# ponimatkin/freepose

Hardware: AMD Instinct MI355X
Metric: proposals/sec (ViT-L feat + top-k + 576-pose render-compare) (higher is better)
Workload: dtype bf16

## Files before the change

### freepose_amd/_lib.py

```python
from __future__ import annotations

import ctypes as C
import os
from pathlib import Path

_HERE = Path(__file__).resolve().parent
LIB_PATH = _HERE / "lib" / "libfreepose_hip.so"
LAB_LIB_PATH = _HERE / "lib" / "libfreepose_hip_lab.so"

_lib = None
_use_lab = False


def use_lab():
    global _use_lab
    if _lib is not None and not _use_lab:
        raise RuntimeError("use_lab() after the product library was loaded")
    _use_lab = True


def is_lab() -> bool:
    return _use_lab

c_void_p, c_int, c_float, c_double, c_size_t, c_char_p = C.c_void_p, C.c_int, C.c_float, C.c_double, C.c_size_t, C.c_char_p
P = C.POINTER


class VitArch(C.Structure):
    _fields_ = [("dim", c_int), ("depth", c_int), ("heads", c_int), ("mlp_dim", c_int), ("patch", c_int),
                ("n_reg", c_int), ("pos_grid", c_int), ("ln_eps", c_float)]


class ClipArch(C.Structure):
    _fields_ = [("width", c_int), ("depth", c_int), ("heads", c_int), ("mlp_dim", c_int), ("patch", c_int), ("grid", c_int),
                ("embed_dim", c_int), ("ln_eps", c_float), ("quick_gelu", c_int)]


class ClipTextArch(C.Structure):
    _fields_ = [("width", c_int), ("depth", c_int), ("heads", c_int), ("mlp_dim", c_int), ("vocab", c_int), ("ctx", c_int),
                ("embed_dim", c_int), ("ln_eps", c_float)]


SIGNATURES = {
    "fp_last_error": (c_char_p, []),
    "fp_version": (c_int, []),
    "fp_ctx_create": (c_int, [c_int, P(c_void_p)]),
    "fp_ctx_destroy": (c_int, [c_void_p]),
    "fp_ctx_set_option": (c_int, [c_void_p, c_char_p, c_int]),
    "fp_ctx_workspace_bytes": (c_size_t, [c_void_p]),
    "fp_vit_create": (c_int, [c_void_p, P(VitArch), P(c_void_p)]),
    "fp_vit_destroy": (c_int, [c_void_p]),
    "fp_vit_set_weight": (c_int, [c_void_p, c_char_p, c_void_p, c_size_t, c_void_p]),
    "fp_vit_forward": (c_int, [c_void_p, c_void_p, c_int, c_int, c_int, c_int, c_int, c_void_p, c_void_p]),
    "fp_vit_flops": (c_double, [c_void_p, c_int, c_int, c_int, c_int]),
    "fp_ffa": (c_int, [c_void_p, c_void_p, c_void_p, c_int, c_int, c_int, c_int, c_int, c_int, c_void_p, c_void_p, c_void_p]),
    "fp_bank_prepare": (c_int, [c_void_p, c_void_p, c_int, c_int, c_void_p, c_void_p]),
    "fp_bank_topk": (c_int, [c_void_p, c_void_p, c_int, c_int, c_void_p, c_int, c_int, c_int, c_void_p, c_void_p, c_void_p]),
    "fp_topk_merge": (c_int, [c_void_p, c_void_p, c_void_p, c_int, c_int, c_int, c_void_p, c_void_p, c_void_p]),
    "fp_rerank_views": (c_int, [c_void_p, c_void_p, c_void_p, c_void_p, c_void_p, c_int, c_int, c_int, c_int, c_void_p, c_void_p]),
    "fp_l2_normalize": (c_int, [c_void_p, c_void_p, c_int, c_int, c_void_p, c_void_p]),
    "fp_template_score": (c_int, [c_void_p, c_void_p, c_void_p, c_void_p, c_int, c_int, c_int, c_void_p, c_void_p]),
    "fp_template_score_normed": (c_int, [c_void_p, c_void_p, c_void_p, c_void_p, c_int, c_int, c_int, c_void_p, c_void_p]),
    "fp_crop_resize_pad": (c_int, [c_void_p, c_void_p, c_int, c_int, c_int, c_int, c_int, c_void_p, c_int, c_float,
                                   c_int, c_void_p, c_int, c_void_p, c_int, c_void_p]),
    "fp_roi_align": (c_int, [c_void_p, c_void_p, c_int, c_int, c_int, c_int, c_void_p, c_int, c_int, c_int, c_int, c_float,
                             c_void_p, c_void_p]),
    "fp_generate_rotations": (c_int, [c_int, c_void_p]),
    "fp_geodesic_select": (c_int, [c_void_p, c_void_p, c_int, c_void_p, c_double, c_void_p, P(c_int), c_void_p]),
    "fp_mesh_upload": (c_int, [c_void_p, c_void_p, c_int, c_void_p, c_int, c_void_p, P(c_void_p)]),
    "fp_mesh_upload_textured": (c_int, [c_void_p, c_void_p, c_int, c_void_p, c_int, c_void_p, c_void_p, c_int, c_int, c_void_p,
                                        P(c_void_p)]),
    "fp_mesh_set_ambient": (c_int, [c_void_p, c_float]),
    "fp_mesh_set_shading": (c_int, [c_void_p, c_int]),
    "fp_mesh_set_filter": (c_int, [c_void_p, c_int]),
    "fp_mesh_set_cull": (c_int, [c_void_p, c_int]),
    "fp_project_vertices": (c_int, [c_void_p, c_void_p, c_void_p, c_int, c_float, c_float, c_float, c_float, c_float, c_void_p,
                                    c_void_p, c_void_p]),
    "fp_mesh_destroy": (c_int, [c_void_p]),
    "fp_rasterize": (c_int, [c_void_p, c_void_p, c_void_p, c_int, c_float, c_float, c_float, c_float, c_float, c_int,
                             c_int, c_void_p, c_void_p, c_void_p]),
    "fp_rasterize_extents": (c_int, [c_void_p, c_void_p, c_void_p, c_int, c_float, c_float, c_float, c_float, c_float, c_int,
                                     c_int, c_void_p, c_void_p, c_void_p, c_void_p, c_void_p]),
    "fp_depth_extents": (c_int, [c_void_p, c_void_p, c_int, c_int, c_int, c_float, c_float, c_float, c_float, c_void_p,
                                 c_void_p]),
    "fp_chamfer": (c_int, [c_void_p, c_void_p, c_int, c_void_p, c_void_p, c_int, c_int, c_int, c_int, c_void_p, c_void_p]),
    "fp_depth_compare": (c_int, [c_void_p, c_void_p, c_void_p, c_int, c_int, c_int, c_void_p, c_int, c_void_p, c_void_p, c_void_p, c_int,
                                 c_void_p, c_void_p]),
    "fp_label_components": (c_int, [c_void_p, c_void_p, c_int, c_int, c_int, c_int, c_void_p, c_void_p]),
    "fp_depthmap_scale": (c_int, [c_void_p, c_void_p, c_void_p, c_int, c_int, c_int, c_double, c_double, c_double, c_double, c_double,
                                  c_double, c_int, c_int, c_void_p, c_void_p, c_void_p, c_void_p]),
    "fp_comm_unique_id": (c_int, [c_void_p]),
    "fp_comm_init": (c_int, [c_void_p, c_int, c_int, c_void_p]),
    "fp_comm_destroy": (c_int, [c_void_p]),
    "fp_comm_size": (c_int, [c_void_p]),
    "fp_comm_rank": (c_int, [c_void_p]),
    "fp_allgather_bytes": (c_int, [c_void_p, c_void_p, c_size_t, c_void_p, c_void_p]),
    "fp_allgather_topk": (c_int, [c_void_p, c_void_p, c_void_p, c_int, c_int, c_int, c_void_p, c_void_p, c_void_p]),
    "fp_allgather_poses": (c_int, [c_void_p, c_void_p, c_int, c_int, c_void_p, c_void_p]),
    "fp_op_gemm": (c_int, [c_void_p, c_void_p, c_int, c_void_p, c_int, c_void_p, c_int, c_void_p, c_void_p, c_void_p, c_int, c_int,
                           c_int, c_int, c_int, c_void_p]),
    "fp_op_gemm_vt": (c_int, [c_void_p, c_void_p, c_int, c_void_p, c_int, c_void_p, c_void_p, c_int, c_int, c_int, c_int, c_int,
                              c_void_p]),
    "fp_op_ln_linear": (c_int, [c_void_p, c_void_p, c_int, c_int, c_void_p, c_void_p, c_float, c_void_p, c_int, c_void_p, c_int, c_int,
                                c_int, c_int, c_float, c_void_p, c_void_p]),
    "fp_op_gemm_stats": (c_int, [c_void_p, c_void_p, c_int, c_void_p, c_int, c_void_p, c_int, c_void_p, c_void_p, c_void_p, c_int, c_int,
                                 c_int, c_int, c_float, c_void_p, c_void_p]),
    "fp_op_gemm_patch": (c_int, [c_void_p, c_void_p, c_int, c_void_p, c_int, c_void_p, c_int, c_void_p, c_void_p, c_int, c_int, c_int,
                                 c_int, c_int, c_int, c_void_p]),
    "fp_op_ln_chain": (c_int, [c_void_p, c_void_p, c_int, c_void_p, c_void_p, c_void_p, c_void_p, c_void_p, c_int, c_int, c_void_p,
                               c_void_p, c_float, c_void_p, c_int, c_void_p, c_int, c_int, c_float, c_int, c_void_p, c_int, c_void_p,
                               c_void_p, c_void_p]),
    "fp_op_gelu": (c_int, [c_void_p, c_void_p, c_size_t, c_void_p]),
    "fp_op_attention": (c_int, [c_void_p, c_int, c_void_p, c_void_p, c_int, c_int, c_int, c_int, c_int, c_int, c_void_p]),
    "fp_op_layernorm": (c_int, [c_void_p, c_void_p, c_void_p, c_void_p, c_int, c_int, c_float, c_void_p]),
    "fp_op_im2col_norm": (c_int, [c_void_p, c_void_p, c_int, c_int, c_int, c_int, c_int, c_void_p]),
    "fp_op_attention_hd": (c_int, [c_void_p, c_int, c_void_p, c_int, c_int, c_int, c_int, c_int, c_int, c_float, c_void_p]),
    "fp_op_attention_causal": (c_int, [c_void_p, c_int, c_void_p, c_int, c_int, c_int, c_int, c_int, c_int, c_float, c_void_p]),
    "fp_clip_text_create": (c_int, [c_void_p, P(ClipTextArch), P(c_void_p)]),
    "fp_clip_text_destroy": (c_int, [c_void_p]),
    "fp_clip_text_set_weight": (c_int, [c_void_p, c_char_p, c_void_p, c_size_t, c_void_p]),
    "fp_clip_text_encode": (c_int, [c_void_p, c_void_p, c_int, c_void_p, c_void_p]),
    "fp_clip_text_flops": (c_double, [c_void_p, c_int]),
    "fp_clip_create": (c_int, [c_void_p, P(ClipArch), P(c_void_p)]),
    "fp_clip_destroy": (c_int, [c_void_p]),
    "fp_clip_set_weight": (c_int, [c_void_p, c_char_p, c_void_p, c_size_t, c_void_p]),
    "fp_clip_encode_image": (c_int, [c_void_p, c_void_p, c_int, c_int, c_void_p, c_void_p]),
    "fp_clip_flops": (c_double, [c_void_p, c_int]),
    "fp_knn_l2": (c_int, [c_void_p, c_void_p, c_int, c_int, c_void_p, c_int, c_int, c_void_p, c_void_p, c_void_p]),
    "fp_patch_points": (c_int, [c_void_p, c_void_p, c_int, c_void_p, c_void_p, c_void_p, c_void_p, c_int, c_int, c_double, c_void_p, c_void_p]),
    "fp_pnp_epnp": (c_int, [c_void_p, c_void_p, c_void_p, c_void_p, c_void_p, c_int, c_int, c_void_p, c_void_p]),
    "fp_video_errors": (c_int, [c_void_p, c_void_p, c_void_p, c_void_p, c_void_p, c_int, c_int, c_int, c_int, c_void_p, c_void_p, c_void_p,
                                c_void_p, c_void_p]),
    "fp_bop_scores": (c_int, [c_void_p, c_void_p, c_void_p, c_void_p, c_void_p, c_void_p, c_void_p, c_int, c_int, c_int, c_int, c_int, c_int,
                              c_int, c_void_p, c_void_p, c_void_p, c_void_p, c_void_p, c_void_p]),
    "fp_gt_visibility": (c_int, [c_void_p, c_void_p, c_int, c_int, c_int, c_int, c_int, c_void_p, c_int, c_int, c_int, c_void_p, c_void_p,
                                 c_void_p, c_void_p, c_void_p, c_void_p]),
    "fp_pts_diameter": (c_int, [c_void_p, c_void_p, c_int, c_void_p, c_int, c_void_p, c_void_p]),
    "fp_timer_create": (c_int, [P(c_void_p)]),
    "fp_timer_start": (c_int, [c_void_p, c_void_p]),
    "fp_timer_stop": (c_int, [c_void_p, c_void_p]),
    "fp_timer_elapsed_ms": (c_int, [c_void_p, P(c_float)]),
    "fp_timer_destroy": (c_int, [c_void_p]),
    "fp_vit_profile": (c_int, [c_void_p, c_int]),
    "fp_vit_profile_read": (c_int, [c_void_p, P(c_float), P(c_float), P(c_float), P(c_double)]),
    "fp_vit_profile_gemm_launches": (C.c_long, [c_void_p]),
}


def load(path: os.PathLike | None = None):
    global _lib
    if _lib is not None and path is None:
        return _lib
    p = Path(path) if path else (LAB_LIB_PATH if _use_lab else LIB_PATH)
    if not p.exists():
        raise RuntimeError(
            f"{p} not found: the HIP extension is not built (run `python -m freepose_amd.build`). "
            "freepose_amd has no CPU fallback.")
    lib = C.CDLL(str(p), mode=C.RTLD_GLOBAL)
    for name, (res, args) in SIGNATURES.items():
        fn = getattr(lib, name)
        fn.restype = res
        fn.argtypes = args
    if hasattr(lib, "fp_lab_set_option"):
        lib.fp_lab_set_option.restype = c_int
        lib.fp_lab_set_option.argtypes = [c_char_p, c_int]
        lib.fp_lab_read_scratch.restype = c_int
        lib.fp_lab_read_scratch.argtypes = [c_void_p, c_void_p, c_size_t]
    if path is None:
        _lib = lib
    return lib


def check(rc: int, what: str = ""):
    if rc != 0:
        msg = load().fp_last_error()
        raise RuntimeError(f"libfreepose_hip {what} failed (code {rc}): {msg.decode() if msg else '?'}")


def ptr(t):
    if t is None:
        return None
    if hasattr(t, "data_ptr"):
        return C.c_void_p(t.data_ptr())
    return C.c_void_p(t.ctypes.data)


def current_stream():
    import torch
    return C.c_void_p(torch.cuda.current_stream().cuda_stream)
```

### freepose_amd/csrc/attention.hip

```cpp
#include "internal.h"

#include <stdlib.h>

#include <type_traits>

namespace {

typedef __attribute__((ext_vector_type(2))) float f32x2_t;

constexpr int HD = 64;
constexpr int KVB = 64;
constexpr int QW = 32;
constexpr int NWAVE = 4;
constexpr int QB = QW * NWAVE;
constexpr int ROWB = 128;
constexpr int TILE = KVB * ROWB;
constexpr int STAGE = 2 * TILE;
constexpr float LAZY_THR = 40.0f;

struct AttnArgs {
    const bf16_t* QK; int ldqk;
    const bf16_t* Vt;
    bf16_t* O; int ldo;
    int B, H, n_tok, npad, D;
    float scale_log2e;
    int q_base;
};

__device__ __forceinline__ float vmax2(float a, float b) {
    float d;
    asm("v_max_f32 %0, %1, %2" : "=v"(d) : "v"(a), "v"(b));
    return d;
}
__device__ __forceinline__ float xlane_max16(float v) {
    const auto r = __builtin_amdgcn_permlane16_swap(__float_as_uint(v), __float_as_uint(v), false, false);
    return vmax2(__uint_as_float(r[0]), __uint_as_float(r[1]));
}
__device__ __forceinline__ float xlane_max32(float v) {
    const auto r = __builtin_amdgcn_permlane32_swap(__float_as_uint(v), __float_as_uint(v), false, false);
    return vmax2(__uint_as_float(r[0]), __uint_as_float(r[1]));
}
__device__ __forceinline__ int key_plain(int row) { return (row >> 1) & 7; }
__device__ __forceinline__ int key_krow(int row) { return ((((row >> 3) & 3) << 1) | ((row >> 1) & 1)) & 7; }
__device__ __forceinline__ int key_perm4(int row) {
    const int rl = row & 63;
    return (((rl >> 4) << 1) | ((rl & 3) >> 1)) & 7;
}

template <int NSLOT, int VAR = 0>
__global__ __launch_bounds__(NWAVE * 64, (VAR & 16) ? 4 : 3) void attn_fwd_kernel(AttnArgs p) {
    extern __shared__ __attribute__((aligned(1024))) char smem[];
    const int tid = threadIdx.x, lane = tid & 63;
    const int wave = __builtin_amdgcn_readfirstlane(tid >> 6);
    const int li = lane & 15, lg = lane >> 4;
    const int nqb = (p.npad - p.q_base + QB - 1) / QB;
    int bid = blockIdx.x;
    {
        const int nwg = gridDim.x;
        const int q = nwg >> 3, r = nwg & 7, xcd = bid & 7, pos = bid >> 3;
        bid = (xcd < r ? xcd * (q + 1) : r * (q + 1) + (xcd - r) * q) + pos;
    }
    const int qb = bid % nqb, bh = bid / nqb;
    const int h = bh % p.H, b = bh / p.H;
    const int q0 = p.q_base + qb * QB + wave * QW;
    const bool idle = q0 >= p.npad;

    const size_t rowbase = (size_t)b * p.npad;
    const char* gQK = (const char*)p.QK;
    const char* gVt = (const char*)(p.Vt + ((size_t)b * p.H + h) * HD * p.npad);

    bf16x8_t qf[2][2];
#pragma unroll
    for (int fq = 0; fq < 2; ++fq) {
        const int q = min(q0 + 16 * fq + li, p.npad - 1);
        const char* src = gQK + ((rowbase + q) * p.ldqk + h * HD) * 2;
#pragma unroll
        for (int kk = 0; kk < 2; ++kk) qf[fq][kk] = *(const bf16x8_t*)(src + (kk * 4 + lg) * 16);
    }

    uint32_t offK[2];
    int rowK[2];
    uint32_t offV[2];
    int slotV[2];
#pragma unroll
    for (int it = 0; it < 2; ++it) {
        const int row = (it * NWAVE + wave) * 8 + (lane >> 3);
        rowK[it] = row;
        offK[it] = (uint32_t)((p.D + h * HD) * 2 + (((lane & 7) ^ key_krow(row)) << 4));
        slotV[it] = (lane & 7) ^ key_perm4(row);
        offV[it] = (uint32_t)row * (uint32_t)p.npad * 2u;
    }
    const char* gKb = gQK + rowbase * (size_t)p.ldqk * 2;
    uint32_t lofK[2], lofV[2];
#pragma unroll
    for (int it = 0; it < 2; ++it) {
        lofK[it] = (uint32_t)rowK[it] * (uint32_t)p.ldqk * 2u + offK[it];
        lofV[it] = offV[it] + (uint32_t)(slotV[it] * 16);
    }
    const uint32_t kstep = (uint32_t)p.ldqk * 2u;
    auto stage = [&](int buf, int kv0) {
        char* sb = smem + buf * STAGE;
        if (kv0 + KVB <= p.npad) {
#pragma unroll
            for (int it = 0; it < 2; ++it) glds16_buf(gKb, lofK[it], (uint32_t)kv0 * kstep, sb + (it * NWAVE + wave) * 1024);
#pragma unroll
            for (int it = 0; it < 2; ++it) glds16_buf(gVt, lofV[it], (uint32_t)kv0 * 2u, sb + TILE + (it * NWAVE + wave) * 1024);
        } else {
#pragma unroll
            for (int it = 0; it < 2; ++it) {
                const int key = min(kv0 + rowK[it], p.npad - 1);
                glds16(gQK + (rowbase + key) * (size_t)p.ldqk * 2 + offK[it], sb + (it * NWAVE + wave) * 1024);
            }
#pragma unroll
            for (int it = 0; it < 2; ++it) {
                const int k8 = min(kv0 + slotV[it] * 8, p.npad - 8);
                glds16(gVt + offV[it] + (size_t)k8 * 2, sb + TILE + (it * NWAVE + wave) * 1024);
            }
        }
    };

    const int keyK = (((li >> 2) << 1) | ((li & 3) >> 1)) & 7;
    const int baseK = ((li >> 2) * 8 + (li & 3)) * ROWB;
    const int keyV = (((li >> 2) << 1) | ((li & 3) >> 1)) & 7;
    const int baseV = TILE + ((li >> 2) * 16 + (li & 3)) * ROWB;

    f32x4_t o[4][2];
#pragma unroll
    for (int i = 0; i < 4; ++i)
#pragma unroll
        for (int j = 0; j < 2; ++j) o[i][j] = f32x4_t{0.f, 0.f, 0.f, 0.f};
    float mrow[2] = {-1e30f, -1e30f};
    float mthr[2] = {-1e30f, -1e30f};
    float nmb[2] = {0.f, 0.f};
    constexpr bool PRE = (VAR & 64) != 0;
    constexpr bool VSUM = (VAR & 256) != 0;
    float vsum[2] = {0.f, 0.f};
    f32x4_t nref[2] = {f32x4_t{0.f, 0.f, 0.f, 0.f}, f32x4_t{0.f, 0.f, 0.f, 0.f}};
    f32x4_t lacc[2] = {f32x4_t{0.f, 0.f, 0.f, 0.f}, f32x4_t{0.f, 0.f, 0.f, 0.f}};
    bf16x8_t ones;
#pragma unroll
    for (int e = 0; e < 8; ++e) ones[e] = (__bf16)1.0f;

    const int ntile = (p.n_tok + KVB - 1) / KVB;
    constexpr bool SHORT = (VAR & 4) != 0;
    auto tile_of = [&](int sq) { return SHORT ? (sq == 0 ? ntile - 1 : sq - 1) : sq; };
    constexpr int PF = NSLOT - 1;
    stage(0, tile_of(0) * KVB);
#pragma unroll
    for (int i = 1; i < PF; ++i)
        if (ntile > i) stage(i, tile_of(i) * KVB);
    asm volatile("s_waitcnt vmcnt(0)" ::: "memory");
#pragma unroll
    for (int fq = 0; fq < 2; ++fq)
#pragma unroll
        for (int kk = 0; kk < 2; ++kk) asm volatile("" : "+v"(qf[fq][kk]));
    if constexpr (VAR & 2) {
        const int d = (blockIdx.x * 5) % 12;
        for (int i = 0; i < d; ++i) __builtin_amdgcn_s_sleep(2);
    }
    auto tile_body = [&](int t, auto slot_c, auto nks_c, auto first_c) {
        const int slot = slot_c;
        constexpr int NKS = decltype(nks_c)::value;
        constexpr bool FIRST = decltype(first_c)::value;
        const int ahead = min(PF - 1, ntile - 1 - t);
        if (ahead >= 2) asm volatile("s_waitcnt vmcnt(8)" ::: "memory");
        else if (ahead == 1) asm volatile("s_waitcnt vmcnt(4)" ::: "memory");
        else asm volatile("s_waitcnt vmcnt(0)" ::: "memory");
        __builtin_amdgcn_s_barrier();
        asm volatile("" ::: "memory");
        if (t + PF < ntile) stage(slot >= 1 ? slot - 1 : NSLOT - 1, tile_of(t + PF) * KVB);
        if (idle) return;
        const char* sb = smem + slot * STAGE;
        const int kv0 = tile_of(t) * KVB;

        f32x4_t s[4][2];
        if constexpr (VAR & 1) __builtin_amdgcn_s_setprio(1);
#pragma unroll
        for (int kk = 0; kk < 2; ++kk) {
            const int slot = (((kk << 2) | lg) ^ keyK) << 4;
#pragma unroll
            for (int fk = 0; fk < 2 * NKS; ++fk) {
                const bf16x8_t kf = *(const bf16x8_t*)(sb + baseK + (32 * (fk >> 1) + 4 * (fk & 1)) * ROWB + slot);
#pragma unroll
                for (int fq = 0; fq < 2; ++fq)
                    s[fk][fq] = __builtin_amdgcn_mfma_f32_16x16x32_bf16(kf, qf[fq][kk], kk == 0 ? (PRE ? nref[fq] : f32x4_t{0.f, 0.f, 0.f, 0.f}) : s[fk][fq], 0, 0, 0);
            }
        }
        if constexpr (VAR & 1) __builtin_amdgcn_s_setprio(0);
        if (kv0 + KVB > p.n_tok) {
#pragma unroll
            for (int fk = 0; fk < 2 * NKS; ++fk)
#pragma unroll
                for (int r = 0; r < 4; ++r)
                    if (kv0 + 32 * (fk >> 1) + 8 * lg + 4 * (fk & 1) + r >= p.n_tok) {
                        s[fk][0][r] = -1e30f;
                        s[fk][1][r] = -1e30f;
                    }
        }

        constexpr bool JITV = (VAR & 16) != 0;
        bf16x8_t vf[JITV ? 1 : 2][4];
        if constexpr (!JITV) {
#pragma unroll
        for (int ks = 0; ks < NKS; ++ks) {
            const int sv = (((ks << 2) | lg) ^ keyV) << 4;
#pragma unroll
            for (int fd = 0; fd < 4; ++fd) vf[ks][fd] = *(const bf16x8_t*)(sb + baseV + fd * 4 * ROWB + sv);
        }
        }

        bf16x8_t pf[2][2];
        auto softmax_max = [&](int fq) {
            float mx;
            if constexpr (NKS == 1)
                asm("v_max3_f32 %0, %1, %2, %3\n\tv_max3_f32 %0, %0, %4, %5\n\tv_max3_f32 %0, %0, %6, %7\n\tv_max_f32 %0, %0, %8"
                    : "=&v"(mx)
                    : "v"(s[0][fq][0]), "v"(s[0][fq][1]), "v"(s[0][fq][2]), "v"(s[0][fq][3]), "v"(s[1][fq][0]), "v"(s[1][fq][1]),
                      "v"(s[1][fq][2]), "v"(s[1][fq][3]));
            else
            asm("v_max3_f32 %0, %1, %2, %3\n\tv_max3_f32 %0, %0, %4, %5\n\tv_max3_f32 %0, %0, %6, %7\n\tv_max3_f32 %0, %0, %8, %9\n\t"
                "v_max3_f32 %0, %0, %10, %11\n\tv_max3_f32 %0, %0, %12, %13\n\tv_max3_f32 %0, %0, %14, %15\n\tv_max_f32 %0, %0, %16"
                : "=&v"(mx)
                : "v"(s[0][fq][0]), "v"(s[0][fq][1]), "v"(s[0][fq][2]), "v"(s[0][fq][3]), "v"(s[1][fq][0]), "v"(s[1][fq][1]),
                  "v"(s[1][fq][2]), "v"(s[1][fq][3]), "v"(s[2][fq][0]), "v"(s[2][fq][1]), "v"(s[2][fq][2]), "v"(s[2][fq][3]),
                  "v"(s[3][fq][0]), "v"(s[3][fq][1]), "v"(s[3][fq][2]), "v"(s[3][fq][3]));
            if constexpr (PRE) {
                constexpr float THR2 = LAZY_THR * 1.4426950408889634f / 8.0f;
                if (FIRST || __builtin_amdgcn_ballot_w64(mx > THR2) != 0) {
                    mx = xlane_max16(mx);
                    mx = xlane_max32(mx);
                    const float delta = FIRST ? mx : vmax2(mx, 0.f);
#pragma unroll
                    for (int r = 0; r < 4; ++r) nref[fq][r] -= delta;
#pragma unroll
                    for (int fk = 0; fk < 2 * NKS; ++fk)
#pragma unroll
                        for (int r = 0; r < 4; ++r) s[fk][fq][r] -= delta;
                    if constexpr (!FIRST) {
                        const float alpha = __builtin_amdgcn_exp2f(-delta);
                        lacc[fq][0] *= alpha;
                        if constexpr (VSUM) vsum[fq] *= alpha;
#pragma unroll
                        for (int fd = 0; fd < 4; ++fd)
#pragma unroll
                            for (int r = 0; r < 4; ++r) o[fd][fq][r] *= alpha;
                    }
                }
            } else
            if (__builtin_amdgcn_ballot_w64(mx > mthr[fq]) != 0) {
                mx = xlane_max16(mx);
                mx = xlane_max32(mx);
                const float mnew = vmax2(mrow[fq], mx);
                const float alpha = __builtin_amdgcn_exp2f((mrow[fq] - mnew) * p.scale_log2e);
                mrow[fq] = mnew;
                mthr[fq] = mnew + LAZY_THR;
                nmb[fq] = -(mnew * p.scale_log2e);
                lacc[fq][0] *= alpha;
#pragma unroll
                for (int fd = 0; fd < 4; ++fd)
#pragma unroll
                    for (int r = 0; r < 4; ++r) o[fd][fq][r] *= alpha;
            }
        };
        auto softmax_exp = [&](int fq) {
            float pv[4][4];
            if constexpr (PRE) {
#pragma unroll
                for (int fk = 0; fk < 2 * NKS; ++fk)
#pragma unroll
                    for (int r = 0; r < 4; ++r) pv[fk][r] = __builtin_amdgcn_exp2f(s[fk][fq][r]);
            } else if constexpr (VAR & 128) {
                const f32x2_t sc2 = {p.scale_log2e, p.scale_log2e};
                const f32x2_t mb2 = {nmb[fq], nmb[fq]};
#pragma unroll
                for (int fk = 0; fk < 2 * NKS; ++fk)
#pragma unroll
                    for (int r = 0; r < 4; r += 2) {
                        const f32x2_t a = {s[fk][fq][r], s[fk][fq][r + 1]};
                        const f32x2_t e = __builtin_elementwise_fma(a, sc2, mb2);
                        pv[fk][r] = __builtin_amdgcn_exp2f(e[0]);
                        pv[fk][r + 1] = __builtin_amdgcn_exp2f(e[1]);
                    }
            } else {
#pragma unroll
                for (int fk = 0; fk < 2 * NKS; ++fk)
#pragma unroll
                    for (int r = 0; r < 4; ++r) {
                        float e;
                        asm("v_fma_f32 %0, %1, %2, %3" : "=v"(e) : "v"(s[fk][fq][r]), "v"(p.scale_log2e), "v"(nmb[fq]));
                        pv[fk][r] = __builtin_amdgcn_exp2f(e);
                    }
            }
#pragma unroll
            for (int ks = 0; ks < NKS; ++ks) {
                uint4 w;
                w.x = pack_bf2(pv[2 * ks][0], pv[2 * ks][1]);
                w.y = pack_bf2(pv[2 * ks][2], pv[2 * ks][3]);
                w.z = pack_bf2(pv[2 * ks + 1][0], pv[2 * ks + 1][1]);
                w.w = pack_bf2(pv[2 * ks + 1][2], pv[2 * ks + 1][3]);
                pf[fq][ks] = __builtin_bit_cast(bf16x8_t, w);
            }
        };
        auto pv_half = [&](int fq) {
#pragma unroll
            for (int ks = 0; ks < NKS; ++ks) {
#pragma unroll
                for (int fd = 0; fd < 4; ++fd)
                    o[fd][fq] = __builtin_amdgcn_mfma_f32_16x16x32_bf16(vf[JITV ? 0 : ks][fd], pf[fq][ks], o[fd][fq], 0, 0, 0);
                lacc[fq] = __builtin_amdgcn_mfma_f32_16x16x32_bf16(ones, pf[fq][ks], lacc[fq], 0, 0, 0);
            }
        };

        if constexpr (JITV) {
            softmax_max(0);
            softmax_exp(0);
            softmax_max(1);
            softmax_exp(1);
#pragma unroll
            for (int ks = 0; ks < NKS; ++ks) {
                const int sv = (((ks << 2) | lg) ^ keyV) << 4;
#pragma unroll
                for (int fd = 0; fd < 4; ++fd) vf[0][fd] = *(const bf16x8_t*)(sb + baseV + fd * 4 * ROWB + sv);
#pragma unroll
                for (int fq = 0; fq < 2; ++fq) {
#pragma unroll
                    for (int fd = 0; fd < 4; ++fd)
                        o[fd][fq] = __builtin_amdgcn_mfma_f32_16x16x32_bf16(vf[0][fd], pf[fq][ks], o[fd][fq], 0, 0, 0);
                    if constexpr (VSUM) {
                        typedef __bf16 bf16x2_hw __attribute__((ext_vector_type(2)));
                        const uint4 pw = __builtin_bit_cast(uint4, pf[fq][ks]);
                        const bf16x2_hw one2 = __builtin_bit_cast(bf16x2_hw, 0x3f803f80u);
                        vsum[fq] = __builtin_amdgcn_fdot2_f32_bf16(__builtin_bit_cast(bf16x2_hw, pw.x), one2, vsum[fq], false);
                        vsum[fq] = __builtin_amdgcn_fdot2_f32_bf16(__builtin_bit_cast(bf16x2_hw, pw.y), one2, vsum[fq], false);
                        vsum[fq] = __builtin_amdgcn_fdot2_f32_bf16(__builtin_bit_cast(bf16x2_hw, pw.z), one2, vsum[fq], false);
                        vsum[fq] = __builtin_amdgcn_fdot2_f32_bf16(__builtin_bit_cast(bf16x2_hw, pw.w), one2, vsum[fq], false);
                    } else {
                        lacc[fq] = __builtin_amdgcn_mfma_f32_16x16x32_bf16(ones, pf[fq][ks], lacc[fq], 0, 0, 0);
                    }
                }
            }
            return;
        }
        softmax_max(0);
        softmax_exp(0);
        softmax_max(1);
        __builtin_amdgcn_sched_barrier(0);
        softmax_exp(1);
        pv_half(0);
#pragma unroll
        for (int g = 0; g < 5 * NKS; ++g) {
            __builtin_amdgcn_sched_group_barrier(0x008, 1, 0);
            __builtin_amdgcn_sched_group_barrier(0x002, 4, 0);
        }
        __builtin_amdgcn_sched_barrier(0);
        if constexpr (VAR & 1) __builtin_amdgcn_s_setprio(1);
        pv_half(1);
        if constexpr (VAR & 1) __builtin_amdgcn_s_setprio(0);
    };
    using full_c = std::integral_constant<int, 2>;
    using half_c = std::integral_constant<int, 1>;
    using yes_c = std::true_type;
    using no_c = std::false_type;
    if constexpr (SHORT) {
        static_assert(NSLOT == 2, "the short-tail prologue is written for the 2-slot ring");
        tile_body(0, std::integral_constant<int, 0>{}, half_c{}, yes_c{});
        for (int t = 1; t < ntile; t += 2) {
            tile_body(t, std::integral_constant<int, 1>{}, full_c{}, no_c{});
            if (t + 1 < ntile) tile_body(t + 1, std::integral_constant<int, 0>{}, full_c{}, no_c{});
        }
    } else if constexpr (NSLOT == 2 && PRE) {
        tile_body(0, std::integral_constant<int, 0>{}, full_c{}, yes_c{});
        for (int t = 1; t < ntile; t += 2) {
            tile_body(t, std::integral_constant<int, 1>{}, full_c{}, no_c{});
            if (t + 1 < ntile) tile_body(t + 1, std::integral_constant<int, 0>{}, full_c{}, no_c{});
        }
    } else if constexpr (NSLOT == 2) {
        for (int t = 0; t < ntile; t += 2) {
            tile_body(t, std::integral_constant<int, 0>{}, full_c{}, no_c{});
            if (t + 1 < ntile) tile_body(t + 1, std::integral_constant<int, 1>{}, full_c{}, no_c{});
        }
    } else {
        tile_body(0, 0, full_c{}, yes_c{});
        int slot = NSLOT > 1 ? 1 : 0;
        for (int t = 1; t < ntile; ++t) {
            tile_body(t, slot, full_c{}, no_c{});
            slot = slot + 1 == NSLOT ? 0 : slot + 1;
        }
    }

#pragma unroll
    for (int fq = 0; fq < 2; ++fq) {
        float rowsum = lacc[fq][0];
        if constexpr (VSUM) {
            rowsum = vsum[fq];
            rowsum += lane_xor<16>(rowsum);
            rowsum += lane_xor<32>(rowsum);
        }
        const float inv = 1.0f / rowsum;
        const int q = q0 + 16 * fq + li;
        if (q < p.npad) {
            uint4 w0, w1;
            w0.x = pack_bf2(o[0][fq][0] * inv, o[0][fq][1] * inv);
            w0.y = pack_bf2(o[0][fq][2] * inv, o[0][fq][3] * inv);
            w0.z = pack_bf2(o[1][fq][0] * inv, o[1][fq][1] * inv);
            w0.w = pack_bf2(o[1][fq][2] * inv, o[1][fq][3] * inv);
            w1.x = pack_bf2(o[2][fq][0] * inv, o[2][fq][1] * inv);
            w1.y = pack_bf2(o[2][fq][2] * inv, o[2][fq][3] * inv);
            w1.z = pack_bf2(o[3][fq][0] * inv, o[3][fq][1] * inv);
            w1.w = pack_bf2(o[3][fq][2] * inv, o[3][fq][3] * inv);
            uint4* dst = (uint4*)(p.O + (rowbase + q) * p.ldo + h * HD + lg * 16);
            dst[0] = w0;
            dst[1] = w1;
        }
    }
}

}

int fp_attention_fwd(const bf16_t* QK, int ldqk, const bf16_t* Vt, bf16_t* O, int ldo, int B, int H,
                     int n_tok, int npad, bool q_prescaled, hipStream_t stream) {
    FP_REQUIRE(B > 0 && H > 0 && n_tok > 0 && npad >= n_tok && npad % 16 == 0,
               "attention: bad shape B=%d H=%d n_tok=%d npad=%d", B, H, n_tok, npad);
    FP_REQUIRE(npad >= 8, "attention: npad too small");
    AttnArgs a;
    a.QK = QK; a.ldqk = ldqk; a.Vt = Vt; a.O = O; a.ldo = ldo;
    a.B = B; a.H = H; a.n_tok = n_tok; a.npad = npad; a.D = H * HD;
    a.scale_log2e = FP_ATTN_QSCALE;
    a.q_base = 0;
    dim3 grid(cdiv(npad - a.q_base, QB) * H * B);
    const bool short_tail = n_tok > KVB && n_tok - (cdiv(n_tok, KVB) - 1) * KVB <= KVB / 2;
#ifdef FP_LAB
    const int nslot = fp_opt_get(FP_OPT_ATTN_SLOTS, 2);
    static int env_var = [] { const char* e = getenv("FP_ATTN_VARIANT"); return e ? atoi(e) : 0; }();
    const int avar = fp_opt_get(FP_OPT_ATTN_VARIANT, env_var);
    if (!q_prescaled) {
    if (nslot == 2 && (avar & 2)) { hipLaunchKernelGGL((attn_fwd_kernel<2, 2>), grid, dim3(NWAVE * 64), 2 * STAGE, stream, a); FP_LAUNCH_CHECK(); return FP_OK; }
    if (nslot == 2 && (avar & 1)) { hipLaunchKernelGGL((attn_fwd_kernel<2, 1>), grid, dim3(NWAVE * 64), 2 * STAGE, stream, a); FP_LAUNCH_CHECK(); return FP_OK; }
    if (nslot == 4) { hipLaunchKernelGGL(attn_fwd_kernel<4>, grid, dim3(NWAVE * 64), 4 * STAGE, stream, a); FP_LAUNCH_CHECK(); return FP_OK; }
    if (nslot == 3) { hipLaunchKernelGGL(attn_fwd_kernel<3>, grid, dim3(NWAVE * 64), 3 * STAGE, stream, a); FP_LAUNCH_CHECK(); return FP_OK; }
    if (avar & 8) { hipLaunchKernelGGL(attn_fwd_kernel<2>, grid, dim3(NWAVE * 64), 2 * STAGE, stream, a); FP_LAUNCH_CHECK(); return FP_OK; }
    if ((avar & 128) && !q_prescaled) {
        if (short_tail) hipLaunchKernelGGL((attn_fwd_kernel<2, 4 | 16 | 128>), grid, dim3(NWAVE * 64), 2 * STAGE, stream, a);
        else hipLaunchKernelGGL((attn_fwd_kernel<2, 16 | 128>), grid, dim3(NWAVE * 64), 2 * STAGE, stream, a);
        FP_LAUNCH_CHECK();
        return FP_OK;
    }
    if (avar & 32) {
        if (short_tail) hipLaunchKernelGGL((attn_fwd_kernel<2, 4>), grid, dim3(NWAVE * 64), 2 * STAGE, stream, a);
        else hipLaunchKernelGGL(attn_fwd_kernel<2>, grid, dim3(NWAVE * 64), 2 * STAGE, stream, a);
        FP_LAUNCH_CHECK();
        return FP_OK;
    }
    }
#endif
#ifdef FP_LAB
    if (q_prescaled && (fp_opt_get(FP_OPT_ATTN_VARIANT, 0) & 256)) {
        if (short_tail) hipLaunchKernelGGL((attn_fwd_kernel<2, 4 | 16 | 64 | 256>), grid, dim3(NWAVE * 64), 2 * STAGE, stream, a);
        else hipLaunchKernelGGL((attn_fwd_kernel<2, 16 | 64 | 256>), grid, dim3(NWAVE * 64), 2 * STAGE, stream, a);
        FP_LAUNCH_CHECK();
        return FP_OK;
    }
#endif
    if (q_prescaled) {
        if (short_tail) hipLaunchKernelGGL((attn_fwd_kernel<2, 4 | 16 | 64>), grid, dim3(NWAVE * 64), 2 * STAGE, stream, a);
        else hipLaunchKernelGGL((attn_fwd_kernel<2, 16 | 64>), grid, dim3(NWAVE * 64), 2 * STAGE, stream, a);
    } else {
        if (short_tail) hipLaunchKernelGGL((attn_fwd_kernel<2, 4 | 16>), grid, dim3(NWAVE * 64), 2 * STAGE, stream, a);
        else hipLaunchKernelGGL((attn_fwd_kernel<2, 16>), grid, dim3(NWAVE * 64), 2 * STAGE, stream, a);
    }
    FP_LAUNCH_CHECK();
    return FP_OK;
}
```

### freepose_amd/csrc/capi.hip

```cpp
#include <stdarg.h>
#include <stdio.h>

#include "../../include/freepose_hip.h"
#include "tower_steps.h"
#include "pnp_core.h"
#include "video_eval_core.h"
#include "gt_info_core.h"

static thread_local char g_err[512] = "";
void fp_set_error(const char* fmt, ...) {
    va_list ap;
    va_start(ap, fmt);
    vsnprintf(g_err, sizeof(g_err), fmt, ap);
    va_end(ap);
}
extern "C" const char* fp_last_error(void) { return g_err; }
extern "C" int fp_version(void) { return 100; }

#ifdef FP_LAB
static int g_opts[FP_OPT_COUNT] = {-1, -1, -1, -1, -1, -1, -1, -1, -1, -1, -1, -1};
int fp_opt_get(int key, int dflt) { return (key >= 0 && key < FP_OPT_COUNT && g_opts[key] >= 0) ? g_opts[key] : dflt; }
extern "C" int fp_lab_set_option(const char* name, int value) {
    FP_REQUIRE(name, "lab_set_option: null name");
    if (!strcmp(name, "gemm_variant")) g_opts[FP_OPT_GEMM_VARIANT] = value;
// ... 207 lines not shown
extern "C" int fp_template_score_normed(fp_ctx* ctx, const void* d_tmpl_normed, const void* d_query, const float* d_weights,
                                        int T, int P, int D, float* d_scores, void* stream) {
    FP_REQUIRE(ctx && d_tmpl_normed && d_query && d_scores, "template_score_normed: null argument");
    if (T == 0) return FP_OK;
    float* dots;
    FP_WS(ctx, "tmpl.dots", (size_t)T * P * 4, dots);
    return fp_template_score_launch((const bf16_t*)d_tmpl_normed, (const bf16_t*)d_query, d_weights, dots, d_scores, T, P, D, 1,
                                    (hipStream_t)stream);
}

extern "C" int fp_chamfer(fp_ctx* ctx, const double* d_pts, int n_pts, const int32_t* d_table, const double* d_xf, int B, int max_n,
                          int ws_pts, int projected, double* d_out, void* stream) {
    FP_REQUIRE(ctx && d_pts && d_table && d_xf && d_out, "chamfer: null argument");
    FP_REQUIRE(B > 0 && B <= 65535, "chamfer: B=%d pairs (1..65535 per call)", B);
    FP_REQUIRE(n_pts > 0 && max_n > 0 && max_n <= n_pts, "chamfer: n_pts=%d max_n=%d (0 < max_n <= n_pts)", n_pts, max_n);
    FP_REQUIRE(ws_pts >= 2 && (size_t)ws_pts <= (size_t)2 * B * (size_t)max_n, "chamfer: ws_pts=%d for %d pairs of clouds up to %d points",
               ws_pts, B, max_n);
    FP_REQUIRE(projected == 0 || projected == 1, "chamfer: projected=%d (0 or 1)", projected);
    float* ws;
    double* slots;
    FP_WS(ctx, "chamfer.cloud", (size_t)ws_pts * 3 * sizeof(float), ws);
    FP_WS(ctx, "chamfer.slots", (size_t)B * 2 * fp_chamfer_chunks(max_n) * sizeof(double), slots);
    return fp_chamfer_launch(d_pts, n_pts, d_table, d_xf, B, max_n, ws_pts, projected, ws, slots, d_out, (hipStream_t)stream);
}

extern "C" int fp_depth_compare(fp_ctx* ctx, const float* d_depth_est, const float* d_depth_gt, int B, int Hh, int W,
                                const float* d_depth_test, int n_img, const int32_t* d_img_idx, const double* d_params,
                                const double* d_taus, int n_tau, int32_t* d_out, void* stream) {
    FP_REQUIRE(ctx && d_depth_est && d_depth_gt && d_out, "depth_compare: null argument");
    FP_REQUIRE(B > 0 && B <= 65535, "depth_compare: B=%d pairs (1..65535 per call)", B);
    FP_REQUIRE(Hh > 0 && W > 0 && (size_t)Hh * W <= ((size_t)1 << 30), "depth_compare: image %d x %d", W, Hh);
    if (d_depth_test) {
        FP_REQUIRE(d_img_idx && d_params && d_taus, "depth_compare: the VSD counts need d_img_idx, d_params and d_taus");
        FP_REQUIRE(n_img > 0 && n_tau > 0 && n_tau <= FP_EVAL_MAX_TAUS, "depth_compare: n_img=%d n_tau=%d (n_tau 1..%d)", n_img, n_tau,
                   FP_EVAL_MAX_TAUS);
    } else {
        FP_REQUIRE(n_tau == 0, "depth_compare: n_tau=%d without a test depth image (the CUS counts take none)", n_tau);
    }
    return fp_depth_compare_launch(d_depth_est, d_depth_gt, B, Hh, W, d_depth_test, n_img, d_img_idx, d_params, d_taus, n_tau, d_out,
                                   (hipStream_t)stream);
}

extern "C" int fp_gt_visibility(fp_ctx* ctx, const float* d_depth_gt, int B, int Hr, int Wr, int ox, int oy, const float* d_depth_test,
                                int n_img, int H, int W, const int32_t* d_img_idx, const double* d_params, uint8_t* d_mask,
                                uint8_t* d_mask_visib, int32_t* d_out, void* stream) {
    FP_REQUIRE(ctx, "gt_visibility: null context");
    FP_REQUIRE(B >= 0 && B <= 65535, "gt_visibility: B=%d instances (0..65535 per call)", B);
    FP_REQUIRE(Hr > 0 && Wr > 0 && (size_t)Hr * Wr <= ((size_t)1 << 30), "gt_visibility: canvas %d x %d", Wr, Hr);
    FP_REQUIRE(gi_window_ok(Wr, Hr, ox, oy, W, H), "gt_visibility: window %d x %d at (%d, %d) leaves the canvas %d x %d", W, H, ox, oy, Wr, Hr);
    FP_REQUIRE(n_img > 0, "gt_visibility: n_img=%d test depth images (>= 1)", n_img);
    if (B == 0) return FP_OK;
    FP_REQUIRE(d_depth_gt && d_depth_test && d_img_idx && d_params && d_out, "gt_visibility: null d_depth_gt, d_depth_test, d_img_idx, d_params or d_out");
    std::vector<int32_t> idx(B);
    FP_HIP(hipMemcpyAsync(idx.data(), d_img_idx, (size_t)B * sizeof(int32_t), hipMemcpyDeviceToHost, (hipStream_t)stream));
    FP_HIP(hipStreamSynchronize((hipStream_t)stream));
    for (int b = 0; b < B; ++b) FP_REQUIRE(gi_img_ok(idx[b], n_img), "gt_visibility: d_img_idx[%d] = %d outside [0, %d)", b, idx[b], n_img);
    return fp_gt_visibility_launch(d_depth_gt, B, Hr, Wr, ox, oy, d_depth_test, n_img, H, W, d_img_idx, d_params, d_mask, d_mask_visib, d_out,
                                   (hipStream_t)stream);
}

extern "C" int fp_pts_diameter(fp_ctx* ctx, const double* d_pts, int n_pts, const int32_t* d_ranges, int M, double* d_out, void* stream) {
    FP_REQUIRE(ctx, "pts_diameter: null context");
    FP_REQUIRE(M >= 0 && M <= 65535, "pts_diameter: M=%d models (0..65535 per call)", M);
    FP_REQUIRE(n_pts >= 0, "pts_diameter: n_pts=%d", n_pts);
    if (M == 0) return FP_OK;
    FP_REQUIRE(d_pts && d_ranges && d_out, "pts_diameter: null d_pts, d_ranges or d_out");
    std::vector<int32_t> rg((size_t)M * 2);
    FP_HIP(hipMemcpyAsync(rg.data(), d_ranges, rg.size() * sizeof(int32_t), hipMemcpyDeviceToHost, (hipStream_t)stream));
    FP_HIP(hipStreamSynchronize((hipStream_t)stream));
    int max_count = 0;
    for (int m = 0; m < M; ++m) {
        FP_REQUIRE(gi_range_ok(rg[2 * m], rg[2 * m + 1], n_pts), "pts_diameter: range %d = {first %d, count %d} is empty or outside [0, %d]", m,
                   rg[2 * m], rg[2 * m + 1], n_pts);
        max_count = std::max(max_count, rg[2 * m + 1]);
    }
    FP_REQUIRE(max_count <= FP_DIAM_MAX_POINTS, "pts_diameter: a model of %d points (at most %d)", max_count, FP_DIAM_MAX_POINTS);
    const size_t tiles = (size_t)cdiv(max_count, fp_pts_diameter_tile()), n_slots = (size_t)M * (tiles * (tiles + 1) / 2);
    FP_REQUIRE(n_slots <= FP_DIAM_MAX_SLOTS, "pts_diameter: %d models of up to %d points need %zu per-block slots (at most %zu per call)", M,
               max_count, n_slots, (size_t)FP_DIAM_MAX_SLOTS);
    double* slots;
    FP_WS(ctx, "diam.slots", n_slots * sizeof(double), slots);
    return fp_pts_diameter_launch(d_pts, n_pts, d_ranges, M, max_count, slots, d_out, (hipStream_t)stream);
}

extern "C" int fp_label_components(fp_ctx* ctx, const uint8_t* d_masks, int n, int H, int W, int connectivity, int32_t* d_labels,
                                   void* stream) {
    FP_REQUIRE(ctx && d_masks && d_labels, "label_components: null argument");
    FP_REQUIRE(connectivity == 4 || connectivity == 8, "label_components: connectivity %d (4 or 8)", connectivity);
    FP_REQUIRE(H >= 1 && W >= 1 && (size_t)H * W <= ((size_t)1 << 30), "label_components: image %d x %d", W, H);
    FP_REQUIRE(n >= 0 && n <= 65535, "label_components: n=%d masks (0..65535 per call)", n);
    if (n == 0) return FP_OK;
    int* uf;
    FP_WS(ctx, "scale.uf", (size_t)n * H * W * sizeof(int), uf);
    return fp_label_launch(d_masks, n, H, W, connectivity, uf, d_labels, nullptr, (hipStream_t)stream);
}

extern "C" int fp_depthmap_scale(fp_ctx* ctx, const double* d_depth, const uint8_t* d_masks, int n, int H, int W, double fx, double fy,
                                 double cx, double cy, double erosion_radius, double std_factor, int min_vertices, int align,
                                 double* d_scale, int32_t* d_info, uint8_t* d_keep, void* stream) {
    FP_REQUIRE(ctx && d_depth && d_masks && d_scale && d_info, "depthmap_scale: null argument");
    FP_REQUIRE(H >= 1 && W >= 1 && (size_t)H * W <= ((size_t)1 << 30), "depthmap_scale: image %d x %d", W, H);
    FP_REQUIRE(n >= 0 && n <= 65535, "depthmap_scale: n=%d masks (0..65535 per call)", n);
    FP_REQUIRE(erosion_radius > 0.0 && erosion_radius <= 8.0, "depthmap_scale: erosion_radius %g (0 < r <= 8: the distance window)", erosion_radius);
    FP_REQUIRE(std_factor >= 0.0 && min_vertices >= 1, "depthmap_scale: std_factor %g, min_vertices %d (>= 0, >= 1)", std_factor, min_vertices);
    FP_REQUIRE(fx != 0.0 && fy != 0.0, "depthmap_scale: focal lengths %g, %g", fx, fy);
    FP_REQUIRE(align == 0 || align == 1, "depthmap_scale: align=%d (0 or 1)", align);
    if (n == 0) return FP_OK;
    const size_t px = (size_t)n * H * W;
    FpScaleWs ws{};
    FP_WS(ctx, "scale.uf", px * sizeof(int), ws.uf);
    FP_WS(ctx, "scale.labels", px * sizeof(int), ws.labels);
    FP_WS(ctx, "scale.area", px * sizeof(int), ws.area);
    FP_WS(ctx, "scale.d2", px, ws.d2);
    FP_WS(ctx, "scale.kflag", px, ws.kflag);
    FP_WS(ctx, "scale.best", (size_t)n * sizeof(unsigned long long), ws.best);
    FP_WS(ctx, "scale.cnt", (size_t)n * 8 * sizeof(int), ws.cnt);
    return fp_depthmap_scale_launch(d_depth, d_masks, n, H, W, fx, fy, cx, cy, erosion_radius, std_factor, min_vertices, align, ws, d_scale,
                                    d_info, d_keep, (hipStream_t)stream);
}

extern "C" int fp_patch_points(fp_ctx* ctx, const double* d_samples, int S, const double* d_T, const double* d_K, const int32_t* d_cells,
                               const int32_t* d_ncells, int B, int C, double patch, int32_t* d_out, void* stream) {
    FP_REQUIRE(ctx && d_samples && d_T && d_K && d_cells && d_ncells && d_out, "patch_points: null argument");
    FP_REQUIRE(S >= 1 && S <= (1 << 24), "patch_points: S=%d samples (1..2^24)", S);
    FP_REQUIRE(B >= 0 && B <= 65535, "patch_points: B=%d items (0..65535 per call)", B);
    FP_REQUIRE(C >= 0 && C <= (1 << 20), "patch_points: C=%d cells per item (0..2^20)", C);
    FP_REQUIRE(patch > 0.0, "patch_points: patch %g (> 0)", patch);
    if (B == 0 || C == 0) return FP_OK;
    double* ws;
    FP_WS(ctx, "refine.proj", (size_t)B * 4 * S * sizeof(double), ws);
    return fp_patch_points_launch(d_samples, S, d_T, d_K, d_cells, d_ncells, B, C, patch, ws, d_out, (hipStream_t)stream);
}

extern "C" int fp_pnp_epnp(fp_ctx* ctx, const double* d_pts3d, const double* d_pts2d, const uint8_t* d_vis, const double* d_K9, int B, int N,
                           double* d_out, void* stream) {
    FP_REQUIRE(ctx && d_pts3d && d_pts2d && d_K9 && d_out, "pnp_epnp: null argument");
    FP_REQUIRE(N >= FP_PNP_MIN_N && N <= FP_PNP_MAX_N, "pnp_epnp: N=%d points (%d..%d)", N, FP_PNP_MIN_N, FP_PNP_MAX_N);
    FP_REQUIRE(B >= 0 && B <= (1 << 20), "pnp_epnp: B=%d problems (0..2^20 per call)", B);
    if (B == 0) return FP_OK;
    return fp_pnp_epnp_launch(d_pts3d, d_pts2d, d_vis, d_K9, B, N, d_out, (hipStream_t)stream);
}

extern "C" int fp_video_errors(fp_ctx* ctx, const double* d_est, const double* d_gt, const int32_t* h_meta, const double* h_params, int M,
                               int V, int Nmax, int D, double* d_per_offset, double* d_final, double* d_aligned, double* d_pairs,
                               void* stream) {
    FP_REQUIRE(ctx && d_est && d_gt && h_meta && h_params && d_per_offset && d_final, "video_errors: null argument");
    FP_REQUIRE(M >= 0 && M <= 65535, "video_errors: M=%d tracks (0..65535 per call)", M);
    FP_REQUIRE(V >= 1 && V <= (1 << 20), "video_errors: V=%d ground-truth trajectories (1..2^20)", V);
    FP_REQUIRE(Nmax >= FP_VE_MIN_N && Nmax <= (1 << 20), "video_errors: Nmax=%d frames (%d..2^20)", Nmax, FP_VE_MIN_N);
    FP_REQUIRE(D >= 1 && D <= FP_VE_MAX_D, "video_errors: D=%d time offsets (1..%d)", D, FP_VE_MAX_D);
    for (int m = 0; m < M; ++m) {
        const int32_t* mt = h_meta + (size_t)m * FP_VE_META_LD;
        const double* pr = h_params + (size_t)m * FP_VE_PARAM_LD;
        FP_REQUIRE(mt[0] >= 0 && mt[0] < V, "video_errors: track %d: video %d (0..%d)", m, mt[0], V - 1);
        FP_REQUIRE(mt[1] >= FP_VE_MIN_N && mt[1] <= Nmax, "video_errors: track %d: N=%d frames (%d..Nmax=%d)", m, mt[1], FP_VE_MIN_N, Nmax);
        FP_REQUIRE(mt[2] >= 1 && mt[2] <= FP_VE_MAX_SYM, "video_errors: track %d: n_sym=%d (1..%d)", m, mt[2], FP_VE_MAX_SYM);
        FP_REQUIRE((mt[3] & ~(FP_VE_HAS_AXIS | FP_VE_HAS_K | FP_VE_NO_ALIGN)) == 0, "video_errors: track %d: flags %d", m, mt[3]);
        for (int d = 0; d < D; ++d)
            FP_REQUIRE(mt[4 + d] >= 1 && mt[4 + d] <= mt[1] - 1, "video_errors: track %d: dt[%d]=%d (1..N-1=%d)", m, d, mt[4 + d], mt[1] - 1);
        FP_REQUIRE(pr[0] > 0.0 && pr[1] > 0.0 && pr[0] < INFINITY && pr[1] < INFINITY, "video_errors: track %d: scales %g, %g (finite, > 0)",
                   m, pr[0], pr[1]);
        FP_REQUIRE(pr[2] > 0.0 && pr[3] > 0.0 && pr[2] < INFINITY && pr[3] < INFINITY, "video_errors: track %d: frame size %g x %g", m, pr[2],
                   pr[3]);
    }
    if (M == 0) return FP_OK;
    int32_t* meta;
    double *params, *frames, *aligned = d_aligned;
    FP_WS(ctx, "video.meta", (size_t)M * FP_VE_META_LD * sizeof(int32_t), meta);
    FP_WS(ctx, "video.params", (size_t)M * FP_VE_PARAM_LD * sizeof(double), params);
    FP_WS(ctx, "video.frames", (size_t)M * Nmax * FP_VE_FRAME_LD * sizeof(double), frames);
    if (!aligned) FP_WS(ctx, "video.aligned", (size_t)M * Nmax * 3 * sizeof(double), aligned);
    hipStream_t s = (hipStream_t)stream;
    FP_HIP(hipMemcpyAsync(meta, h_meta, (size_t)M * FP_VE_META_LD * sizeof(int32_t), hipMemcpyHostToDevice, s));
    FP_HIP(hipMemcpyAsync(params, h_params, (size_t)M * FP_VE_PARAM_LD * sizeof(double), hipMemcpyHostToDevice, s));
    FP_HIP(hipStreamSynchronize(s));
    return fp_video_errors_launch(d_est, d_gt, meta, params, M, Nmax, D, aligned, frames, d_per_offset, d_final, d_pairs, s);
}

extern "C" int fp_bop_scores(fp_ctx* ctx, const double* d_err, const int32_t* d_groups, const uint8_t* d_gt_valid, const int32_t* d_gt_obj,
                             const int32_t* d_gt_scene, const double* d_th, int P, int Gr, int R, int T, int n_obj, int n_scene, int n_top,
                             int32_t* d_match, int32_t* d_tp_obj, int32_t* d_tp_scene, int32_t* d_tar_obj, int32_t* d_tar_scene,
                             void* stream) {
    FP_REQUIRE(ctx && d_th && d_tp_obj && d_tp_scene && d_tar_obj && d_tar_scene, "bop_scores: null argument");
    FP_REQUIRE(T >= 1 && T <= 65536, "bop_scores: T=%d thresholds (1..65536)", T);
    FP_REQUIRE(P >= 0 && Gr >= 0 && R >= 0, "bop_scores: P=%d errors, Gr=%d groups, R=%d ground truths (>= 0)", P, Gr, R);
    FP_REQUIRE(n_obj >= 1 && n_scene >= 1, "bop_scores: n_obj=%d, n_scene=%d (>= 1)", n_obj, n_scene);
    FP_REQUIRE((int64_t)Gr * T <= INT32_MAX && (int64_t)R * T <= INT32_MAX && (int64_t)n_obj * T <= INT32_MAX &&
                   (int64_t)n_scene * T <= INT32_MAX,
               "bop_scores: Gr=%d, R=%d, n_obj=%d, n_scene=%d times T=%d (each product below 2^31)", Gr, R, n_obj, n_scene, T);
    FP_REQUIRE(P == 0 || d_err, "bop_scores: null d_err with P=%d", P);
    FP_REQUIRE(Gr == 0 || d_groups, "bop_scores: null d_groups with Gr=%d", Gr);
    FP_REQUIRE(R == 0 || (d_gt_valid && d_gt_obj && d_gt_scene && d_match), "bop_scores: null ground-truth table or d_match with R=%d", R);
    return fp_bop_scores_launch(d_err, d_groups, d_gt_valid, d_gt_obj, d_gt_scene, d_th, P, Gr, R, T, n_obj, n_scene, n_top, d_match,
                                d_tp_obj, d_tp_scene, d_tar_obj, d_tar_scene, (hipStream_t)stream);
}

extern "C" int fp_op_gemm(fp_ctx* ctx, const void* X, int ldx, const void* W, int ldw, void* Cc, int ldc, const void* bias,
                          const void* gamma, const void* resid, int ldr, int M, int N, int K, int epi, void* stream) {
    FP_REQUIRE(ctx && X && W && Cc && bias, "op_gemm: null argument");
    FP_REQUIRE(epi >= 0 && epi <= 2, "op_gemm: epi %d (0..2)", epi);
    GemmStep t((const bf16_t*)X, ldx, (const bf16_t*)W, K, (bf16_t*)Cc, ldc, (const bf16_t*)bias, M, N, epi == FP_EPI_BIAS_GELU);
    if (epi == FP_EPI_BIAS_LS_RES) t.residual((const bf16_t*)gamma, (const bf16_t*)resid, ldr);
    t.g.ldw = ldw;
    return t.run(ctx, (hipStream_t)stream);
}
extern "C" int fp_op_gemm_vt(fp_ctx* ctx, const void* X, int ldx, const void* W, int ldw, void* Vt, const void* bias, int M, int N,
                             int K, int npad, int heads, void* stream) {
    FP_REQUIRE(ctx && X && W && Vt, "op_gemm_vt: null argument");
    GemmStep t((const bf16_t*)X, ldx, (const bf16_t*)W, K, (bf16_t*)Vt, 8, (const bf16_t*)bias, M, N);
    t.transposed_v(npad, heads).g.ldw = ldw;
    return t.run(ctx, (hipStream_t)stream);
}
extern "C" int fp_op_ln_linear(fp_ctx* ctx, const void* X, int M, int K, const void* g_ln, const void* b_ln, float eps,
                               const void* W, int N, const void* bias, int mode, int npad, int heads, int n_scaled, float row_scale,
                               void* out, void* stream) {
    FP_REQUIRE(ctx && X && g_ln && b_ln && W && bias && out, "op_ln_linear: null argument");
    FP_REQUIRE(mode >= 0 && mode <= 2, "op_ln_linear: mode %d (0..2)", mode);
    hipStream_t s = (hipStream_t)stream;
    const bf16_t* Xb = (const bf16_t*)X;
    bf16_t* Wf;
    uint4* cb;
    LnStats st{nullptr, nullptr, nullptr, M, K, eps};
    int rc;
    FP_WS(ctx, "op.ln_wf", (size_t)N * K * 2, Wf);
    FP_WS(ctx, "op.ln_cb", (size_t)N * sizeof(uint4), cb);
    FP_WS(ctx, "op.ln_stat", (size_t)M * sizeof(uint4), st.stat);
    FP_WS(ctx, "op.ln_rstd", (size_t)M * sizeof(float), st.rstd);
    FP_REQUIRE(n_scaled >= 0 && n_scaled <= N, "op_ln_linear: n_scaled %d outside [0, N]", n_scaled);
    if ((rc = fp_ln_fold((const bf16_t*)W, (const bf16_t*)g_ln, (const bf16_t*)b_ln, (const bf16_t*)bias, Wf, cb, N, K, n_scaled, row_scale, s))) return rc;
    if ((rc = st.ready(Xb, N, s))) return rc;
    GemmStep t(Xb, K, Wf, K, (bf16_t*)out, N, (const bf16_t*)bias, M, N, mode == 1);
    if (mode == 2) t.transposed_v(npad, heads);
    if ((rc = st.attach(t, cb))) return rc;
    return t.run(ctx, s);
}
extern "C" int fp_op_gemm_stats(fp_ctx* ctx, const void* X, int ldx, const void* W, int ldw, void* Cc, int ldc, const void* bias,
                                const void* gamma, const void* resid, int ldr, int M, int N, int K, float eps, float* d_stat,
                                void* stream) {
    FP_REQUIRE(ctx && X && W && Cc && bias && gamma && resid && d_stat, "op_gemm_stats: null argument");
    hipStream_t s = (hipStream_t)stream;
    LnStats st{nullptr, nullptr, nullptr, M, N, eps};
    int rc;
    FP_WS(ctx, "op.ln_part", (size_t)M * (N / 64) * sizeof(float2), st.part);
    FP_WS(ctx, "op.ln_stat", (size_t)M * sizeof(uint4), st.stat);
    FP_WS(ctx, "op.ln_rstd", (size_t)M * sizeof(float), st.rstd);
    GemmStep t((const bf16_t*)X, ldx, (const bf16_t*)W, K, (bf16_t*)Cc, ldc, (const bf16_t*)bias, M, N);
    t.residual((const bf16_t*)gamma, (const bf16_t*)resid, ldr, st.part).g.ldw = ldw;
    if ((rc = t.run(ctx, s))) return rc;
    if ((rc = fp_stats_finalize(st.part, st.stat, st.rstd, M, N, eps, s))) return rc;
    FP_HIP(hipMemcpy2DAsync(d_stat, 24, st.stat, 16, 16, M, hipMemcpyDeviceToDevice, s));
    FP_HIP(hipMemcpy2DAsync(d_stat + 4, 24, st.rstd, 4, 4, M, hipMemcpyDeviceToDevice, s));
    return FP_OK;
}
extern "C" int fp_op_gemm_patch(fp_ctx* ctx, const void* X, int ldx, const void* W, int ldw, void* Cc, int ldc, const void* bias,
                                const void* pos, int M, int N, int K, int P, int npad, int tok_off, void* stream) {
    FP_REQUIRE(ctx && X && W && Cc && bias && pos, "op_gemm_patch: null argument");
    FP_REQUIRE(P > 0 && M > 0 && M % P == 0 && tok_off >= 0 && tok_off + P <= npad && ldc >= N,
               "op_gemm_patch: M=%d P=%d npad=%d tok_off=%d (M %% P == 0, tok_off + P <= npad, ldc >= N)", M, P, npad, tok_off);
    GemmStep t((const bf16_t*)X, ldx, (const bf16_t*)W, K, (bf16_t*)Cc, ldc, (const bf16_t*)bias, M, N);
    t.patch_embed((const bf16_t*)pos, P, npad, tok_off).g.ldw = ldw;
    return t.run(ctx, (hipStream_t)stream);
}
extern "C" int fp_op_ln_chain(fp_ctx* ctx, const void* X1, int K1, const void* W1, const void* b1, const void* gamma, const void* resid,
                              void* Y, int M, int D, const void* g_ln, const void* b_ln, float eps, const void* W2, int N2,
                              const void* b2, int mode, int n_scaled, float row_scale, int route, void* out, int ldo, void* d_mfrag,
                              float* d_rstd, void* stream) {
    FP_REQUIRE(ctx && X1 && W1 && b1 && gamma && resid && Y && g_ln && b_ln && W2 && b2 && out && d_mfrag && d_rstd, "op_ln_chain: null argument");
    FP_REQUIRE((mode == 0 || mode == 1) && (route == 0 || route == 1), "op_ln_chain: mode %d (0..1), route %d (0..1)", mode, route);
    FP_REQUIRE(M > 0 && D > 0 && D % 64 == 0 && ldo >= N2 && n_scaled >= 0 && n_scaled <= N2, "op_ln_chain: M=%d D=%d N2=%d ldo=%d n_scaled=%d", M, D, N2, ldo, n_scaled);
    hipStream_t s = (hipStream_t)stream;
    bf16_t* Wf;
    uint4* cb;
    LnStats st{nullptr, nullptr, nullptr, M, D, eps};
    int rc;
    FP_WS(ctx, "op.ln_wf", (size_t)N2 * D * 2, Wf);
    FP_WS(ctx, "op.ln_cb", (size_t)N2 * sizeof(uint4), cb);
    FP_WS(ctx, "op.ln_stat", (size_t)M * sizeof(uint4), st.stat);
    FP_WS(ctx, "op.ln_rstd", (size_t)M * sizeof(float), st.rstd);
    FP_WS(ctx, "op.ln_part", (size_t)M * (D / 64) * sizeof(float2), st.part);
    FP_HIP(hipMemsetAsync(st.stat, 0xFF, (size_t)M * sizeof(uint4), s));
    FP_HIP(hipMemsetAsync(st.rstd, 0xFF, (size_t)M * sizeof(float), s));
    if ((rc = fp_ln_fold((const bf16_t*)W2, (const bf16_t*)g_ln, (const bf16_t*)b_ln, (const bf16_t*)b2, Wf, cb, N2, D, n_scaled, row_scale, s))) return rc;
    GemmStep prod((const bf16_t*)X1, K1, (const bf16_t*)W1, K1, (bf16_t*)Y, D, (const bf16_t*)b1, M, D);
    if ((rc = prod.residual((const bf16_t*)gamma, (const bf16_t*)resid, D, st.part).run(ctx, s))) return rc;
    if (route == 0 && (rc = fp_stats_finalize(st.part, st.stat, st.rstd, M, D, eps, s))) return rc;
    st.pending = route == 1;
    GemmStep cons((const bf16_t*)Y, D, Wf, D, (bf16_t*)out, ldo, (const bf16_t*)b2, M, N2, mode == 1);
    if ((rc = st.attach(cons, cb))) return rc;
    if ((rc = cons.run(ctx, s))) return rc;
    FP_HIP(hipMemcpyAsync(d_mfrag, st.stat, (size_t)M * sizeof(uint4), hipMemcpyDeviceToDevice, s));
    FP_HIP(hipMemcpyAsync(d_rstd, st.rstd, (size_t)M * sizeof(float), hipMemcpyDeviceToDevice, s));
    return FP_OK;
}
extern "C" int fp_op_gelu(const void* x, void* y, size_t n, void* stream) {
    FP_REQUIRE(x && y, "op_gelu: null argument");
    return fp_gemm_gelu_direct((const bf16_t*)x, (bf16_t*)y, n, (hipStream_t)stream);
}
extern "C" int fp_op_attention(const void* QK, int ldqk, const void* Vt, void* O, int ldo, int B, int H, int n_tok,
                               int npad, int q_prescaled, void* stream) {
    FP_REQUIRE(QK && Vt && O, "op_attention: null argument");
    return fp_attention_fwd((const bf16_t*)QK, ldqk, (const bf16_t*)Vt, (bf16_t*)O, ldo, B, H, n_tok, npad, q_prescaled != 0,
                            (hipStream_t)stream);
}
extern "C" int fp_op_attention_hd(const void* QKV, int ldqkv, void* O, int ldo, int B, int heads, int head_dim, int n_tok, int npad,
                                  float scale, void* stream) {
    return fp_attention_hd_fwd((const bf16_t*)QKV, ldqkv, (bf16_t*)O, ldo, B, heads, head_dim, n_tok, npad, scale, (hipStream_t)stream);
}
extern "C" int fp_op_attention_causal(const void* QKV, int ldqkv, void* O, int ldo, int B, int heads, int head_dim, int n_tok, int npad,
                                      float scale, void* stream) {
    return fp_attention_causal_fwd((const bf16_t*)QKV, ldqkv, (bf16_t*)O, ldo, B, heads, head_dim, n_tok, npad, scale, (hipStream_t)stream);
}
extern "C" int fp_knn_l2(fp_ctx* ctx, const float* d_table, int N, int E, const float* d_queries, int Q, int k, int32_t* d_out_idx,
                         float* d_out_d2, void* stream) {
    FP_REQUIRE(ctx, "knn_l2: null context");
    FP_REQUIRE(N > 0 && Q > 0, "knn_l2: bad shape N=%d Q=%d", N, Q);
    float* ws = nullptr;
    FP_WS(ctx, "knn.d2", (size_t)Q * N * sizeof(float), ws);
    return fp_knn_l2_launch(d_table, N, E, d_queries, Q, k, ws, d_out_idx, d_out_d2, (hipStream_t)stream);
}
extern "C" int fp_op_im2col_norm(const void* img, void* A, int B, int H, int W, int ps, int KP, void* stream) {
    FP_REQUIRE(img && A && B > 0, "op_im2col_norm: null argument / empty batch");
    return fp_im2col_norm_ms((const bf16_t*)img, (bf16_t*)A, B, H, W, ps, KP, FP_IMAGENET_MEAN, FP_IMAGENET_SD, (hipStream_t)stream);
}
extern "C" int fp_op_layernorm(const void* X, void* Y, const void* g, const void* b, int rows, int D, float eps,
                               void* stream) {
    FP_REQUIRE(X && Y && g && b, "op_layernorm: null argument");
    return fp_layernorm((const bf16_t*)X, (bf16_t*)Y, (const bf16_t*)g, (const bf16_t*)b, rows, D, eps, 0, 0, 0,
                        (hipStream_t)stream);
}

struct FpTimer { hipEvent_t a, b; };
extern "C" int fp_timer_create(void** out) {
    FP_REQUIRE(out, "timer_create: null");
    FpTimer* t = new FpTimer();
    FP_HIP(hipEventCreate(&t->a));
    FP_HIP(hipEventCreate(&t->b));
    *out = t;
    return FP_OK;
}
extern "C" int fp_timer_start(void* t, void* s) { FP_HIP(hipEventRecord(((FpTimer*)t)->a, (hipStream_t)s)); return FP_OK; }
extern "C" int fp_timer_stop(void* t, void* s) { FP_HIP(hipEventRecord(((FpTimer*)t)->b, (hipStream_t)s)); return FP_OK; }
extern "C" int fp_timer_elapsed_ms(void* t, float* ms) {
    FP_HIP(hipEventSynchronize(((FpTimer*)t)->b));
    FP_HIP(hipEventElapsedTime(ms, ((FpTimer*)t)->a, ((FpTimer*)t)->b));
    return FP_OK;
}
extern "C" int fp_timer_destroy(void* t) {
    if (!t) return FP_OK;
    (void)hipEventDestroy(((FpTimer*)t)->a);
    (void)hipEventDestroy(((FpTimer*)t)->b);
    delete (FpTimer*)t;
    return FP_OK;
}
```

### freepose_amd/csrc/internal.h

```cpp
#pragma once
#include <algorithm>
#include <map>
#include <string>
#include <vector>

#include "common.h"
#include "gemm_bf16.h"

struct fp_ctx {
    int device = 0;
    struct Buf { void* p = nullptr; size_t bytes = 0; };
    std::map<std::string, Buf> bufs;
    int get(const char* name, size_t bytes, void** out);
    template <class T> int ws(const char* name, size_t bytes, T*& out) { return get(name, bytes, (void**)&out); }
    void* comm = nullptr;
    int comm_rank = 0, comm_size = 1;
    int opt_ln_fused = -1;
    int opt_raster_tiled = -1;
    int opt_comm_timeout_s = -1;
    int opt_row_split = -1;
    int opt_stream_k = -1;
    float* sk_ws = nullptr;
    int* sk_cnt = nullptr;
    static constexpr size_t SK_WS_BYTES = (size_t)64 << 20;
    static constexpr int SK_CNT_N = 16384;
    int sk_scratch(FpGemmArgs& g, hipStream_t s);
    int gemm(FpGemmArgs& g, int epi, hipStream_t s);
    int* ffa_arrive = nullptr;
    size_t total() const;
    void release();
};
#define FP_WS(ctx, name, bytes, p)                                   \
    do {                                                             \
        if (int rc__ = (ctx)->ws(name, bytes, p)) return rc__;       \
    } while (0)

constexpr float FP_ATTN_QSCALE = 1.4426950408889634f / 8.0f;
int fp_attention_fwd(const bf16_t* QK, int ldqk, const bf16_t* Vt, bf16_t* O, int ldo, int B, int H, int n_tok,
                     int npad, bool q_prescaled, hipStream_t stream);
int fp_attention_hd_fwd(const bf16_t* QKV, int ldqkv, bf16_t* O, int ldo, int B, int heads, int head_dim, int n_tok, int npad, float scale,
                        hipStream_t stream);
int fp_attention_causal_fwd(const bf16_t* QKV, int ldqkv, bf16_t* O, int ldo, int B, int heads, int head_dim, int n_tok, int npad, float scale,
                            hipStream_t stream);
constexpr float FP_IMAGENET_MEAN[3] = {0.485f, 0.456f, 0.406f}, FP_IMAGENET_SD[3] = {0.229f, 0.224f, 0.225f};
int fp_im2col_norm_ms(const bf16_t* img, bf16_t* A, int B, int H, int W, int ps, int KP, const float* mean, const float* sd, hipStream_t s);
int fp_token_init(bf16_t* X, const bf16_t* cls, const bf16_t* pos0, const bf16_t* reg, int nreg, int B, int n_tok,
                  int npad, int D, hipStream_t s);
int fp_layernorm(const bf16_t* X, bf16_t* Y, const bf16_t* gamma, const bf16_t* beta, int rows, int D, float eps,
                 int rows_per_b, int in_stride_b, int in_off, hipStream_t s, int l2_normalize = 0);
int fp_posembed_aa(const bf16_t* src, bf16_t* dst, int G, int gh, int gw, int D, hipStream_t s);
int fp_ffa_pool(const bf16_t* feats, const uint8_t* mask, bf16_t* out, float* out_f32, int B, int P, int D, int gh,
                int gw, int cell, uint8_t* pm_scratch, hipStream_t s, bf16_t* out_norm = nullptr, int* arrive = nullptr);
int fp_l2norm_rows(const bf16_t* X, bf16_t* Y, int rows, int D, hipStream_t s);
int fp_row_stats(const bf16_t* X, uint4* mfrag, float* rstd, int rows, int D, float eps, hipStream_t s);
int fp_stats_finalize(const float2* part, uint4* mfrag, float* rstd, int rows, int D, float eps, hipStream_t s, int part_ld = 0);
int fp_ln_fold(const bf16_t* W, const bf16_t* gamma, const bf16_t* beta, const bf16_t* bias, bf16_t* Wf, uint4* cfrag, int N, int K,
               int n_scaled, float row_scale, hipStream_t s);
int fp_cast_f32_bf16(const float* x, bf16_t* y, size_t n, hipStream_t s);
int fp_bank_scan(const bf16_t* bank, const bf16_t* queries, uint16_t* keys, int ldk, int N, int D, int Q, hipStream_t s);
int fp_topk_select(const uint16_t* keys, int ldk, int N, int Q, int k, int idx_offset, float* out_scores, int* out_idx,
                   hipStream_t s);
int fp_topk_merge_launch(const float* cs, const int* ci, int Q, int C, int k, float* out_scores, int* out_idx,
                         hipStream_t s);
int fp_rerank_views_launch(const bf16_t* views, const int* offsets, const int* cand, const bf16_t* queries, float* out,
                           int Q, int C, int D, int k, hipStream_t s);
int fp_template_score_launch(const bf16_t* tmpl, const bf16_t* qn, const float* weights, float* dots, float* scores,
                             int T, int P, int D, int templates_normalised, hipStream_t s);
int fp_knn_l2_launch(const float* table, int N, int E, const float* queries, int Q, int k, float* d2_ws, int* out_idx, float* out_d2,
                     hipStream_t s);
#define FP_EVAL_XF_LD 40
#define FP_EVAL_TABLE_LD 8
#define FP_EVAL_MAX_TAUS 16
int fp_chamfer_chunks(int max_n);
int fp_chamfer_launch(const double* pts, int n_pts, const int* table, const double* xf, int B, int max_n, int ws_pts, int projected,
                      float* ws, double* slots, double* out, hipStream_t s);
int fp_depth_compare_launch(const float* d_est, const float* d_gt, int B, int Hh, int W, const float* d_test, int n_img, const int* img_idx,
                            const double* params, const double* taus, int n_tau, int* out, hipStream_t s);
struct FpScaleWs {
    int* uf;
    int* labels;
    int* area;
    uint8_t* d2;
    uint8_t* kflag;
    unsigned long long* best;
    int* cnt;
};
int fp_label_launch(const uint8_t* masks, int n, int H, int W, int connectivity, int* uf, int* labels, int* area, hipStream_t s);
int fp_depthmap_scale_launch(const double* depth, const uint8_t* masks, int n, int H, int W, double fx, double fy, double cx, double cy,
                             double erosion_radius, double std_factor, int min_vertices, int align, const FpScaleWs& ws, double* scale,
                             int* info, uint8_t* keep, hipStream_t s);
int fp_patch_points_launch(const double* samples, int S, const double* Tm, const double* Km, const int* cells, const int* ncells, int B, int C,
                           double patch, double* ws, int* out, hipStream_t s);
int fp_pnp_epnp_launch(const double* pts3d, const double* pts2d, const uint8_t* vis, const double* K9, int B, int N, double* out,
                       hipStream_t s);
int fp_video_errors_launch(const double* est, const double* gt, const int* meta, const double* params, int M, int Nmax, int D,
                           double* aligned, double* frames, double* per_offset, double* final_out, double* pairs_out, hipStream_t s);
int fp_bop_scores_launch(const double* err, const int32_t* groups, const uint8_t* gt_valid, const int32_t* gt_obj, const int32_t* gt_scene,
                         const double* th, int P, int Gr, int R, int T, int n_obj, int n_scene, int n_top, int32_t* match, int32_t* tp_obj,
                         int32_t* tp_scene, int32_t* tar_obj, int32_t* tar_scene, hipStream_t s);
int fp_gt_visibility_launch(const float* d_gt, int B, int Hr, int Wr, int ox, int oy, const float* d_test, int n_img, int H, int W,
                            const int* img_idx, const double* params, uint8_t* mask, uint8_t* mask_visib, int32_t* out, hipStream_t s);
#define FP_DIAM_MAX_POINTS (1 << 21)
#define FP_DIAM_MAX_SLOTS ((size_t)1 << 26)
int fp_pts_diameter_tile(void);
int fp_pts_diameter_launch(const double* pts, int n_pts, const int* ranges, int M, int max_count, double* slots, double* out, hipStream_t s);
```

### freepose_amd/csrc/vit.hip

```cpp
#include <stdio.h>

#include "../../include/freepose_hip.h"
#include "tower_steps.h"

struct fp_vit {
    fp_ctx* ctx = nullptr;
    fp_vit_arch a{};
    TowerEmbedW emb;
    const bf16_t *normw = nullptr, *normb = nullptr;
    bf16_t* ones = nullptr;
    std::vector<TowerBlockW> blk;
    struct VitFold { bf16_t *qkvw = nullptr, *fc1w = nullptr; uint4 *qkv_cb = nullptr, *fc1_cb = nullptr; };
    std::vector<VitFold> fold;
    int folded_upto = 0;
    hipEvent_t fold_ev = nullptr;
    hipStream_t fold_stream = nullptr;
    bool refold = false;
    std::map<std::pair<int, int>, bf16_t*> pos_cache;
    TowerProf prof;
};

extern "C" int fp_vit_create(fp_ctx* ctx, const fp_vit_arch* arch, fp_vit** out) {
    FP_REQUIRE(ctx && arch && out, "vit_create: null argument");
    FP_REQUIRE(arch->dim % 64 == 0 && arch->heads * 64 == arch->dim, "vit_create: dim=%d heads=%d (head dim must be 64)",
               arch->dim, arch->heads);
    FP_REQUIRE(arch->mlp_dim % 64 == 0 && arch->depth > 0 && arch->patch > 0, "vit_create: bad arch");
    fp_vit* v = new fp_vit();
    v->ctx = ctx;
    v->a = *arch;
    v->blk.resize(arch->depth);
    v->fold.resize(arch->depth);
    v->emb.patch = arch->patch; v->emb.n_reg = arch->n_reg; v->emb.mean = FP_IMAGENET_MEAN; v->emb.sd = FP_IMAGENET_SD;
    v->emb.KP = cdiv(3 * arch->patch * arch->patch, 64) * 64;
    if (hipMalloc((void**)&v->emb.pe_w, (size_t)arch->dim * v->emb.KP * 2) != hipSuccess ||
        hipMalloc((void**)&v->ones, (size_t)arch->dim * 2) != hipSuccess) {
        fp_set_error("vit_create: hipMalloc failed");
        delete v;
        return FP_ERR_HIP;
    }
    FP_HIP(hipMemset(v->emb.pe_w, 0, (size_t)arch->dim * v->emb.KP * 2));
    std::vector<bf16_t> one(arch->dim, f2bf(1.0f));
    FP_HIP(hipMemcpy(v->ones, one.data(), (size_t)arch->dim * 2, hipMemcpyHostToDevice));
    *out = v;
    return FP_OK;
}
extern "C" int fp_vit_destroy(fp_vit* v) {
    if (!v) return FP_OK;
    if (v->emb.pe_w) (void)hipFree(v->emb.pe_w);
    if (v->ones) (void)hipFree(v->ones);
    for (auto& kv : v->pos_cache) (void)hipFree(kv.second);
    for (auto& f : v->fold) {
        if (f.qkvw) (void)hipFree(f.qkvw);
        if (f.fc1w) (void)hipFree(f.fc1w);
        if (f.qkv_cb) (void)hipFree(f.qkv_cb);
        if (f.fc1_cb) (void)hipFree(f.fc1_cb);
    }
    for (auto& p : v->prof.ev_pool) { (void)hipEventDestroy(p.a); (void)hipEventDestroy(p.b); }
    if (v->fold_ev) (void)hipEventDestroy(v->fold_ev);
    delete v;
    return FP_OK;
}

extern "C" int fp_vit_set_weight(fp_vit* v, const char* name, const void* d, size_t numel, void* stream) {
    FP_REQUIRE(v && name && d, "vit_set_weight: null argument");
    const fp_vit_arch& a = v->a;
    const bf16_t* p = (const bf16_t*)d;
    const size_t D = a.dim;
    if (v->folded_upto > 0) v->refold = true;
    v->folded_upto = 0;
    std::string s(name);
    if (s == "pos_embed") {
        if (!fp_weight_numel("vit_set_weight", name, numel, (size_t)(1 + a.pos_grid * a.pos_grid) * D)) return FP_ERR_INVALID;
        v->emb.pos = p;
        for (auto& kv : v->pos_cache) (void)hipFree(kv.second);
        v->pos_cache.clear();
        return FP_OK;
    }
    if (s == "mask_token") return FP_OK;
    if (s == "patch_embed.proj.weight") return fp_tower_set_patch_weight("vit_set_weight", name, p, numel, v->emb, D, (hipStream_t)stream);
    const WeightEnt top[] = {{"cls_token", &v->emb.cls, D}, {"register_tokens", &v->emb.reg, (size_t)a.n_reg * D}, {"patch_embed.proj.bias", &v->emb.pe_b, D},
                             {"norm.weight", &v->normw, D}, {"norm.bias", &v->normb, D}};
    if (const int hit = fp_set_named_weight("vit_set_weight", name, name, top, p, numel)) return hit > 0 ? FP_OK : FP_ERR_INVALID;
    int bi = -1;
    char rest[64] = {0};
    if (sscanf(name, "blocks.%d.%63s", &bi, rest) == 2 && bi >= 0 && bi < a.depth) {
        TowerBlockW& w = v->blk[bi];
        const size_t M = a.mlp_dim;
        const WeightEnt tab[] = {
            {"norm1.weight", &w.n1w, D}, {"norm1.bias", &w.n1b, D},
            {"attn.qkv.weight", &w.qkvw, 3 * D * D}, {"attn.qkv.bias", &w.qkvb, 3 * D},
            {"attn.proj.weight", &w.projw, D * D}, {"attn.proj.bias", &w.projb, D},
            {"ls1.gamma", &w.ls1, D}, {"norm2.weight", &w.n2w, D}, {"norm2.bias", &w.n2b, D},
            {"mlp.fc1.weight", &w.fc1w, M * D}, {"mlp.fc1.bias", &w.fc1b, M},
            {"mlp.fc2.weight", &w.fc2w, D * M}, {"mlp.fc2.bias", &w.fc2b, D}, {"ls2.gamma", &w.ls2, D}};
        if (const int hit = fp_set_named_weight("vit_set_weight", name, rest, tab, p, numel)) return hit > 0 ? FP_OK : FP_ERR_INVALID;
    }
    fp_set_error("vit_set_weight: unknown tensor name '%s'", name);
    return FP_ERR_INVALID;
}

static int vit_pos(fp_vit* v, int gh, int gw, hipStream_t s, const bf16_t** out) {
    const fp_vit_arch& a = v->a;
    if (gh == a.pos_grid && gw == a.pos_grid) { *out = v->emb.pos + a.dim; return FP_OK; }
    auto key = std::make_pair(gh, gw);
    auto it = v->pos_cache.find(key);
    if (it == v->pos_cache.end()) {
        bf16_t* buf = nullptr;
        FP_HIP(hipMalloc((void**)&buf, (size_t)gh * gw * a.dim * 2));
        int rc = fp_posembed_aa(v->emb.pos + a.dim, buf, a.pos_grid, gh, gw, a.dim, s);
        if (rc) { (void)hipFree(buf); return rc; }
        it = v->pos_cache.emplace(key, buf).first;
    }
    *out = it->second;
    return FP_OK;
}

static int vit_fold(fp_vit* v, int first, int L, hipStream_t s) {
    const fp_vit_arch& a = v->a;
    const size_t D = a.dim, Mm = a.mlp_dim;
    for (int i = first; i < L; ++i) {
        const TowerBlockW& w = v->blk[i];
        fp_vit::VitFold& f = v->fold[i];
        if (!f.qkvw) FP_HIP(hipMalloc((void**)&f.qkvw, 3 * D * D * 2));
        if (!f.qkv_cb) FP_HIP(hipMalloc((void**)&f.qkv_cb, 3 * D * sizeof(uint4)));
        if (!f.fc1w) FP_HIP(hipMalloc((void**)&f.fc1w, Mm * D * 2));
        if (!f.fc1_cb) FP_HIP(hipMalloc((void**)&f.fc1_cb, Mm * sizeof(uint4)));
        int rc;
        if ((rc = fp_ln_fold(w.qkvw, w.n1w, w.n1b, w.qkvb, f.qkvw, f.qkv_cb, (int)(3 * D), (int)D, (int)D, FP_ATTN_QSCALE, s))) return rc;
        if ((rc = fp_ln_fold(w.fc1w, w.n2w, w.n2b, w.fc1b, f.fc1w, f.fc1_cb, (int)Mm, (int)D, 0, 1.0f, s))) return rc;
    }
    return FP_OK;
}

extern "C" double fp_vit_flops(const fp_vit* v, int B, int H, int W, int layer) {
    const fp_vit_arch& a = v->a;
    const double P = (double)(H / a.patch) * (W / a.patch), N = P + 1 + a.n_reg, D = a.dim;
    const int L = std::min(layer, a.depth);
    const double mlp_ratio = (double)a.mlp_dim / a.dim;
    const double per_block = (8.0 + 4.0 * mlp_ratio) * N * D * D + 4.0 * N * N * D;
    return B * (L * per_block + 2.0 * P * (3.0 * a.patch * a.patch) * D);
}

extern "C" int fp_vit_forward(fp_vit* v, const void* d_images, int B, int H, int W, int layer, int feature_type,
                              void* d_out, void* stream) {
    FP_REQUIRE(v && d_images && d_out, "vit_forward: null argument");
    const fp_vit_arch& a = v->a;
    hipStream_t s = (hipStream_t)stream;
    fp_ctx* ctx = v->ctx;
    FP_REQUIRE(B > 0 && H % a.patch == 0 && W % a.patch == 0, "vit_forward: B=%d H=%d W=%d (patch %d)", B, H, W, a.patch);
    FP_REQUIRE(feature_type >= 0 && feature_type <= 3, "vit_forward: feature_type %d", feature_type);
    FP_REQUIRE(v->emb.cls && v->emb.pos && v->emb.pe_b && v->normw && v->normb && (a.n_reg == 0 || v->emb.reg),
               "vit_forward: embedding / final-norm weights not set");
    const int L = (layer >= 1 && layer <= a.depth) ? layer : a.depth;
    for (int i = 0; i < L; ++i) {
        FP_REQUIRE(v->blk[i].complete(), "vit_forward: weights of block %d not set", i);
    }
    const int D = a.dim, gh = H / a.patch, gw = W / a.patch, P = gh * gw;
    const int n_tok = P + 1 + a.n_reg;
    const int npad = cdiv(n_tok, 16) * 16;
    const size_t M = (size_t)B * npad;
    FP_REQUIRE(M * (size_t)a.mlp_dim * 2 < 0xffffffffull, "vit_forward: batch too large for 32-bit tile offsets (B=%d)", B);
    const int Mi = (int)M;

    bf16_t *A0, *X, *Y, *QK, *Vt, *AO, *H1;
    int rc;
    const bool lnf = ctx->opt_ln_fused != 0 && D % 64 == 0;
    LnStats st{nullptr, nullptr, nullptr, Mi, D, a.ln_eps};
    if (lnf) {
        if (v->fold_ev && s != v->fold_stream) FP_HIP(hipStreamWaitEvent(s, v->fold_ev, 0));
        if (v->folded_upto < L) {
            if (v->refold) {
                FP_HIP(hipDeviceSynchronize());
                v->refold = false;
            }
            if ((rc = vit_fold(v, v->folded_upto, L, s))) return rc;
            if (!v->fold_ev) FP_HIP(hipEventCreateWithFlags(&v->fold_ev, hipEventDisableTiming));
            FP_HIP(hipEventRecord(v->fold_ev, s));
            v->fold_stream = s;
            v->folded_upto = L;
        }
        FP_WS(ctx, "vit.ln_stat", M * sizeof(uint4), st.stat);
        FP_WS(ctx, "vit.ln_rstd", M * sizeof(float), st.rstd);
        FP_WS(ctx, "vit.ln_part", M * (size_t)(D / 64) * sizeof(float2), st.part);
    }
    FP_WS(ctx, "vit.im2col", (size_t)B * P * v->emb.KP * 2, A0);
    FP_WS(ctx, "vit.x", M * D * 2, X);
    FP_WS(ctx, "vit.y", M * D * 2, Y);
    FP_WS(ctx, "vit.qk", M * 2 * D * 2, QK);
    FP_WS(ctx, "vit.vt", M * D * 2 + 256, Vt);
    FP_WS(ctx, "vit.ao", M * D * 2, AO);
    FP_WS(ctx, "vit.h1", M * (size_t)a.mlp_dim * 2, H1);

    const bf16_t* pos_patch;
    if ((rc = vit_pos(v, gh, gw, s, &pos_patch))) return rc;

    const TowerRun t{ctx, &v->prof, s, B, n_tok, npad, D, a.mlp_dim, a.ln_eps, X, Y, AO, H1, v->ones};
    if ((rc = fp_tower_embed(t, v->emb, pos_patch, (const bf16_t*)d_images, H, W, A0, X))) return rc;
    const bf16_t* in = lnf ? X : Y;
    for (int i = 0; i < L; ++i) {
        const TowerBlockW& w = v->blk[i];
        const fp_vit::VitFold& f = v->fold[i];
        {
            ProfScope ps(&v->prof, s, TOWER_OTHER);
            if ((rc = lnf ? st.ready(i == 0 ? X : nullptr, 2 * D, s) : fp_layernorm(X, Y, w.n1w, w.n1b, Mi, D, a.ln_eps, 0, 0, 0, s))) return rc;
        }
        {
            ProfScope ps(&v->prof, s, TOWER_GEMM);
            const bf16_t* qkvw = lnf ? f.qkvw : w.qkvw;
            GemmStep qk(in, D, qkvw, D, QK, 2 * D, w.qkvb, Mi, 2 * D), vt(in, D, qkvw + (size_t)2 * D * D, D, Vt, 8, w.qkvb + 2 * D, Mi, D);
            vt.transposed_v(npad, a.heads);
            if (lnf && ((rc = st.attach(qk, f.qkv_cb)) || (rc = st.attach(vt, f.qkv_cb + 2 * D)))) return rc;
            if ((rc = qk.run(ctx, s))) return rc;
            if ((rc = vt.run(ctx, s))) return rc;
            t.count(2.0 * 3.0 * D * D, 2);
        }
        {
            ProfScope ps(&v->prof, s, TOWER_ATTN);
            if ((rc = fp_attention_fwd(QK, 2 * D, Vt, AO, D, B, a.heads, n_tok, npad, lnf, s))) return rc;
        }
        if ((rc = fp_tower_out_proj(t, w, st.part))) return rc;
        if ((rc = fp_tower_mlp(t, w, lnf ? &st : nullptr, f.fc1w, f.fc1_cb, i + 1 < L ? st.part : nullptr))) return rc;
    }
    {
        ProfScope ps(&v->prof, s, TOWER_OTHER);
        const int rows_per_b = feature_type == 0 ? 1 : (feature_type == 1 ? a.n_reg : P);
        const int off = feature_type == 0 ? 0 : (feature_type == 1 ? 1 : 1 + a.n_reg);
        if (rows_per_b > 0)
            if ((rc = fp_layernorm(X, (bf16_t*)d_out, v->normw, v->normb, B * rows_per_b, D, a.ln_eps, rows_per_b, npad,
                                   off, s, feature_type == 3)))
                return rc;
    }
    return FP_OK;
}

extern "C" int fp_vit_profile(fp_vit* v, int enable) {
    FP_REQUIRE(v, "vit_profile: null");
    TowerProf& p = v->prof;
    p.on = enable != 0;
    p.ev_used = 0;
    p.gemm_flops = 0;
    p.gemm_launches = 0;
    return FP_OK;
}
extern "C" int fp_vit_profile_read(fp_vit* v, float* g, float* at, float* o, double* fl) {
    FP_REQUIRE(v, "vit_profile_read: null");
    TowerProf& p = v->prof;
    float acc[3] = {0.f, 0.f, 0.f};
    for (size_t i = 0; i < p.ev_used; ++i) {
        FP_HIP(hipEventSynchronize(p.ev_pool[i].b));
        float ms = 0.f;
        FP_HIP(hipEventElapsedTime(&ms, p.ev_pool[i].a, p.ev_pool[i].b));
        acc[p.ev_pool[i].cls] += ms;
    }
    if (g) *g = acc[TOWER_GEMM];
    if (at) *at = acc[TOWER_ATTN];
    if (o) *o = acc[TOWER_OTHER];
    if (fl) *fl = p.gemm_flops;
    return FP_OK;
}
extern "C" long fp_vit_profile_gemm_launches(const fp_vit* v) { return v ? v->prof.gemm_launches : 0; }
```

### freepose_amd/ops.py

```python
from __future__ import annotations

import ctypes as C
import functools
from typing import Optional

import numpy as np
import torch

from . import _lib
from ._lib import check, current_stream, ptr

_ctx = {}


def context(device: Optional[int] = None):
    if device is None:
        device = torch.cuda.current_device()
    h = _ctx.get(device)
    if h is None:
        lib = _lib.load()
        out = C.c_void_p()
        check(lib.fp_ctx_create(int(device), C.byref(out)), "fp_ctx_create")
        h = _ctx[device] = out
    return h
# ... 594 lines not shown
            if len(wrong):
                r = int(idx[wrong[0]])
                raise ValueError(f"bop_scores: {name}[{r}] = {int(col[r])} (one index in 0..{n - 1} for all rows of a group)")
    return err, groups, gt_valid, gt_obj, gt_scene, th


def bop_scores(err, groups, gt_valid, gt_obj, gt_scene, th, n_obj: int, n_scene: int, n_top: int = 0):
    err, groups, gt_valid, gt_obj, gt_scene, th = bop_tables_check(err, groups, gt_valid, gt_obj, gt_scene, th, n_obj, n_scene)
    lib = _lib.load()
    P, Gr, R, T = len(err), len(groups), len(gt_valid), len(th)
    dev = torch.device("cuda", torch.cuda.current_device())
    up = lambda a: torch.from_numpy(a).to(dev) if a.size else None
    d_err, d_groups, d_valid, d_obj, d_scene, d_th = up(err), up(groups), up(gt_valid), up(gt_obj), up(gt_scene), up(th)
    match = torch.empty((T, R), dtype=torch.int32, device=dev)
    tp_obj = torch.empty((T, int(n_obj)), dtype=torch.int32, device=dev)
    tp_scene = torch.empty((T, int(n_scene)), dtype=torch.int32, device=dev)
    tar_obj = torch.empty((int(n_obj),), dtype=torch.int32, device=dev)
    tar_scene = torch.empty((int(n_scene),), dtype=torch.int32, device=dev)
    check(lib.fp_bop_scores(context(), ptr(d_err), ptr(d_groups), ptr(d_valid), ptr(d_obj), ptr(d_scene), ptr(d_th), P, Gr, R, T, int(n_obj),
                            int(n_scene), int(n_top), ptr(match) if R else None, ptr(tp_obj), ptr(tp_scene), ptr(tar_obj), ptr(tar_scene),
                            current_stream()), "fp_bop_scores")
    return match, tp_obj, tp_scene, tar_obj, tar_scene


EVAL_XF_LD, EVAL_TABLE_LD, EVAL_MAX_TAUS = 40, 8, 16
EVAL_MAX_PAIRS = 65535
EVAL_MAX_WS_POINTS = 32 << 20


def _per_pair(x, B, shape, what):
    a = np.asarray(x.detach().cpu() if isinstance(x, torch.Tensor) else x, dtype=np.float64)
    if a.size == int(np.prod(shape)):
        a = np.broadcast_to(a.reshape(shape), (B,) + tuple(shape))
    if a.size != B * int(np.prod(shape)):
        raise ValueError(f"{what}: expected {tuple(shape)} or {(B,) + tuple(shape)}, got {a.shape}")
    return a.reshape((B,) + tuple(shape))


def _chamfer(clouds, pairs, s_e, R_e, t_e, R_g, t_g, K):
    lib = _lib.load()
    pairs = np.asarray(pairs, dtype=np.int64).reshape(-1, 2)
    B = pairs.shape[0]
    dev = torch.device("cuda", torch.cuda.current_device())
    out = torch.empty((B,), dtype=torch.float64, device=dev)
    if B == 0:
        return out
    cl = [_dev(torch.as_tensor(c), torch.float64).reshape(-1, 3) for c in clouds]
    sizes = np.array([c.shape[0] for c in cl], dtype=np.int64)
    if (sizes <= 0).any():
        raise ValueError("chamfer: empty vertex cloud")
    if pairs.min() < 0 or pairs.max() >= len(cl):
        raise ValueError("chamfer: pair refers to a cloud that was not given")
    starts = np.concatenate([[0], np.cumsum(sizes)])
    if starts[-1] >= 1 << 31:
        raise ValueError("chamfer: more than 2^31 vertices in one call")
    pts = cl[0] if len(cl) == 1 else torch.cat(cl, dim=0)
    centroid = {}
    for g in np.unique(pairs[:, 1]):
        centroid[int(g)] = cl[int(g)].mean(dim=0).cpu().numpy()
    xf = np.zeros((B, EVAL_XF_LD), dtype=np.float64)
    xf[:, 0] = _per_pair(s_e, B, (), "s_e")
    xf[:, 1:10] = _per_pair(R_e, B, (3, 3), "R_e").reshape(B, 9)
    xf[:, 10:13] = _per_pair(t_e, B, (3,), "t_e")
    xf[:, 13:22] = _per_pair(R_g, B, (3, 3), "R_g").reshape(B, 9)
    xf[:, 22:25] = _per_pair(t_g, B, (3,), "t_g")
    xf[:, 25:28] = np.stack([centroid[int(g)] for g in pairs[:, 1]])
    if K is not None:
        xf[:, 28:37] = _per_pair(K, B, (3, 3), "K").reshape(B, 9)
    n_e, n_g = sizes[pairs[:, 0]], sizes[pairs[:, 1]]
    b0 = 0
    while b0 < B:
        b1, ws = b0, 0
        while b1 < B and b1 - b0 < EVAL_MAX_PAIRS and (b1 == b0 or ws + n_e[b1] + n_g[b1] <= EVAL_MAX_WS_POINTS):
            ws += int(n_e[b1] + n_g[b1])
            b1 += 1
        if ws >= 1 << 31:
            raise ValueError("chamfer: one pair of clouds exceeds the workspace index range")
        nb = b1 - b0
        table = np.zeros((nb, EVAL_TABLE_LD), dtype=np.int32)
        table[:, 0], table[:, 1] = starts[pairs[b0:b1, 0]], n_e[b0:b1]
        table[:, 2], table[:, 3] = starts[pairs[b0:b1, 1]], n_g[b0:b1]
        slot = np.concatenate([[0], np.cumsum(n_e[b0:b1] + n_g[b0:b1])])
        table[:, 4], table[:, 5] = slot[:-1], slot[:-1] + n_e[b0:b1]
        d_table = torch.from_numpy(table).to(dev)
        d_xf = torch.from_numpy(xf[b0:b1].copy()).to(dev)
        max_n = int(max(n_e[b0:b1].max(), n_g[b0:b1].max()))
        check(lib.fp_chamfer(context(), ptr(pts), int(starts[-1]), ptr(d_table), ptr(d_xf), nb, max_n, int(ws), int(K is not None),
                             C.c_void_p(out.data_ptr() + 8 * b0), current_stream()), "fp_chamfer")
        b0 = b1
    return out


def chamfer(clouds, pairs, s_e, R_e, t_e, R_g, t_g) -> torch.Tensor:
    return _chamfer(clouds, pairs, s_e, R_e, t_e, R_g, t_g, None)


def chamfer_proj(clouds, pairs, s_e, R_e, t_e, R_g, t_g, K) -> torch.Tensor:
    return _chamfer(clouds, pairs, s_e, R_e, t_e, R_g, t_g, K)


def depth_compare(depth_est: torch.Tensor, depth_gt: torch.Tensor, depth_test: Optional[torch.Tensor] = None, img_idx=None, K=None,
                  delta=None, taus=None, divisor=1.0) -> torch.Tensor:
    lib = _lib.load()
    de, dg = _dev(depth_est, torch.float32), _dev(depth_gt, torch.float32)
    if de.dim() != 3 or de.shape != dg.shape:
        raise ValueError(f"depth_compare: depth stacks {tuple(de.shape)} and {tuple(dg.shape)}")
    B, H, W = de.shape
    if depth_test is None:
        out = torch.zeros((B, 4), dtype=torch.int32, device=de.device)
        for b0 in range(0, B, EVAL_MAX_PAIRS):
            nb = min(EVAL_MAX_PAIRS, B - b0)
            check(lib.fp_depth_compare(context(), ptr(de[b0:]), ptr(dg[b0:]), nb, H, W, None, 0, None, None, None, 0, ptr(out[b0:]),
                                       current_stream()), "fp_depth_compare")
        return out
    dt = _dev(depth_test, torch.float32)
    if dt.dim() == 2:
        dt = dt[None]
    if tuple(dt.shape[1:]) != (H, W):
        raise ValueError(f"depth_compare: test depth {tuple(dt.shape)} for renders of {H} x {W}")
    tau = np.asarray(taus, dtype=np.float64).reshape(-1)
    if not 0 < tau.size <= EVAL_MAX_TAUS:
        raise ValueError(f"depth_compare: {tau.size} taus (1..{EVAL_MAX_TAUS})")
    idx = np.zeros(B, np.int32) if img_idx is None else np.asarray(img_idx, dtype=np.int32).reshape(B)
    if B and (idx.min() < 0 or idx.max() >= dt.shape[0]):
        raise ValueError("depth_compare: img_idx outside the test depth stack")
    Kb = _per_pair(K, B, (3, 3), "K")
    prm = np.zeros((B, 8), dtype=np.float64)
    prm[:, 0], prm[:, 1], prm[:, 2], prm[:, 3] = Kb[:, 0, 0], Kb[:, 1, 1], Kb[:, 0, 2], Kb[:, 1, 2]
    prm[:, 4] = _per_pair(delta, B, (), "delta")
    prm[:, 5] = _per_pair(divisor, B, (), "divisor")
    d_prm, d_idx, d_tau = torch.from_numpy(prm).to(de.device), torch.from_numpy(idx).to(de.device), torch.from_numpy(tau).to(de.device)
    out = torch.zeros((B, 4 + tau.size), dtype=torch.int32, device=de.device)
    for b0 in range(0, B, EVAL_MAX_PAIRS):
        nb = min(EVAL_MAX_PAIRS, B - b0)
        check(lib.fp_depth_compare(context(), ptr(de[b0:]), ptr(dg[b0:]), nb, H, W, ptr(dt), int(dt.shape[0]), ptr(d_idx[b0:]),
                                   ptr(d_prm[b0:]), ptr(d_tau), int(tau.size), ptr(out[b0:]), current_stream()), "fp_depth_compare")
    return out


GT_INFO_OUT_LD = 12
GT_INFO_MAX_BATCH = 65535
GT_INFO_BOX_EMPTY = (2 ** 31 - 1, 2 ** 31 - 1, -2 ** 31, -2 ** 31)
DIAMETER_TILE = 1024
DIAMETER_MAX_POINTS = 1 << 21
DIAMETER_MAX_MODELS = 65535
DIAMETER_MAX_SLOTS = 1 << 24


def gt_visibility(depth_gt, depth_test, img_idx, K, delta, window=None, want_masks: bool = True):
    lib = _lib.load()
    dg, dt = _dev(torch.as_tensor(depth_gt), torch.float32), _dev(torch.as_tensor(depth_test), torch.float32)
    if dt.dim() == 2:
        dt = dt[None]
    if dg.dim() != 3 or dt.dim() != 3:
        raise ValueError(f"gt_visibility: depth stacks {tuple(dg.shape)} and {tuple(dt.shape)} ([B,Hr,Wr] and [n_img,H,W])")
    B, Hr, Wr = dg.shape
    n_img, H, W = dt.shape
    if window is None:
        if (Hr, Wr) != (H, W):
            raise ValueError(f"gt_visibility: canvases of {Wr} x {Hr} for images of {W} x {H} need a window")
        ox, oy = 0, 0
    else:
        ox, oy = int(window[0]), int(window[1])
    if n_img < 1 or H < 1 or W < 1 or Hr * Wr > 1 << 30:
        raise ValueError(f"gt_visibility: {n_img} test images of {W} x {H}, canvas {Wr} x {Hr}")
    if ox < 0 or oy < 0 or ox + W > Wr or oy + H > Hr:
        raise ValueError(f"gt_visibility: window {W} x {H} at ({ox}, {oy}) leaves the canvas {Wr} x {Hr}")
    idx = np.zeros(B, np.int32) if img_idx is None else np.asarray(img_idx, dtype=np.int64).reshape(-1)
    if idx.size != B:
        raise ValueError(f"gt_visibility: {idx.size} image indices for {B} instances")
    if B and (idx.min() < 0 or idx.max() >= n_img):
        raise ValueError(f"gt_visibility: img_idx outside [0, {n_img})")
    Kb = _per_pair(K, B, (3, 3), "K")
    prm = np.zeros((B, 8), dtype=np.float64)
    prm[:, 0], prm[:, 1], prm[:, 2], prm[:, 3] = Kb[:, 0, 0], Kb[:, 1, 1], Kb[:, 0, 2], Kb[:, 1, 2]
    prm[:, 4] = _per_pair(delta, B, (), "delta")
    out = torch.empty((B, GT_INFO_OUT_LD), dtype=torch.int32, device=dg.device)
    mask = torch.empty((B, H, W), dtype=torch.uint8, device=dg.device) if want_masks else None
    visib = torch.empty((B, H, W), dtype=torch.uint8, device=dg.device) if want_masks else None
    if B == 0:
        return out, mask, visib
    d_prm, d_idx = torch.from_numpy(prm).to(dg.device), torch.from_numpy(idx.astype(np.int32)).to(dg.device)
    for b0 in range(0, B, GT_INFO_MAX_BATCH):
        nb = min(GT_INFO_MAX_BATCH, B - b0)
        check(lib.fp_gt_visibility(context(), ptr(dg[b0:]), nb, Hr, Wr, ox, oy, ptr(dt), n_img, H, W, ptr(d_idx[b0:]), ptr(d_prm[b0:]),
                                   ptr(mask[b0:]) if want_masks else None, ptr(visib[b0:]) if want_masks else None, ptr(out[b0:]),
                                   current_stream()), "fp_gt_visibility")
    return out, mask, visib


def pts_diameter(clouds) -> torch.Tensor:
    lib = _lib.load()
    cl = [_dev(torch.as_tensor(c), torch.float64).reshape(-1, 3) for c in clouds]
    M = len(cl)
    dev = torch.device("cuda", torch.cuda.current_device())
    out = torch.empty((M, 8), dtype=torch.float64, device=dev)
    if M == 0:
        return out
    sizes = np.array([c.shape[0] for c in cl], dtype=np.int64)
    if (sizes <= 0).any():
        raise ValueError(f"pts_diameter: cloud {int(np.flatnonzero(sizes <= 0)[0])} is empty")
    if sizes.max() > DIAMETER_MAX_POINTS:
        raise ValueError(f"pts_diameter: a cloud of {int(sizes.max())} points (at most {DIAMETER_MAX_POINTS})")
    starts = np.concatenate([[0], np.cumsum(sizes)])
    if starts[-1] >= 1 << 31:
        raise ValueError("pts_diameter: more than 2^31 points in one call")
    pts = cl[0] if M == 1 else torch.cat(cl, dim=0)
    tiles = -(-sizes // DIAMETER_TILE)
    pairs = tiles * (tiles + 1) // 2
    if pairs.max() > DIAMETER_MAX_SLOTS:
        raise ValueError(f"pts_diameter: a cloud of {int(sizes.max())} points needs {int(pairs.max())} slots (limit {DIAMETER_MAX_SLOTS})")
    m0 = 0
    while m0 < M:
        m1, most = m0, 0
        while m1 < M and m1 - m0 < DIAMETER_MAX_MODELS and (m1 == m0 or max(most, int(pairs[m1])) * (m1 - m0 + 1) <= DIAMETER_MAX_SLOTS):
            most = max(most, int(pairs[m1]))
            m1 += 1
        rg = np.stack([starts[m0:m1], sizes[m0:m1]], axis=1).astype(np.int32)
        d_rg = torch.from_numpy(rg).to(dev)
        check(lib.fp_pts_diameter(context(), ptr(pts), int(starts[-1]), ptr(d_rg), m1 - m0, ptr(out[m0:]), current_stream()), "fp_pts_diameter")
        m0 = m1
    return out


def gemm(x: torch.Tensor, w: torch.Tensor, bias: torch.Tensor, epi: int = 0, gamma=None, resid=None,
         out: Optional[torch.Tensor] = None) -> torch.Tensor:
    lib = _lib.load()
    x, w, bias = _dev(x, torch.bfloat16), _dev(w, torch.bfloat16), _dev(bias, torch.bfloat16)
    M, K = x.shape
    N = w.shape[0]
    g = _dev(gamma, torch.bfloat16) if gamma is not None else None
    r = _dev(resid, torch.bfloat16) if resid is not None else None
    if out is None:
        out = torch.empty((M, N), dtype=torch.bfloat16, device=x.device)
    check(lib.fp_op_gemm(context(), ptr(x), K, ptr(w), K, ptr(out), N, ptr(bias), ptr(g), ptr(r), N, M, N, K, epi, current_stream()),
          "fp_op_gemm")
    return out


def gelu_direct(x: torch.Tensor) -> torch.Tensor:
    x = _dev(x, torch.bfloat16)
    y = torch.empty_like(x)
    check(_lib.load().fp_op_gelu(ptr(x), ptr(y), x.numel(), current_stream()), "fp_op_gelu")
    return y


def gemm_vt(x: torch.Tensor, w: torch.Tensor, bias: torch.Tensor, npad: int, heads: int,
            out: Optional[torch.Tensor] = None) -> torch.Tensor:
    lib = _lib.load()
    x, w, bias = _dev(x, torch.bfloat16), _dev(w, torch.bfloat16), _dev(bias, torch.bfloat16)
    M, K = x.shape
    N = w.shape[0]
    B = M // npad
    vt = out if out is not None else torch.zeros((B, heads, 64, npad), dtype=torch.bfloat16, device=x.device)
    check(lib.fp_op_gemm_vt(context(), ptr(x), K, ptr(w), K, ptr(vt), ptr(bias), M, N, K, npad, heads, current_stream()), "fp_op_gemm_vt")
    return vt


def ln_linear(x: torch.Tensor, g_ln: torch.Tensor, b_ln: torch.Tensor, w: torch.Tensor, bias: torch.Tensor, mode: int = 0,
              npad: int = 0, heads: int = 0, eps: float = 1e-6, n_scaled: int = 0, row_scale: float = 1.0) -> torch.Tensor:
    lib = _lib.load()
    x, w, bias = _dev(x, torch.bfloat16), _dev(w, torch.bfloat16), _dev(bias, torch.bfloat16)
    g_ln, b_ln = _dev(g_ln, torch.bfloat16), _dev(b_ln, torch.bfloat16)
    M, K = x.shape
    N = w.shape[0]
    if mode == 2:
        out = torch.zeros((M // npad, heads, 64, npad), dtype=torch.bfloat16, device=x.device)
    else:
        out = torch.empty((M, N), dtype=torch.bfloat16, device=x.device)
    check(lib.fp_op_ln_linear(context(), ptr(x), M, K, ptr(g_ln), ptr(b_ln), float(eps), ptr(w), N, ptr(bias), int(mode), int(npad),
                              int(heads), int(n_scaled), float(row_scale), ptr(out), current_stream()), "fp_op_ln_linear")
    return out


def gemm_stats(x: torch.Tensor, w: torch.Tensor, bias: torch.Tensor, gamma: torch.Tensor, resid: torch.Tensor, eps: float = 1e-6):
    lib = _lib.load()
    x, w, bias = _dev(x, torch.bfloat16), _dev(w, torch.bfloat16), _dev(bias, torch.bfloat16)
    g, r = _dev(gamma, torch.bfloat16), _dev(resid, torch.bfloat16)
    M, K = x.shape
    N = w.shape[0]
    out = torch.empty((M, N), dtype=torch.bfloat16, device=x.device)
    raw = torch.zeros((M, 6), dtype=torch.float32, device=x.device)
    check(lib.fp_op_gemm_stats(context(), ptr(x), K, ptr(w), K, ptr(out), N, ptr(bias), ptr(g), ptr(r), N, M, N, K, float(eps), ptr(raw),
                               current_stream()), "fp_op_gemm_stats")
    rec = raw[:, :4].contiguous().view(torch.bfloat16).float()
    stat = torch.stack([-(rec[:, 3] + rec[:, 4]), rec[:, 0] + rec[:, 1], raw[:, 4]], dim=1)
    return out, stat


ATTN_QSCALE = 1.4426950408889634 / 8.0


def attention(qk: torch.Tensor, vt: torch.Tensor, n_tok: int, out: Optional[torch.Tensor] = None, q_prescaled: bool = False) -> torch.Tensor:
    lib = _lib.load()
    qk, vt = _dev(qk, torch.bfloat16), _dev(vt, torch.bfloat16)
    B, H, _, npad = vt.shape
    if out is None:
        out = torch.zeros((B * npad, H * 64), dtype=torch.bfloat16, device=qk.device)
    check(lib.fp_op_attention(ptr(qk), 2 * H * 64, ptr(vt), ptr(out), H * 64, B, H, n_tok, npad, int(bool(q_prescaled)), current_stream()),
          "fp_op_attention")
    return out


def attention_hd(qkv: torch.Tensor, heads: int, n_tok: int, scale: Optional[float] = None, out: Optional[torch.Tensor] = None) -> torch.Tensor:
    lib = _lib.load()
    qkv = _dev(qkv, torch.bfloat16)
    if qkv.dim() != 3 or qkv.shape[2] % (3 * heads) != 0:
        raise ValueError(f"attention_hd: qkv of shape {tuple(qkv.shape)} ([B, npad, 3*heads*hd]) with heads={heads}")
    B, npad, w3 = qkv.shape
    width = w3 // 3
    hd = width // heads
    if out is None:
        out = torch.zeros((B, npad, width), dtype=torch.bfloat16, device=qkv.device)
    else:
        assert out.dtype == torch.bfloat16 and out.is_cuda and tuple(out.shape) == (B, npad, width)
        assert out.stride(2) == 1 and out.stride(0) == npad * out.stride(1)
    sc = float(scale) if scale is not None else 1.0 / float(np.sqrt(hd))
    check(lib.fp_op_attention_hd(ptr(qkv), w3, ptr(out), int(out.stride(1)), B, heads, hd, int(n_tok), npad, sc, current_stream()),
          "fp_op_attention_hd")
    return out


def attention_causal(qkv: torch.Tensor, heads: int, n_tok: int, scale: Optional[float] = None, out: Optional[torch.Tensor] = None) -> torch.Tensor:
    lib = _lib.load()
    qkv = _dev(qkv, torch.bfloat16)
    if qkv.dim() != 3 or qkv.shape[2] % (3 * heads) != 0:
        raise ValueError(f"attention_causal: qkv of shape {tuple(qkv.shape)} ([B, npad, 3*heads*hd]) with heads={heads}")
    B, npad, w3 = qkv.shape
    width = w3 // 3
    hd = width // heads
    if out is None:
        out = torch.zeros((B, npad, width), dtype=torch.bfloat16, device=qkv.device)
    else:
        assert out.dtype == torch.bfloat16 and out.is_cuda and tuple(out.shape) == (B, npad, width)
        assert out.stride(2) == 1 and out.stride(0) == npad * out.stride(1)
    sc = float(scale) if scale is not None else 1.0 / float(np.sqrt(hd))
    check(lib.fp_op_attention_causal(ptr(qkv), w3, ptr(out), int(out.stride(1)), B, heads, hd, int(n_tok), npad, sc, current_stream()),
          "fp_op_attention_causal")
    return out


def knn_l2(table: torch.Tensor, queries: torch.Tensor, k: int):
    lib = _lib.load()
    t, q = _dev(torch.as_tensor(table), torch.float32), _dev(torch.as_tensor(queries), torch.float32)
    if t.dim() != 2 or q.dim() != 2 or t.shape[1] != q.shape[1]:
        raise ValueError(f"knn_l2: table {tuple(t.shape)} and queries {tuple(q.shape)} ([N,E] and [Q,E])")
    N, E = t.shape
    Q = q.shape[0]
    idx = torch.empty((Q, int(k)), dtype=torch.int32, device=t.device)
    d2 = torch.empty((Q, int(k)), dtype=torch.float32, device=t.device)
    if Q > 0:
        check(lib.fp_knn_l2(context(), ptr(t), N, E, ptr(q), Q, int(k), ptr(idx), ptr(d2), current_stream()), "fp_knn_l2")
    return idx, d2


CLIP_ARCHS = {
    "ViT-bigG-14": (1664, 48, 16, 8192, 1280, 14, 16),
    "ViT-H-14": (1280, 32, 16, 5120, 1024, 14, 16),
    "ViT-L-14": (1024, 24, 16, 4096, 768, 14, 16),
    "tiny-64": (128, 2, 2, 512, 64, 14, 16), "tiny-80": (320, 2, 4, 640, 64, 14, 16), "tiny-104": (832, 2, 8, 1024, 64, 14, 16),
    "tiny-64-s56": (128, 2, 2, 512, 64, 14, 4), "tiny-80-s56": (320, 2, 4, 640, 64, 14, 4), "tiny-104-s56": (832, 2, 8, 1024, 64, 14, 4),
    "tiny-bigG-wide": (1664, 1, 16, 128, 1280, 14, 4),
}


def clip_state_dict_names(model_name: str) -> dict:
    width, depth, heads, mlp, embed, patch, grid = CLIP_ARCHS[model_name]
    names = {"conv1.weight": (width, 3, patch, patch), "class_embedding": (width,), "positional_embedding": (1 + grid * grid, width),
             "ln_pre.weight": (width,), "ln_pre.bias": (width,), "ln_post.weight": (width,), "ln_post.bias": (width,), "proj": (width, embed)}
    for i in range(depth):
        p = f"transformer.resblocks.{i}."
        names.update({p + "ln_1.weight": (width,), p + "ln_1.bias": (width,), p + "attn.in_proj_weight": (3 * width, width),
                      p + "attn.in_proj_bias": (3 * width,), p + "attn.out_proj.weight": (width, width), p + "attn.out_proj.bias": (width,),
                      p + "ln_2.weight": (width,), p + "ln_2.bias": (width,), p + "mlp.c_fc.weight": (mlp, width), p + "mlp.c_fc.bias": (mlp,),
                      p + "mlp.c_proj.weight": (width, mlp), p + "mlp.c_proj.bias": (width,)})
    return names


def random_clip_state_dict(model_name: str, seed: int = 0) -> dict:
    width = CLIP_ARCHS[model_name][0]
    g = torch.Generator().manual_seed(seed)

    def tn(shape, std=0.02):
        return torch.nn.init.trunc_normal_(torch.empty(*shape), std=std, a=-2 * std, b=2 * std, generator=g)

    sd = {}
    for name, shape in clip_state_dict_names(model_name).items():
        if name.endswith(("ln_pre.weight", "ln_post.weight", "ln_1.weight", "ln_2.weight")):
            sd[name] = torch.ones(shape) + tn(shape, std=0.05)
        elif name == "proj":
            sd[name] = tn(shape, std=width ** -0.5)
        else:
            sd[name] = tn(shape)
    return {k: v.to(torch.bfloat16) for k, v in sd.items()}


class ClipVisual:

    def __init__(self, model_name: str = "ViT-bigG-14", state_dict: Optional[dict] = None, seed: int = 0, device: Optional[int] = None,
                 quick_gelu: bool = False):
        if model_name not in CLIP_ARCHS:
            raise ValueError(f"unknown CLIP model {model_name}")
        self.width, self.depth, self.heads, self.mlp_dim, self.embed_dim, self.patch, self.grid = CLIP_ARCHS[model_name]
        self.model_name = model_name
        self.image_size = self.patch * self.grid
        self.lib = _lib.load()
        self.ctx = context(device)
        arch = _lib.ClipArch(self.width, self.depth, self.heads, self.mlp_dim, self.patch, self.grid, self.embed_dim, 1e-5, int(bool(quick_gelu)))
        h = C.c_void_p()
        check(self.lib.fp_clip_create(self.ctx, C.byref(arch), C.byref(h)), "fp_clip_create")
        self.handle = h
        self.weights = {}
        self.load_state_dict(state_dict if state_dict is not None else random_clip_state_dict(model_name, seed))

    def load_state_dict(self, sd: dict):
        s = current_stream()
        want = clip_state_dict_names(self.model_name)
        missing = sorted(set(want) - set(sd))
        if missing:
            raise KeyError(f"CLIP state dict lacks {len(missing)} tensors, e.g. {missing[:3]}")
        for name in want:
            w = _dev(torch.as_tensor(sd[name]), torch.bfloat16)
            self.weights[name] = w
            check(self.lib.fp_clip_set_weight(self.handle, name.encode(), ptr(w), w.numel(), s), f"set_weight({name})")
        torch.cuda.synchronize()

    def encode_image(self, images: torch.Tensor) -> torch.Tensor:
        x = _dev(images, torch.bfloat16)
        if x.dim() != 4 or x.shape[1] != 3 or x.shape[2] != x.shape[3]:
            raise ValueError(f"CLIP images of shape {tuple(x.shape)} ([B,3,S,S])")
        B, S = x.shape[0], x.shape[2]
        out = torch.empty((B, self.embed_dim), dtype=torch.bfloat16, device=x.device)
        if B > 0:
            check(self.lib.fp_clip_encode_image(self.handle, ptr(x), B, S, ptr(out), current_stream()), "fp_clip_encode_image")
        return out

    __call__ = encode_image

    def flops(self, B: int) -> float:
        return float(self.lib.fp_clip_flops(self.handle, int(B)))

    def __del__(self):
        try:
            self.lib.fp_clip_destroy(self.handle)
        except Exception:
            pass


CLIP_TEXT_ARCHS = {
    "ViT-bigG-14": (1280, 32, 20, 5120, 49408, 77, 1280),
    "ViT-H-14": (1024, 24, 16, 4096, 49408, 77, 1024),
    "ViT-L-14": (768, 12, 12, 3072, 49408, 77, 768),
    "tiny-64": (128, 2, 2, 512, 1024, 77, 64), "tiny-80": (320, 2, 4, 640, 1024, 77, 64), "tiny-104": (832, 2, 8, 1024, 1024, 77, 64),
    "tiny-64-s56": (128, 2, 2, 512, 1024, 77, 64), "tiny-80-s56": (320, 2, 4, 640, 1024, 77, 64), "tiny-104-s56": (832, 2, 8, 1024, 1024, 77, 64),
    "tiny-bigG-wide": (1280, 2, 20, 256, 1024, 77, 1280),
    "tiny-64-c17": (128, 2, 2, 512, 1024, 17, 64),
    "tiny-bigG-text": (1280, 1, 20, 256, 1024, 77, 1280),
}


def clip_text_state_dict_names(model_name: str) -> dict:
    width, depth, heads, mlp, vocab, ctx, embed = CLIP_TEXT_ARCHS[model_name]
    names = {"token_embedding.weight": (vocab, width), "positional_embedding": (ctx, width), "ln_final.weight": (width,),
             "ln_final.bias": (width,), "text_projection": (width, embed)}
    for i in range(depth):
        p = f"transformer.resblocks.{i}."
        names.update({p + "ln_1.weight": (width,), p + "ln_1.bias": (width,), p + "attn.in_proj_weight": (3 * width, width),
                      p + "attn.in_proj_bias": (3 * width,), p + "attn.out_proj.weight": (width, width), p + "attn.out_proj.bias": (width,),
                      p + "ln_2.weight": (width,), p + "ln_2.bias": (width,), p + "mlp.c_fc.weight": (mlp, width), p + "mlp.c_fc.bias": (mlp,),
                      p + "mlp.c_proj.weight": (width, mlp), p + "mlp.c_proj.bias": (width,)})
    return names


def random_clip_text_state_dict(model_name: str, seed: int = 0) -> dict:
    width = CLIP_TEXT_ARCHS[model_name][0]
    g = torch.Generator().manual_seed(seed)

    def tn(shape, std=0.02):
        return torch.nn.init.trunc_normal_(torch.empty(*shape), std=std, a=-2 * std, b=2 * std, generator=g)

    sd = {}
    for name, shape in clip_text_state_dict_names(model_name).items():
        if name.endswith(("ln_final.weight", "ln_1.weight", "ln_2.weight")):
            sd[name] = torch.ones(shape) + tn(shape, std=0.05)
        elif name == "text_projection":
            sd[name] = tn(shape, std=width ** -0.5)
        elif name == "positional_embedding":
            sd[name] = tn(shape, std=0.01)
        else:
            sd[name] = tn(shape)
    return {k: v.to(torch.bfloat16) for k, v in sd.items()}


class ClipText:

    def __init__(self, model_name: str = "ViT-bigG-14", state_dict: Optional[dict] = None, seed: int = 0, device: Optional[int] = None,
                 chunk: int = 256):
        if model_name not in CLIP_TEXT_ARCHS:
            raise ValueError(f"unknown CLIP text model {model_name}")
        self.width, self.depth, self.heads, self.mlp_dim, self.vocab, self.ctx, self.embed_dim = CLIP_TEXT_ARCHS[model_name]
        self.model_name = model_name
        self.chunk = int(chunk)
        self.lib = _lib.load()
        self.ctx_handle = context(device)
        arch = _lib.ClipTextArch(self.width, self.depth, self.heads, self.mlp_dim, self.vocab, self.ctx, self.embed_dim, 1e-5)
        h = C.c_void_p()
        check(self.lib.fp_clip_text_create(self.ctx_handle, C.byref(arch), C.byref(h)), "fp_clip_text_create")
        self.handle = h
        self.weights = {}
        self.load_state_dict(state_dict if state_dict is not None else random_clip_text_state_dict(model_name, seed))

    def load_state_dict(self, sd: dict):
        s = current_stream()
        want = clip_text_state_dict_names(self.model_name)
        missing = sorted(set(want) - set(sd))
        if missing:
            raise KeyError(f"CLIP text state dict lacks {len(missing)} tensors, e.g. {missing[:3]}")
        for name in want:
            w = _dev(torch.as_tensor(sd[name]), torch.bfloat16)
            self.weights[name] = w
            check(self.lib.fp_clip_text_set_weight(self.handle, name.encode(), ptr(w), w.numel(), s), f"set_weight({name})")
        torch.cuda.synchronize()

    def encode_text(self, ids: torch.Tensor, chunk: Optional[int] = None) -> torch.Tensor:
        ids = torch.as_tensor(ids)
        if ids.dim() != 2 or ids.shape[1] != self.ctx or ids.is_floating_point():
            raise ValueError(f"CLIP text ids of shape {tuple(ids.shape)} {ids.dtype} (integer [N, {self.ctx}])")
        x = ids.to("cuda", dtype=torch.int32).contiguous()
        step = max(1, int(chunk or self.chunk))
        out = torch.empty((x.shape[0], self.embed_dim), dtype=torch.bfloat16, device=x.device)
        for i in range(0, x.shape[0], step):
            part, dst = x[i:i + step], out[i:i + step]
            check(self.lib.fp_clip_text_encode(self.handle, ptr(part), part.shape[0], ptr(dst), current_stream()), "fp_clip_text_encode")
        return out

    __call__ = encode_text

    def flops(self, B: int) -> float:
        return float(self.lib.fp_clip_text_flops(self.handle, int(B)))

    def __del__(self):
        try:
            self.lib.fp_clip_text_destroy(self.handle)
        except Exception:
            pass


def im2col_norm(images: torch.Tensor, ps: int = 14, kp: Optional[int] = None) -> torch.Tensor:
    lib = _lib.load()
    images = _dev(images, torch.bfloat16)
    B, _, H, W = images.shape
    kp = kp or (3 * ps * ps + 63) // 64 * 64
    out = torch.empty((B * (H // ps) * (W // ps), kp), dtype=torch.bfloat16, device=images.device)
    check(lib.fp_op_im2col_norm(ptr(images), ptr(out), B, H, W, ps, kp, current_stream()), "fp_op_im2col_norm")
    return out


def layernorm(x: torch.Tensor, gamma: torch.Tensor, beta: torch.Tensor, eps: float = 1e-6) -> torch.Tensor:
    lib = _lib.load()
    x, gamma, beta = _dev(x, torch.bfloat16), _dev(gamma, torch.bfloat16), _dev(beta, torch.bfloat16)
    rows, D = x.shape
    y = torch.empty_like(x)
    check(lib.fp_op_layernorm(ptr(x), ptr(y), ptr(gamma), ptr(beta), rows, D, float(eps), current_stream()), "fp_op_layernorm")
    return y


def plan_vit_batches(n: int, n_tok: int, max_batch: int = 192, n_cu: int = 256) -> list:
    return list(_plan_vit_batches(int(n), int(n_tok), int(max_batch), int(n_cu)))


@functools.lru_cache(maxsize=256)
def _plan_vit_batches(n: int, n_tok: int, max_batch: int, n_cu: int) -> tuple:
    if n <= 0:
        return ()
    npad = (n_tok + 15) // 16 * 16
    lo, hi = max(1, max_batch // 2), max_batch + max(1, max_batch // 8)

    def rounds(b):
        return -(-(-(-b * npad // 256) * 4) // n_cu)

    if n <= hi:
        return (n,)
    INF = (1 << 60, 1 << 60)
    best = [INF] * (n + 1)
    back = [0] * (n + 1)
    best[0] = (0, 0)
    for m in range(1, n + 1):
        for b in range(lo, min(hi, m) + 1):
            prev = best[m - b]
            if prev == INF:
                continue
            cand = (prev[0] + rounds(b), prev[1] + 1)
            if cand < best[m]:
                best[m], back[m] = cand, b
    if best[n] == INF:
        return (n,) if n <= hi else (n // 2, n - n // 2)
    out, m = [], n
    while m > 0:
        out.append(back[m])
        m -= back[m]
    return tuple(sorted(out, reverse=True))


class Timer:

    def __init__(self):
# ... 22 lines not shown
```

### include/freepose_hip.h

```cpp
#ifndef FREEPOSE_HIP_H
#define FREEPOSE_HIP_H
#include <stddef.h>
#include <stdint.h>

#ifdef __cplusplus
extern "C" {
#endif

#define FP_OK 0
#define FP_ERR_INVALID 1
#define FP_ERR_HIP 2
#define FP_ERR_STATE 3

typedef struct fp_ctx fp_ctx;
typedef struct fp_vit fp_vit;
typedef struct fp_mesh fp_mesh;

const char* fp_last_error(void);
int fp_version(void);
int fp_ctx_create(int device, fp_ctx** out);
int fp_ctx_destroy(fp_ctx* ctx);
int fp_ctx_set_option(fp_ctx* ctx, const char* name, int value);
size_t fp_ctx_workspace_bytes(const fp_ctx* ctx);

typedef struct {
    int dim;
    int depth;
    int heads;
    int mlp_dim;
    int patch;
    int n_reg;
    int pos_grid;
    float ln_eps;
} fp_vit_arch;

int fp_vit_create(fp_ctx* ctx, const fp_vit_arch* arch, fp_vit** out);
int fp_vit_destroy(fp_vit* vit);
int fp_vit_set_weight(fp_vit* vit, const char* name, const void* d_bf16, size_t numel, void* stream);
int fp_vit_forward(fp_vit* vit, const void* d_images, int B, int H, int W, int layer, int feature_type,
                   void* d_out_bf16, void* stream);
double fp_vit_flops(const fp_vit* vit, int B, int H, int W, int layer);

int fp_ffa(fp_ctx* ctx, const void* d_feats, const uint8_t* d_mask, int B, int gh, int gw, int D, int cell,
           int normalize, void* d_out_bf16, float* d_out_f32, void* stream);

int fp_bank_prepare(fp_ctx* ctx, const float* d_bank_f32, int N, int D, void* d_bank_bf16, void* stream);
int fp_bank_topk(fp_ctx* ctx, const void* d_bank_bf16, int N, int D, const void* d_queries, int Q, int k,
                 int idx_offset, float* d_out_scores, int32_t* d_out_idx, void* stream);
int fp_topk_merge(fp_ctx* ctx, const float* d_cand_scores, const int32_t* d_cand_idx, int Q, int C, int k,
                  float* d_out_scores, int32_t* d_out_idx, void* stream);
int fp_rerank_views(fp_ctx* ctx, const void* d_views, const int32_t* d_offsets, const int32_t* d_cand,
                    const void* d_queries, int Q, int C, int D, int k, float* d_out, void* stream);
int fp_l2_normalize(fp_ctx* ctx, const void* d_x_bf16, int rows, int D, void* d_y_bf16, void* stream);

int fp_template_score(fp_ctx* ctx, const void* d_tmpl, const void* d_query, const float* d_weights, int T, int P,
                      int D, float* d_scores, void* stream);
int fp_template_score_normed(fp_ctx* ctx, const void* d_tmpl_normed, const void* d_query, const float* d_weights, int T,
                             int P, int D, float* d_scores, void* stream);

int fp_crop_resize_pad(fp_ctx* ctx, const void* d_images, int src_fmt, int n_img, int C, int H, int W,
                       const int32_t* d_boxes, int n, float bbox_extend, int target, const uint8_t* d_masks,
                       int mask_mode, void* d_out, int out_fmt, void* stream);

int fp_roi_align(fp_ctx* ctx, const float* d_images, int n_img, int C, int H, int W, const float* d_rois, int n,
                 int pooled_h, int pooled_w, int sampling_ratio, float spatial_scale, float* d_out, void* stream);

int fp_generate_rotations(int n, double* h_out);
int fp_geodesic_select(fp_ctx* ctx, const double* d_grid, int G, const double* h_Rprev9, double thresh_deg,
                       int32_t* d_out_idx, int* h_n, void* stream);

int fp_mesh_upload(fp_ctx* ctx, const float* h_verts, int V, const int32_t* h_faces, int F,
                   const uint8_t* h_colors, fp_mesh** out);
int fp_mesh_upload_textured(fp_ctx* ctx, const float* h_verts, int V, const int32_t* h_faces, int F, const float* h_uv,
                            const uint8_t* h_texture, int th, int tw, const float* h_kd3, fp_mesh** out);
int fp_mesh_destroy(fp_mesh* mesh);
int fp_mesh_set_ambient(fp_mesh* mesh, float ambient);
int fp_mesh_set_shading(fp_mesh* mesh, int mode);
int fp_mesh_set_filter(fp_mesh* mesh, int mode);
int fp_mesh_set_cull(fp_mesh* mesh, int mode);
int fp_project_vertices(fp_ctx* ctx, const fp_mesh* mesh, const float* d_poses, int Hn, float scale, float fx, float fy,
                        float cx, float cy, int32_t* d_xy, float* d_zc, void* stream);
int fp_rasterize(fp_ctx* ctx, const fp_mesh* mesh, const float* d_poses, int Hn, float scale, float fx, float fy,
                 float cx, float cy, int W, int Hh, uint8_t* d_rgb, float* d_depth, void* stream);
int fp_rasterize_extents(fp_ctx* ctx, const fp_mesh* mesh, const float* d_poses, int Hn, float scale, float fx, float fy,
                         float cx, float cy, int W, int Hh, uint8_t* d_rgb, float* d_depth, double* d_ext, int32_t* d_boxes,
                         void* stream);
int fp_depth_extents(fp_ctx* ctx, const float* d_depth, int Hn, int Hh, int W, float fx, float fy, float cx,
                     float cy, double* d_out, void* stream);

int fp_chamfer(fp_ctx* ctx, const double* d_pts, int n_pts, const int32_t* d_table, const double* d_xf, int B, int max_n, int ws_pts,
               int projected, double* d_out, void* stream);
int fp_depth_compare(fp_ctx* ctx, const float* d_depth_est, const float* d_depth_gt, int B, int Hh, int W, const float* d_depth_test,
                     int n_img, const int32_t* d_img_idx, const double* d_params, const double* d_taus, int n_tau, int32_t* d_out,
                     void* stream);

int fp_label_components(fp_ctx* ctx, const uint8_t* d_masks, int n, int H, int W, int connectivity, int32_t* d_labels, void* stream);
int fp_depthmap_scale(fp_ctx* ctx, const double* d_depth, const uint8_t* d_masks, int n, int H, int W, double fx, double fy, double cx,
                      double cy, double erosion_radius, double std_factor, int min_vertices, int align, double* d_scale, int32_t* d_info,
                      uint8_t* d_keep, void* stream);

int fp_comm_unique_id(void* out_id128);
int fp_comm_init(fp_ctx* ctx, int nranks, int rank, const void* unique_id128);
int fp_comm_destroy(fp_ctx* ctx);
int fp_comm_size(const fp_ctx* ctx);
int fp_comm_rank(const fp_ctx* ctx);
int fp_allgather_bytes(fp_ctx* ctx, const void* d_send, size_t bytes, void* d_recv, void* stream);
int fp_allgather_topk(fp_ctx* ctx, const float* d_scores, const int32_t* d_idx, int Q, int k, int k_out, float* d_out_scores,
                      int32_t* d_out_idx, void* stream);
int fp_allgather_poses(fp_ctx* ctx, const double* d_rows, int n_rows, int row_len, double* d_out, void* stream);

int fp_op_gemm(fp_ctx* ctx, const void* d_X, int ldx, const void* d_W, int ldw, void* d_C, int ldc, const void* d_bias,
               const void* d_gamma, const void* d_resid, int ldr, int M, int N, int K, int epi, void* stream);
int fp_op_gemm_vt(fp_ctx* ctx, const void* d_X, int ldx, const void* d_W, int ldw, void* d_Vt, const void* d_bias, int M, int N,
                  int K, int npad, int heads, void* stream);
int fp_op_ln_linear(fp_ctx* ctx, const void* d_X, int M, int K, const void* d_g_ln, const void* d_b_ln, float eps, const void* d_W,
                    int N, const void* d_bias, int mode, int npad, int heads, int n_scaled, float row_scale, void* d_out, void* stream);
int fp_op_gemm_stats(fp_ctx* ctx, const void* d_X, int ldx, const void* d_W, int ldw, void* d_C, int ldc, const void* d_bias,
                     const void* d_gamma, const void* d_resid, int ldr, int M, int N, int K, float eps, float* d_stat, void* stream);
int fp_op_gemm_patch(fp_ctx* ctx, const void* d_X, int ldx, const void* d_W, int ldw, void* d_C, int ldc, const void* d_bias,
                     const void* d_pos, int M, int N, int K, int P, int npad, int tok_off, void* stream);
int fp_op_ln_chain(fp_ctx* ctx, const void* d_X1, int K1, const void* d_W1, const void* d_b1, const void* d_gamma, const void* d_resid,
                   void* d_Y, int M, int D, const void* d_g_ln, const void* d_b_ln, float eps, const void* d_W2, int N2,
                   const void* d_b2, int mode, int n_scaled, float row_scale, int route, void* d_out, int ldo, void* d_mfrag,
                   float* d_rstd, void* stream);
int fp_op_gelu(const void* d_x, void* d_y, size_t n, void* stream);
int fp_op_attention(const void* d_QK, int ldqk, const void* d_Vt, void* d_O, int ldo, int B, int H, int n_tok,
                    int npad, int q_prescaled, void* stream);
int fp_op_layernorm(const void* d_X, void* d_Y, const void* d_gamma, const void* d_beta, int rows, int D, float eps,
                    void* stream);
int fp_op_im2col_norm(const void* d_img, void* d_A, int B, int H, int W, int ps, int KP, void* stream);

int fp_op_attention_hd(const void* d_QKV, int ldqkv, void* d_O, int ldo, int B, int heads, int head_dim, int n_tok, int npad, float scale,
                       void* stream);
int fp_op_attention_causal(const void* d_QKV, int ldqkv, void* d_O, int ldo, int B, int heads, int head_dim, int n_tok, int npad, float scale,
                           void* stream);

typedef struct fp_clip fp_clip;
typedef struct {
    int width;
    int depth;
    int heads;
    int mlp_dim;
    int patch;
    int grid;
    int embed_dim;
    float ln_eps;
    int quick_gelu;
} fp_clip_arch;
int fp_clip_create(fp_ctx* ctx, const fp_clip_arch* arch, fp_clip** out);
int fp_clip_destroy(fp_clip* clip);
int fp_clip_set_weight(fp_clip* clip, const char* name, const void* d_tensor, size_t numel, void* stream);
int fp_clip_encode_image(fp_clip* clip, const void* d_images, int B, int S, void* d_out, void* stream);
double fp_clip_flops(const fp_clip* clip, int B);

typedef struct fp_clip_text fp_clip_text;
typedef struct {
    int width;
    int depth;
    int heads;
    int mlp_dim;
    int vocab;
    int ctx;
    int embed_dim;
    float ln_eps;
} fp_clip_text_arch;
int fp_clip_text_create(fp_ctx* ctx, const fp_clip_text_arch* arch, fp_clip_text** out);
int fp_clip_text_destroy(fp_clip_text* text);
int fp_clip_text_set_weight(fp_clip_text* text, const char* name, const void* d_tensor, size_t numel, void* stream);
int fp_clip_text_encode(fp_clip_text* text, const int32_t* d_ids, int B, void* d_out, void* stream);
double fp_clip_text_flops(const fp_clip_text* text, int B);

int fp_knn_l2(fp_ctx* ctx, const float* d_table, int N, int E, const float* d_queries, int Q, int k, int32_t* d_out_idx, float* d_out_d2,
              void* stream);

int fp_patch_points(fp_ctx* ctx, const double* d_samples, int S, const double* d_T, const double* d_K, const int32_t* d_cells,
                    const int32_t* d_ncells, int B, int C, double patch, int32_t* d_out, void* stream);
int fp_pnp_epnp(fp_ctx* ctx, const double* d_pts3d, const double* d_pts2d, const uint8_t* d_vis, const double* d_K9, int B, int N,
                double* d_out, void* stream);

int fp_video_errors(fp_ctx* ctx, const double* d_est, const double* d_gt, const int32_t* h_meta, const double* h_params, int M, int V,
                    int Nmax, int D, double* d_per_offset, double* d_final, double* d_aligned, double* d_pairs, void* stream);

int fp_bop_scores(fp_ctx* ctx, const double* d_err, const int32_t* d_groups, const uint8_t* d_gt_valid, const int32_t* d_gt_obj,
                  const int32_t* d_gt_scene, const double* d_th, int P, int Gr, int R, int T, int n_obj, int n_scene, int n_top,
                  int32_t* d_match, int32_t* d_tp_obj, int32_t* d_tp_scene, int32_t* d_tar_obj, int32_t* d_tar_scene, void* stream);

int fp_gt_visibility(fp_ctx* ctx, const float* d_depth_gt, int B, int Hr, int Wr, int ox, int oy, const float* d_depth_test, int n_img,
                     int H, int W, const int32_t* d_img_idx, const double* d_params, uint8_t* d_mask, uint8_t* d_mask_visib,
                     int32_t* d_out, void* stream);
int fp_pts_diameter(fp_ctx* ctx, const double* d_pts, int n_pts, const int32_t* d_ranges, int M, double* d_out, void* stream);

int fp_timer_create(void** out);
int fp_timer_start(void* timer, void* stream);
int fp_timer_stop(void* timer, void* stream);
int fp_timer_elapsed_ms(void* timer, float* h_ms);
int fp_timer_destroy(void* timer);
int fp_vit_profile(fp_vit* vit, int enable);
int fp_vit_profile_read(fp_vit* vit, float* h_ms_gemm, float* h_ms_attn, float* h_ms_other, double* h_gemm_flops);
long fp_vit_profile_gemm_launches(const fp_vit* vit);

#ifdef __cplusplus
}
#endif
#endif
```

Baseline: 2.010.

## Fuse QKV projection into one GEMM and read V from row-major QKV in attention

```diff
diff --git a/freepose_amd/_lib.py b/freepose_amd/_lib.py
--- a/freepose_amd/_lib.py
+++ b/freepose_amd/_lib.py
@@ -112,6 +112,7 @@
                                c_void_p, c_void_p]),
     "fp_op_gelu": (c_int, [c_void_p, c_void_p, c_size_t, c_void_p]),
     "fp_op_attention": (c_int, [c_void_p, c_int, c_void_p, c_void_p, c_int, c_int, c_int, c_int, c_int, c_int, c_void_p]),
+    "fp_op_attention_qkv": (c_int, [c_void_p, c_int, c_void_p, c_int, c_int, c_int, c_int, c_int, c_int, c_void_p]),
     "fp_op_layernorm": (c_int, [c_void_p, c_void_p, c_void_p, c_void_p, c_int, c_int, c_float, c_void_p]),
     "fp_op_im2col_norm": (c_int, [c_void_p, c_void_p, c_int, c_int, c_int, c_int, c_int, c_void_p]),
     "fp_op_attention_hd": (c_int, [c_void_p, c_int, c_void_p, c_int, c_int, c_int, c_int, c_int, c_int, c_float, c_void_p]),
diff --git a/freepose_amd/csrc/attention.hip b/freepose_amd/csrc/attention.hip
--- a/freepose_amd/csrc/attention.hip
+++ b/freepose_amd/csrc/attention.hip
@@ -1,421 +1,4 @@
-#include "internal.h"
-
-#include <stdlib.h>
-
-#include <type_traits>
-
-namespace {
-
-typedef __attribute__((ext_vector_type(2))) float f32x2_t;
-
-constexpr int HD = 64;
-constexpr int KVB = 64;
-constexpr int QW = 32;
-constexpr int NWAVE = 4;
-constexpr int QB = QW * NWAVE;
-constexpr int ROWB = 128;
-constexpr int TILE = KVB * ROWB;
-constexpr int STAGE = 2 * TILE;
-constexpr float LAZY_THR = 40.0f;
-
-struct AttnArgs {
-    const bf16_t* QK; int ldqk;
-    const bf16_t* Vt;
-    bf16_t* O; int ldo;
-    int B, H, n_tok, npad, D;
-    float scale_log2e;
-    int q_base;
-};
-
-__device__ __forceinline__ float vmax2(float a, float b) {
-    float d;
-    asm("v_max_f32 %0, %1, %2" : "=v"(d) : "v"(a), "v"(b));
-    return d;
-}
-__device__ __forceinline__ float xlane_max16(float v) {
-    const auto r = __builtin_amdgcn_permlane16_swap(__float_as_uint(v), __float_as_uint(v), false, false);
-    return vmax2(__uint_as_float(r[0]), __uint_as_float(r[1]));
-}
-__device__ __forceinline__ float xlane_max32(float v) {
-    const auto r = __builtin_amdgcn_permlane32_swap(__float_as_uint(v), __float_as_uint(v), false, false);
-    return vmax2(__uint_as_float(r[0]), __uint_as_float(r[1]));
-}
-__device__ __forceinline__ int key_plain(int row) { return (row >> 1) & 7; }
-__device__ __forceinline__ int key_krow(int row) { return ((((row >> 3) & 3) << 1) | ((row >> 1) & 1)) & 7; }
-__device__ __forceinline__ int key_perm4(int row) {
-    const int rl = row & 63;
-    return (((rl >> 4) << 1) | ((rl & 3) >> 1)) & 7;
-}
-
-template <int NSLOT, int VAR = 0>
-__global__ __launch_bounds__(NWAVE * 64, (VAR & 16) ? 4 : 3) void attn_fwd_kernel(AttnArgs p) {
-    extern __shared__ __attribute__((aligned(1024))) char smem[];
-    const int tid = threadIdx.x, lane = tid & 63;
-    const int wave = __builtin_amdgcn_readfirstlane(tid >> 6);
-    const int li = lane & 15, lg = lane >> 4;
-    const int nqb = (p.npad - p.q_base + QB - 1) / QB;
-    int bid = blockIdx.x;
-    {
-        const int nwg = gridDim.x;
-        const int q = nwg >> 3, r = nwg & 7, xcd = bid & 7, pos = bid >> 3;
-        bid = (xcd < r ? xcd * (q + 1) : r * (q + 1) + (xcd - r) * q) + pos;
-    }
-    const int qb = bid % nqb, bh = bid / nqb;
-    const int h = bh % p.H, b = bh / p.H;
-    const int q0 = p.q_base + qb * QB + wave * QW;
-    const bool idle = q0 >= p.npad;
-
-    const size_t rowbase = (size_t)b * p.npad;
-    const char* gQK = (const char*)p.QK;
-    const char* gVt = (const char*)(p.Vt + ((size_t)b * p.H + h) * HD * p.npad);
-
-    bf16x8_t qf[2][2];
-#pragma unroll
-    for (int fq = 0; fq < 2; ++fq) {
-        const int q = min(q0 + 16 * fq + li, p.npad - 1);
-        const char* src = gQK + ((rowbase + q) * p.ldqk + h * HD) * 2;
-#pragma unroll
-        for (int kk = 0; kk < 2; ++kk) qf[fq][kk] = *(const bf16x8_t*)(src + (kk * 4 + lg) * 16);
-    }
-
-    uint32_t offK[2];
-    int rowK[2];
-    uint32_t offV[2];
-    int slotV[2];
-#pragma unroll
-    for (int it = 0; it < 2; ++it) {
-        const int row = (it * NWAVE + wave) * 8 + (lane >> 3);
-        rowK[it] = row;
-        offK[it] = (uint32_t)((p.D + h * HD) * 2 + (((lane & 7) ^ key_krow(row)) << 4));
-        slotV[it] = (lane & 7) ^ key_perm4(row);
-        offV[it] = (uint32_t)row * (uint32_t)p.npad * 2u;
-    }
-    const char* gKb = gQK + rowbase * (size_t)p.ldqk * 2;
-    uint32_t lofK[2], lofV[2];
-#pragma unroll
-    for (int it = 0; it < 2; ++it) {
-        lofK[it] = (uint32_t)rowK[it] * (uint32_t)p.ldqk * 2u + offK[it];
-        lofV[it] = offV[it] + (uint32_t)(slotV[it] * 16);
-    }
-    const uint32_t kstep = (uint32_t)p.ldqk * 2u;
-    auto stage = [&](int buf, int kv0) {
-        char* sb = smem + buf * STAGE;
-        if (kv0 + KVB <= p.npad) {
-#pragma unroll
-            for (int it = 0; it < 2; ++it) glds16_buf(gKb, lofK[it], (uint32_t)kv0 * kstep, sb + (it * NWAVE + wave) * 1024);
-#pragma unroll
-            for (int it = 0; it < 2; ++it) glds16_buf(gVt, lofV[it], (uint32_t)kv0 * 2u, sb + TILE + (it * NWAVE + wave) * 1024);
-        } else {
-#pragma unroll
-            for (int it = 0; it < 2; ++it) {
-                const int key = min(kv0 + rowK[it], p.npad - 1);
-                glds16(gQK + (rowbase + key) * (size_t)p.ldqk * 2 + offK[it], sb + (it * NWAVE + wave) * 1024);
-            }
-#pragma unroll
-            for (int it = 0; it < 2; ++it) {
-                const int k8 = min(kv0 + slotV[it] * 8, p.npad - 8);
-                glds16(gVt + offV[it] + (size_t)k8 * 2, sb + TILE + (it * NWAVE + wave) * 1024);
-            }
-        }
-    };
-
-    const int keyK = (((li >> 2) << 1) | ((li & 3) >> 1)) & 7;
-    const int baseK = ((li >> 2) * 8 + (li & 3)) * ROWB;
-    const int keyV = (((li >> 2) << 1) | ((li & 3) >> 1)) & 7;
-    const int baseV = TILE + ((li >> 2) * 16 + (li & 3)) * ROWB;
-
-    f32x4_t o[4][2];
-#pragma unroll
-    for (int i = 0; i < 4; ++i)
-#pragma unroll
-        for (int j = 0; j < 2; ++j) o[i][j] = f32x4_t{0.f, 0.f, 0.f, 0.f};
-    float mrow[2] = {-1e30f, -1e30f};
-    float mthr[2] = {-1e30f, -1e30f};
-    float nmb[2] = {0.f, 0.f};
-    constexpr bool PRE = (VAR & 64) != 0;
-    constexpr bool VSUM = (VAR & 256) != 0;
-    float vsum[2] = {0.f, 0.f};
-    f32x4_t nref[2] = {f32x4_t{0.f, 0.f, 0.f, 0.f}, f32x4_t{0.f, 0.f, 0.f, 0.f}};
-    f32x4_t lacc[2] = {f32x4_t{0.f, 0.f, 0.f, 0.f}, f32x4_t{0.f, 0.f, 0.f, 0.f}};
-    bf16x8_t ones;
-#pragma unroll
-    for (int e = 0; e < 8; ++e) ones[e] = (__bf16)1.0f;
-
-    const int ntile = (p.n_tok + KVB - 1) / KVB;
-    constexpr bool SHORT = (VAR & 4) != 0;
-    auto tile_of = [&](int sq) { return SHORT ? (sq == 0 ? ntile - 1 : sq - 1) : sq; };
-    constexpr int PF = NSLOT - 1;
-    stage(0, tile_of(0) * KVB);
-#pragma unroll
-    for (int i = 1; i < PF; ++i)
-        if (ntile > i) stage(i, tile_of(i) * KVB);
-    asm volatile("s_waitcnt vmcnt(0)" ::: "memory");
-#pragma unroll
-    for (int fq = 0; fq < 2; ++fq)
-#pragma unroll
-        for (int kk = 0; kk < 2; ++kk) asm volatile("" : "+v"(qf[fq][kk]));
-    if constexpr (VAR & 2) {
-        const int d = (blockIdx.x * 5) % 12;
-        for (int i = 0; i < d; ++i) __builtin_amdgcn_s_sleep(2);
-    }
-    auto tile_body = [&](int t, auto slot_c, auto nks_c, auto first_c) {
-        const int slot = slot_c;
-        constexpr int NKS = decltype(nks_c)::value;
-        constexpr bool FIRST = decltype(first_c)::value;
-        const int ahead = min(PF - 1, ntile - 1 - t);
-        if (ahead >= 2) asm volatile("s_waitcnt vmcnt(8)" ::: "memory");
-        else if (ahead == 1) asm volatile("s_waitcnt vmcnt(4)" ::: "memory");
-        else asm volatile("s_waitcnt vmcnt(0)" ::: "memory");
-        __builtin_amdgcn_s_barrier();
-        asm volatile("" ::: "memory");
-        if (t + PF < ntile) stage(slot >= 1 ? slot - 1 : NSLOT - 1, tile_of(t + PF) * KVB);
-        if (idle) return;
-        const char* sb = smem + slot * STAGE;
-        const int kv0 = tile_of(t) * KVB;
-
-        f32x4_t s[4][2];
-        if constexpr (VAR & 1) __builtin_amdgcn_s_setprio(1);
-#pragma unroll
-        for (int kk = 0; kk < 2; ++kk) {
-            const int slot = (((kk << 2) | lg) ^ keyK) << 4;
-#pragma unroll
-            for (int fk = 0; fk < 2 * NKS; ++fk) {
-                const bf16x8_t kf = *(const bf16x8_t*)(sb + baseK + (32 * (fk >> 1) + 4 * (fk & 1)) * ROWB + slot);
-#pragma unroll
-                for (int fq = 0; fq < 2; ++fq)
-                    s[fk][fq] = __builtin_amdgcn_mfma_f32_16x16x32_bf16(kf, qf[fq][kk], kk == 0 ? (PRE ? nref[fq] : f32x4_t{0.f, 0.f, 0.f, 0.f}) : s[fk][fq], 0, 0, 0);
-            }
-        }
-        if constexpr (VAR & 1) __builtin_amdgcn_s_setprio(0);
-        if (kv0 + KVB > p.n_tok) {
-#pragma unroll
-            for (int fk = 0; fk < 2 * NKS; ++fk)
-#pragma unroll
-                for (int r = 0; r < 4; ++r)
-                    if (kv0 + 32 * (fk >> 1) + 8 * lg + 4 * (fk & 1) + r >= p.n_tok) {
-                        s[fk][0][r] = -1e30f;
-                        s[fk][1][r] = -1e30f;
-                    }
-        }
-
-        constexpr bool JITV = (VAR & 16) != 0;
-        bf16x8_t vf[JITV ? 1 : 2][4];
-        if constexpr (!JITV) {
-#pragma unroll
-        for (int ks = 0; ks < NKS; ++ks) {
-            const int sv = (((ks << 2) | lg) ^ keyV) << 4;
-#pragma unroll
-            for (int fd = 0; fd < 4; ++fd) vf[ks][fd] = *(const bf16x8_t*)(sb + baseV + fd * 4 * ROWB + sv);
-        }
-        }
-
-        bf16x8_t pf[2][2];
-        auto softmax_max = [&](int fq) {
-            float mx;
-            if constexpr (NKS == 1)
-                asm("v_max3_f32 %0, %1, %2, %3\n\tv_max3_f32 %0, %0, %4, %5\n\tv_max3_f32 %0, %0, %6, %7\n\tv_max_f32 %0, %0, %8"
-                    : "=&v"(mx)
-                    : "v"(s[0][fq][0]), "v"(s[0][fq][1]), "v"(s[0][fq][2]), "v"(s[0][fq][3]), "v"(s[1][fq][0]), "v"(s[1][fq][1]),
-                      "v"(s[1][fq][2]), "v"(s[1][fq][3]));
-            else
-            asm("v_max3_f32 %0, %1, %2, %3\n\tv_max3_f32 %0, %0, %4, %5\n\tv_max3_f32 %0, %0, %6, %7\n\tv_max3_f32 %0, %0, %8, %9\n\t"
-                "v_max3_f32 %0, %0, %10, %11\n\tv_max3_f32 %0, %0, %12, %13\n\tv_max3_f32 %0, %0, %14, %15\n\tv_max_f32 %0, %0, %16"
-                : "=&v"(mx)
-                : "v"(s[0][fq][0]), "v"(s[0][fq][1]), "v"(s[0][fq][2]), "v"(s[0][fq][3]), "v"(s[1][fq][0]), "v"(s[1][fq][1]),
-                  "v"(s[1][fq][2]), "v"(s[1][fq][3]), "v"(s[2][fq][0]), "v"(s[2][fq][1]), "v"(s[2][fq][2]), "v"(s[2][fq][3]),
-                  "v"(s[3][fq][0]), "v"(s[3][fq][1]), "v"(s[3][fq][2]), "v"(s[3][fq][3]));
-            if constexpr (PRE) {
-                constexpr float THR2 = LAZY_THR * 1.4426950408889634f / 8.0f;
-                if (FIRST || __builtin_amdgcn_ballot_w64(mx > THR2) != 0) {
-                    mx = xlane_max16(mx);
-                    mx = xlane_max32(mx);
-                    const float delta = FIRST ? mx : vmax2(mx, 0.f);
-#pragma unroll
-                    for (int r = 0; r < 4; ++r) nref[fq][r] -= delta;
-#pragma unroll
-                    for (int fk = 0; fk < 2 * NKS; ++fk)
-#pragma unroll
-                        for (int r = 0; r < 4; ++r) s[fk][fq][r] -= delta;
-                    if constexpr (!FIRST) {
-                        const float alpha = __builtin_amdgcn_exp2f(-delta);
-                        lacc[fq][0] *= alpha;
-                        if constexpr (VSUM) vsum[fq] *= alpha;
-#pragma unroll
-                        for (int fd = 0; fd < 4; ++fd)
-#pragma unroll
-                            for (int r = 0; r < 4; ++r) o[fd][fq][r] *= alpha;
-                    }
-                }
-            } else
-            if (__builtin_amdgcn_ballot_w64(mx > mthr[fq]) != 0) {
-                mx = xlane_max16(mx);
-                mx = xlane_max32(mx);
-                const float mnew = vmax2(mrow[fq], mx);
-                const float alpha = __builtin_amdgcn_exp2f((mrow[fq] - mnew) * p.scale_log2e);
-                mrow[fq] = mnew;
-                mthr[fq] = mnew + LAZY_THR;
-                nmb[fq] = -(mnew * p.scale_log2e);
-                lacc[fq][0] *= alpha;
-#pragma unroll
-                for (int fd = 0; fd < 4; ++fd)
-#pragma unroll
-                    for (int r = 0; r < 4; ++r) o[fd][fq][r] *= alpha;
-            }
-        };
-        auto softmax_exp = [&](int fq) {
-            float pv[4][4];
-            if constexpr (PRE) {
-#pragma unroll
-                for (int fk = 0; fk < 2 * NKS; ++fk)
-#pragma unroll
-                    for (int r = 0; r < 4; ++r) pv[fk][r] = __builtin_amdgcn_exp2f(s[fk][fq][r]);
-            } else if constexpr (VAR & 128) {
-                const f32x2_t sc2 = {p.scale_log2e, p.scale_log2e};
-                const f32x2_t mb2 = {nmb[fq], nmb[fq]};
-#pragma unroll
-                for (int fk = 0; fk < 2 * NKS; ++fk)
-#pragma unroll
-                    for (int r = 0; r < 4; r += 2) {
-                        const f32x2_t a = {s[fk][fq][r], s[fk][fq][r + 1]};
-                        const f32x2_t e = __builtin_elementwise_fma(a, sc2, mb2);
-                        pv[fk][r] = __builtin_amdgcn_exp2f(e[0]);
-                        pv[fk][r + 1] = __builtin_amdgcn_exp2f(e[1]);
-                    }
-            } else {
-#pragma unroll
-                for (int fk = 0; fk < 2 * NKS; ++fk)
-#pragma unroll
-                    for (int r = 0; r < 4; ++r) {
-                        float e;
-                        asm("v_fma_f32 %0, %1, %2, %3" : "=v"(e) : "v"(s[fk][fq][r]), "v"(p.scale_log2e), "v"(nmb[fq]));
-                        pv[fk][r] = __builtin_amdgcn_exp2f(e);
-                    }
-            }
-#pragma unroll
-            for (int ks = 0; ks < NKS; ++ks) {
-                uint4 w;
-                w.x = pack_bf2(pv[2 * ks][0], pv[2 * ks][1]);
-                w.y = pack_bf2(pv[2 * ks][2], pv[2 * ks][3]);
-                w.z = pack_bf2(pv[2 * ks + 1][0], pv[2 * ks + 1][1]);
-                w.w = pack_bf2(pv[2 * ks + 1][2], pv[2 * ks + 1][3]);
-                pf[fq][ks] = __builtin_bit_cast(bf16x8_t, w);
-            }
-        };
-        auto pv_half = [&](int fq) {
-#pragma unroll
-            for (int ks = 0; ks < NKS; ++ks) {
-#pragma unroll
-                for (int fd = 0; fd < 4; ++fd)
-                    o[fd][fq] = __builtin_amdgcn_mfma_f32_16x16x32_bf16(vf[JITV ? 0 : ks][fd], pf[fq][ks], o[fd][fq], 0, 0, 0);
-                lacc[fq] = __builtin_amdgcn_mfma_f32_16x16x32_bf16(ones, pf[fq][ks], lacc[fq], 0, 0, 0);
-            }
-        };
-
-        if constexpr (JITV) {
-            softmax_max(0);
-            softmax_exp(0);
-            softmax_max(1);
-            softmax_exp(1);
-#pragma unroll
-            for (int ks = 0; ks < NKS; ++ks) {
-                const int sv = (((ks << 2) | lg) ^ keyV) << 4;
-#pragma unroll
-                for (int fd = 0; fd < 4; ++fd) vf[0][fd] = *(const bf16x8_t*)(sb + baseV + fd * 4 * ROWB + sv);
-#pragma unroll
-                for (int fq = 0; fq < 2; ++fq) {
-#pragma unroll
-                    for (int fd = 0; fd < 4; ++fd)
-                        o[fd][fq] = __builtin_amdgcn_mfma_f32_16x16x32_bf16(vf[0][fd], pf[fq][ks], o[fd][fq], 0, 0, 0);
-                    if constexpr (VSUM) {
-                        typedef __bf16 bf16x2_hw __attribute__((ext_vector_type(2)));
-                        const uint4 pw = __builtin_bit_cast(uint4, pf[fq][ks]);
-                        const bf16x2_hw one2 = __builtin_bit_cast(bf16x2_hw, 0x3f803f80u);
-                        vsum[fq] = __builtin_amdgcn_fdot2_f32_bf16(__builtin_bit_cast(bf16x2_hw, pw.x), one2, vsum[fq], false);
-                        vsum[fq] = __builtin_amdgcn_fdot2_f32_bf16(__builtin_bit_cast(bf16x2_hw, pw.y), one2, vsum[fq], false);
-                        vsum[fq] = __builtin_amdgcn_fdot2_f32_bf16(__builtin_bit_cast(bf16x2_hw, pw.z), one2, vsum[fq], false);
-                        vsum[fq] = __builtin_amdgcn_fdot2_f32_bf16(__builtin_bit_cast(bf16x2_hw, pw.w), one2, vsum[fq], false);
-                    } else {
-                        lacc[fq] = __builtin_amdgcn_mfma_f32_16x16x32_bf16(ones, pf[fq][ks], lacc[fq], 0, 0, 0);
-                    }
-                }
-            }
-            return;
-        }
-        softmax_max(0);
-        softmax_exp(0);
-        softmax_max(1);
-        __builtin_amdgcn_sched_barrier(0);
-        softmax_exp(1);
-        pv_half(0);
-#pragma unroll
-        for (int g = 0; g < 5 * NKS; ++g) {
-            __builtin_amdgcn_sched_group_barrier(0x008, 1, 0);
-            __builtin_amdgcn_sched_group_barrier(0x002, 4, 0);
-        }
-        __builtin_amdgcn_sched_barrier(0);
-        if constexpr (VAR & 1) __builtin_amdgcn_s_setprio(1);
-        pv_half(1);
-        if constexpr (VAR & 1) __builtin_amdgcn_s_setprio(0);
-    };
-    using full_c = std::integral_constant<int, 2>;
-    using half_c = std::integral_constant<int, 1>;
-    using yes_c = std::true_type;
-    using no_c = std::false_type;
-    if constexpr (SHORT) {
-        static_assert(NSLOT == 2, "the short-tail prologue is written for the 2-slot ring");
-        tile_body(0, std::integral_constant<int, 0>{}, half_c{}, yes_c{});
-        for (int t = 1; t < ntile; t += 2) {
-            tile_body(t, std::integral_constant<int, 1>{}, full_c{}, no_c{});
-            if (t + 1 < ntile) tile_body(t + 1, std::integral_constant<int, 0>{}, full_c{}, no_c{});
-        }
-    } else if constexpr (NSLOT == 2 && PRE) {
-        tile_body(0, std::integral_constant<int, 0>{}, full_c{}, yes_c{});
-        for (int t = 1; t < ntile; t += 2) {
-            tile_body(t, std::integral_constant<int, 1>{}, full_c{}, no_c{});
-            if (t + 1 < ntile) tile_body(t + 1, std::integral_constant<int, 0>{}, full_c{}, no_c{});
-        }
-    } else if constexpr (NSLOT == 2) {
-        for (int t = 0; t < ntile; t += 2) {
-            tile_body(t, std::integral_constant<int, 0>{}, full_c{}, no_c{});
-            if (t + 1 < ntile) tile_body(t + 1, std::integral_constant<int, 1>{}, full_c{}, no_c{});
-        }
-    } else {
-        tile_body(0, 0, full_c{}, yes_c{});
-        int slot = NSLOT > 1 ? 1 : 0;
-        for (int t = 1; t < ntile; ++t) {
-            tile_body(t, slot, full_c{}, no_c{});
-            slot = slot + 1 == NSLOT ? 0 : slot + 1;
-        }
-    }
-
-#pragma unroll
-    for (int fq = 0; fq < 2; ++fq) {
-        float rowsum = lacc[fq][0];
-        if constexpr (VSUM) {
-            rowsum = vsum[fq];
-            rowsum += lane_xor<16>(rowsum);
-            rowsum += lane_xor<32>(rowsum);
-        }
-        const float inv = 1.0f / rowsum;
-        const int q = q0 + 16 * fq + li;
-        if (q < p.npad) {
-            uint4 w0, w1;
-            w0.x = pack_bf2(o[0][fq][0] * inv, o[0][fq][1] * inv);
-            w0.y = pack_bf2(o[0][fq][2] * inv, o[0][fq][3] * inv);
-            w0.z = pack_bf2(o[1][fq][0] * inv, o[1][fq][1] * inv);
-            w0.w = pack_bf2(o[1][fq][2] * inv, o[1][fq][3] * inv);
-            w1.x = pack_bf2(o[2][fq][0] * inv, o[2][fq][1] * inv);
-            w1.y = pack_bf2(o[2][fq][2] * inv, o[2][fq][3] * inv);
-            w1.z = pack_bf2(o[3][fq][0] * inv, o[3][fq][1] * inv);
-            w1.w = pack_bf2(o[3][fq][2] * inv, o[3][fq][3] * inv);
-            uint4* dst = (uint4*)(p.O + (rowbase + q) * p.ldo + h * HD + lg * 16);
-            dst[0] = w0;
-            dst[1] = w1;
-        }
-    }
-}
-
-}
+#include "attn_fwd_kernel.inc"
 
 int fp_attention_fwd(const bf16_t* QK, int ldqk, const bf16_t* Vt, bf16_t* O, int ldo, int B, int H,
                      int n_tok, int npad, bool q_prescaled, hipStream_t stream) {
diff --git a/freepose_amd/csrc/attention_qkv.hip b/freepose_amd/csrc/attention_qkv.hip
--- /dev/null
+++ b/freepose_amd/csrc/attention_qkv.hip
@@ -0,0 +1,26 @@
+#include "attn_fwd_kernel.inc"
+
+int fp_attention_fwd_qkv(const bf16_t* QKV, int ldqkv, bf16_t* O, int ldo, int B, int H, int n_tok, int npad, bool q_prescaled,
+                         hipStream_t stream) {
+    FP_REQUIRE(B > 0 && H > 0 && n_tok > 0 && npad >= n_tok && npad % 16 == 0,
+               "attention_qkv: bad shape B=%d H=%d n_tok=%d npad=%d", B, H, n_tok, npad);
+    FP_REQUIRE(ldqkv >= 3 * H * HD && ldqkv % 8 == 0 && ldo >= H * HD && ldo % 8 == 0,
+               "attention_qkv: ldqkv=%d ldo=%d (>= 3D / D = %d, multiples of 8)", ldqkv, ldo, H * HD);
+    FP_REQUIRE((size_t)npad * (size_t)ldqkv * 2 < 0x80000000ull, "attention_qkv: a crop's rows exceed the 32-bit DMA offsets (npad=%d ldqkv=%d)", npad, ldqkv);
+    AttnArgs a;
+    a.QK = QKV; a.ldqk = ldqkv; a.Vt = nullptr; a.O = O; a.ldo = ldo;
+    a.B = B; a.H = H; a.n_tok = n_tok; a.npad = npad; a.D = H * HD;
+    a.scale_log2e = FP_ATTN_QSCALE;
+    a.q_base = 0;
+    dim3 grid(cdiv(npad, QB) * H * B);
+    const bool short_tail = n_tok > KVB && n_tok - (cdiv(n_tok, KVB) - 1) * KVB <= KVB / 2;
+    if (q_prescaled) {
+        if (short_tail) hipLaunchKernelGGL((attn_fwd_kernel<2, 4 | 16 | 64 | 512>), grid, dim3(NWAVE * 64), 2 * STAGE, stream, a);
+        else hipLaunchKernelGGL((attn_fwd_kernel<2, 16 | 64 | 512>), grid, dim3(NWAVE * 64), 2 * STAGE, stream, a);
+    } else {
+        if (short_tail) hipLaunchKernelGGL((attn_fwd_kernel<2, 4 | 16 | 512>), grid, dim3(NWAVE * 64), 2 * STAGE, stream, a);
+        else hipLaunchKernelGGL((attn_fwd_kernel<2, 16 | 512>), grid, dim3(NWAVE * 64), 2 * STAGE, stream, a);
+    }
+    FP_LAUNCH_CHECK();
+    return FP_OK;
+}
diff --git a/freepose_amd/csrc/attn_fwd_kernel.inc b/freepose_amd/csrc/attn_fwd_kernel.inc
--- /dev/null
+++ b/freepose_amd/csrc/attn_fwd_kernel.inc
@@ -0,0 +1,502 @@
+#include "internal.h"
+
+#include <stdlib.h>
+
+#include <type_traits>
+
+namespace {
+
+typedef __attribute__((ext_vector_type(2))) float f32x2_t;
+
+constexpr int HD = 64;
+constexpr int KVB = 64;
+constexpr int QW = 32;
+constexpr int NWAVE = 4;
+constexpr int QB = QW * NWAVE;
+constexpr int ROWB = 128;
+constexpr int TILE = KVB * ROWB;
+constexpr int STAGE = 2 * TILE;
+constexpr float LAZY_THR = 40.0f;
+
+struct AttnArgs {
+    const bf16_t* QK; int ldqk;
+    const bf16_t* Vt;
+    bf16_t* O; int ldo;
+    int B, H, n_tok, npad, D;
+    float scale_log2e;
+    int q_base;
+};
+
+__device__ __forceinline__ float vmax2(float a, float b) {
+    float d;
+    asm("v_max_f32 %0, %1, %2" : "=v"(d) : "v"(a), "v"(b));
+    return d;
+}
+__device__ __forceinline__ float xlane_max16(float v) {
+    const auto r = __builtin_amdgcn_permlane16_swap(__float_as_uint(v), __float_as_uint(v), false, false);
+    return vmax2(__uint_as_float(r[0]), __uint_as_float(r[1]));
+}
+__device__ __forceinline__ float xlane_max32(float v) {
+    const auto r = __builtin_amdgcn_permlane32_swap(__float_as_uint(v), __float_as_uint(v), false, false);
+    return vmax2(__uint_as_float(r[0]), __uint_as_float(r[1]));
+}
+typedef __attribute__((ext_vector_type(4))) __bf16 bf16x4_t;
+__device__ __forceinline__ void lds_read_tr16_x8(bf16x4_t (&t)[8], const uint32_t (&a)[4], int off, int off2) {
+#if defined(__HIP_DEVICE_COMPILE__)
+    asm volatile(
+        "ds_read_b64_tr_b16 %0, %8 offset:%12\n\t"
+        "ds_read_b64_tr_b16 %1, %8 offset:%13\n\t"
+        "ds_read_b64_tr_b16 %2, %9 offset:%12\n\t"
+        "ds_read_b64_tr_b16 %3, %9 offset:%13\n\t"
+        "ds_read_b64_tr_b16 %4, %10 offset:%12\n\t"
+        "ds_read_b64_tr_b16 %5, %10 offset:%13\n\t"
+        "ds_read_b64_tr_b16 %6, %11 offset:%12\n\t"
+        "ds_read_b64_tr_b16 %7, %11 offset:%13"
+        : "=&v"(t[0]), "=&v"(t[1]), "=&v"(t[2]), "=&v"(t[3]), "=&v"(t[4]), "=&v"(t[5]), "=&v"(t[6]), "=&v"(t[7])
+        : "v"(a[0]), "v"(a[1]), "v"(a[2]), "v"(a[3]), "n"(off), "n"(off2)
+        : "memory");
+#else
+    (void)t; (void)a; (void)off; (void)off2;
+#endif
+}
+template <int PENDING>
+__device__ __forceinline__ bf16x8_t lds_wait_tr16(bf16x4_t& lo, bf16x4_t& hi) {
+#if defined(__HIP_DEVICE_COMPILE__)
+    asm volatile("s_waitcnt lgkmcnt(%2)" : "+v"(lo), "+v"(hi) : "n"(PENDING));
+#endif
+    return __builtin_shufflevector(lo, hi, 0, 1, 2, 3, 4, 5, 6, 7);
+}
+__device__ __forceinline__ int key_plain(int row) { return (row >> 1) & 7; }
+__device__ __forceinline__ int key_krow(int row) { return ((((row >> 3) & 3) << 1) | ((row >> 1) & 1)) & 7; }
+__device__ __forceinline__ int key_perm4(int row) {
+    const int rl = row & 63;
+    return (((rl >> 4) << 1) | ((rl & 3) >> 1)) & 7;
+}
+
+template <int NSLOT, int VAR = 0>
+__global__ __launch_bounds__(NWAVE * 64, (VAR & 16) ? 4 : 3) void attn_fwd_kernel(AttnArgs p) {
+    extern __shared__ __attribute__((aligned(1024))) char smem[];
+    const int tid = threadIdx.x, lane = tid & 63;
+    const int wave = __builtin_amdgcn_readfirstlane(tid >> 6);
+    const int li = lane & 15, lg = lane >> 4;
+    const int nqb = (p.npad - p.q_base + QB - 1) / QB;
+    int bid = blockIdx.x;
+    {
+        const int nwg = gridDim.x;
+        const int q = nwg >> 3, r = nwg & 7, xcd = bid & 7, pos = bid >> 3;
+        bid = (xcd < r ? xcd * (q + 1) : r * (q + 1) + (xcd - r) * q) + pos;
+    }
+    const int qb = bid % nqb, bh = bid / nqb;
+    const int h = bh % p.H, b = bh / p.H;
+    const int q0 = p.q_base + qb * QB + wave * QW;
+    const bool idle = q0 >= p.npad;
+
+    const size_t rowbase = (size_t)b * p.npad;
+    const char* gQK = (const char*)p.QK;
+    const char* gVt = (const char*)(p.Vt + ((size_t)b * p.H + h) * HD * p.npad);
+
+    bf16x8_t qf[2][2];
+#pragma unroll
+    for (int fq = 0; fq < 2; ++fq) {
+        const int q = min(q0 + 16 * fq + li, p.npad - 1);
+        const char* src = gQK + ((rowbase + q) * p.ldqk + h * HD) * 2;
+#pragma unroll
+        for (int kk = 0; kk < 2; ++kk) qf[fq][kk] = *(const bf16x8_t*)(src + (kk * 4 + lg) * 16);
+    }
+
+    constexpr bool RMV = (VAR & 512) != 0;
+    static_assert(!RMV || ((VAR & 16) && NSLOT == 2), "the row-major V flavour reads its fragments per 32-key half (JITV), at compile-time ring slots");
+    uint32_t offK[2];
+    int rowK[2];
+    uint32_t offV[2];
+    int slotV[2];
+#pragma unroll
+    for (int it = 0; it < 2; ++it) {
+        const int row = (it * NWAVE + wave) * 8 + (lane >> 3);
+        rowK[it] = row;
+        offK[it] = (uint32_t)((p.D + h * HD) * 2 + (((lane & 7) ^ key_krow(row)) << 4));
+        slotV[it] = (lane & 7) ^ key_perm4(row);
+        offV[it] = (uint32_t)row * (uint32_t)p.npad * 2u;
+    }
+    const char* gKb = gQK + rowbase * (size_t)p.ldqk * 2;
+    uint32_t lofK[2], lofV[2];
+#pragma unroll
+    for (int it = 0; it < 2; ++it) {
+        lofK[it] = (uint32_t)rowK[it] * (uint32_t)p.ldqk * 2u + offK[it];
+        lofV[it] = offV[it] + (uint32_t)(slotV[it] * 16);
+    }
+    const uint32_t kstep = (uint32_t)p.ldqk * 2u;
+    auto stage = [&](int buf, int kv0) {
+        char* sb = smem + buf * STAGE;
+        if (kv0 + KVB <= p.npad) {
+#pragma unroll
+            for (int it = 0; it < 2; ++it) {
+                if constexpr (RMV) glds16_buf(gKb, lofK[0], (uint32_t)(kv0 + 32 * it) * kstep, sb + (it * NWAVE + wave) * 1024);
+                else glds16_buf(gKb, lofK[it], (uint32_t)kv0 * kstep, sb + (it * NWAVE + wave) * 1024);
+            }
+#pragma unroll
+            for (int it = 0; it < 2; ++it) {
+                if constexpr (RMV) glds16_buf(gKb, lofK[0], (uint32_t)(kv0 + 32 * it) * kstep + (uint32_t)p.D * 2u, sb + TILE + (it * NWAVE + wave) * 1024);
+                else glds16_buf(gVt, lofV[it], (uint32_t)kv0 * 2u, sb + TILE + (it * NWAVE + wave) * 1024);
+            }
+        } else {
+#pragma unroll
+            for (int it = 0; it < 2; ++it) {
+                const int key = min(kv0 + (RMV ? rowK[0] + 32 * it : rowK[it]), p.npad - 1);
+                glds16(gQK + (rowbase + key) * (size_t)p.ldqk * 2 + offK[RMV ? 0 : it], sb + (it * NWAVE + wave) * 1024);
+            }
+#pragma unroll
+            for (int it = 0; it < 2; ++it) {
+                if constexpr (RMV) {
+                    const int key = min(kv0 + rowK[0] + 32 * it, p.npad - 1);
+                    glds16(gQK + (rowbase + key) * (size_t)p.ldqk * 2 + offK[0] + (size_t)p.D * 2, sb + TILE + (it * NWAVE + wave) * 1024);
+                } else {
+                    const int k8 = min(kv0 + slotV[it] * 8, p.npad - 8);
+                    glds16(gVt + offV[it] + (size_t)k8 * 2, sb + TILE + (it * NWAVE + wave) * 1024);
+                }
+            }
+        }
+    };
+
+    const int keyK = (((li >> 2) << 1) | ((li & 3) >> 1)) & 7;
+    const int baseK = ((li >> 2) * 8 + (li & 3)) * ROWB;
+    const int keyV = (((li >> 2) << 1) | ((li & 3) >> 1)) & 7;
+    const int baseV = TILE + ((li >> 2) * 16 + (li & 3)) * ROWB;
+    uint32_t baseT[4];
+#pragma unroll
+    for (int fd = 0; fd < 4; ++fd) {
+        const int q = li >> 2, pp = li & 3, row = 8 * lg + q;
+        baseT[fd] = (uint32_t)(uintptr_t)(__attribute__((address_space(3))) char*)smem + TILE + row * ROWB + (((2 * pp + (fd >> 1)) ^ key_krow(row)) << 4) + 8 * ((fd & 1) ^ (pp & 1));
+    }
+
+    f32x4_t o[4][2];
+#pragma unroll
+    for (int i = 0; i < 4; ++i)
+#pragma unroll
+        for (int j = 0; j < 2; ++j) o[i][j] = f32x4_t{0.f, 0.f, 0.f, 0.f};
+    float mrow[2] = {-1e30f, -1e30f};
+    float mthr[2] = {-1e30f, -1e30f};
+    float nmb[2] = {0.f, 0.f};
+    constexpr bool PRE = (VAR & 64) != 0;
+    constexpr bool VSUM = (VAR & 256) != 0;
+    float vsum[2] = {0.f, 0.f};
+    f32x4_t nref[2] = {f32x4_t{0.f, 0.f, 0.f, 0.f}, f32x4_t{0.f, 0.f, 0.f, 0.f}};
+    f32x4_t lacc[2] = {f32x4_t{0.f, 0.f, 0.f, 0.f}, f32x4_t{0.f, 0.f, 0.f, 0.f}};
+    bf16x8_t ones;
+#pragma unroll
+    for (int e = 0; e < 8; ++e) ones[e] = (__bf16)1.0f;
+
+    const int ntile = (p.n_tok + KVB - 1) / KVB;
+    constexpr bool SHORT = (VAR & 4) != 0;
+    auto tile_of = [&](int sq) { return SHORT ? (sq == 0 ? ntile - 1 : sq - 1) : sq; };
+    constexpr int PF = NSLOT - 1;
+    stage(0, tile_of(0) * KVB);
+#pragma unroll
+    for (int i = 1; i < PF; ++i)
+        if (ntile > i) stage(i, tile_of(i) * KVB);
+    asm volatile("s_waitcnt vmcnt(0)" ::: "memory");
+#pragma unroll
+    for (int fq = 0; fq < 2; ++fq)
+#pragma unroll
+        for (int kk = 0; kk < 2; ++kk) asm volatile("" : "+v"(qf[fq][kk]));
+    if constexpr (VAR & 2) {
+        const int d = (blockIdx.x * 5) % 12;
+        for (int i = 0; i < d; ++i) __builtin_amdgcn_s_sleep(2);
+    }
+    auto tile_body = [&](int t, auto slot_c, auto nks_c, auto first_c) {
+        const int slot = slot_c;
+        constexpr int NKS = decltype(nks_c)::value;
+        constexpr bool FIRST = decltype(first_c)::value;
+        const int ahead = min(PF - 1, ntile - 1 - t);
+        if (ahead >= 2) asm volatile("s_waitcnt vmcnt(8)" ::: "memory");
+        else if (ahead == 1) asm volatile("s_waitcnt vmcnt(4)" ::: "memory");
+        else asm volatile("s_waitcnt vmcnt(0)" ::: "memory");
+        __builtin_amdgcn_s_barrier();
+        asm volatile("" ::: "memory");
+        if (t + PF < ntile) stage(slot >= 1 ? slot - 1 : NSLOT - 1, tile_of(t + PF) * KVB);
+        if (idle) return;
+        const char* sb = smem + slot * STAGE;
+        const int kv0 = tile_of(t) * KVB;
+
+        f32x4_t s[4][2];
+        if constexpr (VAR & 1) __builtin_amdgcn_s_setprio(1);
+#pragma unroll
+        for (int kk = 0; kk < 2; ++kk) {
+            const int slot = (((kk << 2) | lg) ^ keyK) << 4;
+#pragma unroll
+            for (int fk = 0; fk < 2 * NKS; ++fk) {
+                const bf16x8_t kf = *(const bf16x8_t*)(sb + baseK + (32 * (fk >> 1) + 4 * (fk & 1)) * ROWB + slot);
+#pragma unroll
+                for (int fq = 0; fq < 2; ++fq)
+                    s[fk][fq] = __builtin_amdgcn_mfma_f32_16x16x32_bf16(kf, qf[fq][kk], kk == 0 ? (PRE ? nref[fq] : f32x4_t{0.f, 0.f, 0.f, 0.f}) : s[fk][fq], 0, 0, 0);
+            }
+        }
+        if constexpr (VAR & 1) __builtin_amdgcn_s_setprio(0);
+        if (kv0 + KVB > p.n_tok) {
+#pragma unroll
+            for (int fk = 0; fk < 2 * NKS; ++fk)
+#pragma unroll
+                for (int r = 0; r < 4; ++r)
+                    if (kv0 + 32 * (fk >> 1) + 8 * lg + 4 * (fk & 1) + r >= p.n_tok) {
+                        s[fk][0][r] = -1e30f;
+                        s[fk][1][r] = -1e30f;
+                    }
+        }
+
+        constexpr bool JITV = (VAR & 16) != 0;
+        bf16x8_t vf[JITV ? 1 : 2][4];
+        if constexpr (!JITV) {
+#pragma unroll
+        for (int ks = 0; ks < NKS; ++ks) {
+            const int sv = (((ks << 2) | lg) ^ keyV) << 4;
+#pragma unroll
+            for (int fd = 0; fd < 4; ++fd) vf[ks][fd] = *(const bf16x8_t*)(sb + baseV + fd * 4 * ROWB + sv);
+        }
+        }
+
+        bf16x8_t pf[2][2];
+        auto softmax_max = [&](int fq) {
+            float mx;
+            if constexpr (NKS == 1)
+                asm("v_max3_f32 %0, %1, %2, %3\n\tv_max3_f32 %0, %0, %4, %5\n\tv_max3_f32 %0, %0, %6, %7\n\tv_max_f32 %0, %0, %8"
+                    : "=&v"(mx)
+                    : "v"(s[0][fq][0]), "v"(s[0][fq][1]), "v"(s[0][fq][2]), "v"(s[0][fq][3]), "v"(s[1][fq][0]), "v"(s[1][fq][1]),
+                      "v"(s[1][fq][2]), "v"(s[1][fq][3]));
+            else
+            asm("v_max3_f32 %0, %1, %2, %3\n\tv_max3_f32 %0, %0, %4, %5\n\tv_max3_f32 %0, %0, %6, %7\n\tv_max3_f32 %0, %0, %8, %9\n\t"
+                "v_max3_f32 %0, %0, %10, %11\n\tv_max3_f32 %0, %0, %12, %13\n\tv_max3_f32 %0, %0, %14, %15\n\tv_max_f32 %0, %0, %16"
+                : "=&v"(mx)
+                : "v"(s[0][fq][0]), "v"(s[0][fq][1]), "v"(s[0][fq][2]), "v"(s[0][fq][3]), "v"(s[1][fq][0]), "v"(s[1][fq][1]),
+                  "v"(s[1][fq][2]), "v"(s[1][fq][3]), "v"(s[2][fq][0]), "v"(s[2][fq][1]), "v"(s[2][fq][2]), "v"(s[2][fq][3]),
+                  "v"(s[3][fq][0]), "v"(s[3][fq][1]), "v"(s[3][fq][2]), "v"(s[3][fq][3]));
+            if constexpr (PRE) {
+                constexpr float THR2 = LAZY_THR * 1.4426950408889634f / 8.0f;
+                if (FIRST || __builtin_amdgcn_ballot_w64(mx > THR2) != 0) {
+                    mx = xlane_max16(mx);
+                    mx = xlane_max32(mx);
+                    const float delta = FIRST ? mx : vmax2(mx, 0.f);
+#pragma unroll
+                    for (int r = 0; r < 4; ++r) nref[fq][r] -= delta;
+#pragma unroll
+                    for (int fk = 0; fk < 2 * NKS; ++fk)
+#pragma unroll
+                        for (int r = 0; r < 4; ++r) s[fk][fq][r] -= delta;
+                    if constexpr (!FIRST) {
+                        const float alpha = __builtin_amdgcn_exp2f(-delta);
+                        lacc[fq][0] *= alpha;
+                        if constexpr (VSUM) vsum[fq] *= alpha;
+#pragma unroll
+                        for (int fd = 0; fd < 4; ++fd)
+#pragma unroll
+                            for (int r = 0; r < 4; ++r) o[fd][fq][r] *= alpha;
+                    }
+                }
+            } else
+            if (__builtin_amdgcn_ballot_w64(mx > mthr[fq]) != 0) {
+                mx = xlane_max16(mx);
+                mx = xlane_max32(mx);
+                const float mnew = vmax2(mrow[fq], mx);
+                const float alpha = __builtin_amdgcn_exp2f((mrow[fq] - mnew) * p.scale_log2e);
+                mrow[fq] = mnew;
+                mthr[fq] = mnew + LAZY_THR;
+                nmb[fq] = -(mnew * p.scale_log2e);
+                lacc[fq][0] *= alpha;
+#pragma unroll
+                for (int fd = 0; fd < 4; ++fd)
+#pragma unroll
+                    for (int r = 0; r < 4; ++r) o[fd][fq][r] *= alpha;
+            }
+        };
+        auto softmax_exp = [&](int fq) {
+            float pv[4][4];
+            if constexpr (PRE) {
+#pragma unroll
+                for (int fk = 0; fk < 2 * NKS; ++fk)
+#pragma unroll
+                    for (int r = 0; r < 4; ++r) pv[fk][r] = __builtin_amdgcn_exp2f(s[fk][fq][r]);
+            } else if constexpr (VAR & 128) {
+                const f32x2_t sc2 = {p.scale_log2e, p.scale_log2e};
+                const f32x2_t mb2 = {nmb[fq], nmb[fq]};
+#pragma unroll
+                for (int fk = 0; fk < 2 * NKS; ++fk)
+#pragma unroll
+                    for (int r = 0; r < 4; r += 2) {
+                        const f32x2_t a = {s[fk][fq][r], s[fk][fq][r + 1]};
+                        const f32x2_t e = __builtin_elementwise_fma(a, sc2, mb2);
+                        pv[fk][r] = __builtin_amdgcn_exp2f(e[0]);
+                        pv[fk][r + 1] = __builtin_amdgcn_exp2f(e[1]);
+                    }
+            } else {
+#pragma unroll
+                for (int fk = 0; fk < 2 * NKS; ++fk)
+#pragma unroll
+                    for (int r = 0; r < 4; ++r) {
+                        float e;
+                        asm("v_fma_f32 %0, %1, %2, %3" : "=v"(e) : "v"(s[fk][fq][r]), "v"(p.scale_log2e), "v"(nmb[fq]));
+                        pv[fk][r] = __builtin_amdgcn_exp2f(e);
+                    }
+            }
+#pragma unroll
+            for (int ks = 0; ks < NKS; ++ks) {
+                uint4 w;
+                w.x = pack_bf2(pv[2 * ks][0], pv[2 * ks][1]);
+                w.y = pack_bf2(pv[2 * ks][2], pv[2 * ks][3]);
+                w.z = pack_bf2(pv[2 * ks + 1][0], pv[2 * ks + 1][1]);
+                w.w = pack_bf2(pv[2 * ks + 1][2], pv[2 * ks + 1][3]);
+                pf[fq][ks] = __builtin_bit_cast(bf16x8_t, w);
+            }
+        };
+        auto pv_half = [&](int fq) {
+#pragma unroll
+            for (int ks = 0; ks < NKS; ++ks) {
+#pragma unroll
+                for (int fd = 0; fd < 4; ++fd)
+                    o[fd][fq] = __builtin_amdgcn_mfma_f32_16x16x32_bf16(vf[JITV ? 0 : ks][fd], pf[fq][ks], o[fd][fq], 0, 0, 0);
+                lacc[fq] = __builtin_amdgcn_mfma_f32_16x16x32_bf16(ones, pf[fq][ks], lacc[fq], 0, 0, 0);
+            }
+        };
+
+        if constexpr (JITV) {
+            softmax_max(0);
+            softmax_exp(0);
+            softmax_max(1);
+            softmax_exp(1);
+#pragma unroll
+            for (int ks = 0; ks < NKS; ++ks) {
+                const int sv = (((ks << 2) | lg) ^ keyV) << 4;
+                if constexpr (RMV) {
+                    static_assert(!RMV || !VSUM, "row-major V keeps the row sums on the matrix pipe");
+                    bf16x4_t tr[8];
+                    __builtin_amdgcn_sched_barrier(0);
+                    lds_read_tr16_x8(tr, baseT, slot * STAGE + 32 * ks * ROWB, slot * STAGE + (32 * ks + 4) * ROWB);
+#pragma unroll
+                    for (int fq = 0; fq < 2; ++fq) lacc[fq] = __builtin_amdgcn_mfma_f32_16x16x32_bf16(ones, pf[fq][ks], lacc[fq], 0, 0, 0);
+                    __builtin_amdgcn_sched_barrier(0);
+                    vf[0][0] = lds_wait_tr16<6>(tr[0], tr[1]);
+#pragma unroll
+                    for (int fq = 0; fq < 2; ++fq) o[0][fq] = __builtin_amdgcn_mfma_f32_16x16x32_bf16(vf[0][0], pf[fq][ks], o[0][fq], 0, 0, 0);
+                    __builtin_amdgcn_sched_barrier(0);
+                    vf[0][1] = lds_wait_tr16<4>(tr[2], tr[3]);
+#pragma unroll
+                    for (int fq = 0; fq < 2; ++fq) o[1][fq] = __builtin_amdgcn_mfma_f32_16x16x32_bf16(vf[0][1], pf[fq][ks], o[1][fq], 0, 0, 0);
+                    __builtin_amdgcn_sched_barrier(0);
+                    vf[0][2] = lds_wait_tr16<2>(tr[4], tr[5]);
+#pragma unroll
+                    for (int fq = 0; fq < 2; ++fq) o[2][fq] = __builtin_amdgcn_mfma_f32_16x16x32_bf16(vf[0][2], pf[fq][ks], o[2][fq], 0, 0, 0);
+                    __builtin_amdgcn_sched_barrier(0);
+                    vf[0][3] = lds_wait_tr16<0>(tr[6], tr[7]);
+#pragma unroll
+                    for (int fq = 0; fq < 2; ++fq) o[3][fq] = __builtin_amdgcn_mfma_f32_16x16x32_bf16(vf[0][3], pf[fq][ks], o[3][fq], 0, 0, 0);
+                    continue;
+                } else {
+#pragma unroll
+                for (int fd = 0; fd < 4; ++fd) vf[0][fd] = *(const bf16x8_t*)(sb + baseV + fd * 4 * ROWB + sv);
+                }
+#pragma unroll
+                for (int fq = 0; fq < 2; ++fq) {
+#pragma unroll
+                    for (int fd = 0; fd < 4; ++fd)
+                        o[fd][fq] = __builtin_amdgcn_mfma_f32_16x16x32_bf16(vf[0][fd], pf[fq][ks], o[fd][fq], 0, 0, 0);
+                    if constexpr (VSUM) {
+                        typedef __bf16 bf16x2_hw __attribute__((ext_vector_type(2)));
+                        const uint4 pw = __builtin_bit_cast(uint4, pf[fq][ks]);
+                        const bf16x2_hw one2 = __builtin_bit_cast(bf16x2_hw, 0x3f803f80u);
+                        vsum[fq] = __builtin_amdgcn_fdot2_f32_bf16(__builtin_bit_cast(bf16x2_hw, pw.x), one2, vsum[fq], false);
+                        vsum[fq] = __builtin_amdgcn_fdot2_f32_bf16(__builtin_bit_cast(bf16x2_hw, pw.y), one2, vsum[fq], false);
+                        vsum[fq] = __builtin_amdgcn_fdot2_f32_bf16(__builtin_bit_cast(bf16x2_hw, pw.z), one2, vsum[fq], false);
+                        vsum[fq] = __builtin_amdgcn_fdot2_f32_bf16(__builtin_bit_cast(bf16x2_hw, pw.w), one2, vsum[fq], false);
+                    } else {
+                        lacc[fq] = __builtin_amdgcn_mfma_f32_16x16x32_bf16(ones, pf[fq][ks], lacc[fq], 0, 0, 0);
+                    }
+                }
+            }
+            return;
+        }
+        softmax_max(0);
+        softmax_exp(0);
+        softmax_max(1);
+        __builtin_amdgcn_sched_barrier(0);
+        softmax_exp(1);
+        pv_half(0);
+#pragma unroll
+        for (int g = 0; g < 5 * NKS; ++g) {
+            __builtin_amdgcn_sched_group_barrier(0x008, 1, 0);
+            __builtin_amdgcn_sched_group_barrier(0x002, 4, 0);
+        }
+        __builtin_amdgcn_sched_barrier(0);
+        if constexpr (VAR & 1) __builtin_amdgcn_s_setprio(1);
+        pv_half(1);
+        if constexpr (VAR & 1) __builtin_amdgcn_s_setprio(0);
+    };
+    using full_c = std::integral_constant<int, 2>;
+    using half_c = std::integral_constant<int, 1>;
+    using yes_c = std::true_type;
+    using no_c = std::false_type;
+    if constexpr (SHORT) {
+        static_assert(NSLOT == 2, "the short-tail prologue is written for the 2-slot ring");
+        tile_body(0, std::integral_constant<int, 0>{}, half_c{}, yes_c{});
+        for (int t = 1; t < ntile; t += 2) {
+            tile_body(t, std::integral_constant<int, 1>{}, full_c{}, no_c{});
+            if (t + 1 < ntile) tile_body(t + 1, std::integral_constant<int, 0>{}, full_c{}, no_c{});
+        }
+    } else if constexpr (NSLOT == 2 && PRE) {
+        tile_body(0, std::integral_constant<int, 0>{}, full_c{}, yes_c{});
+        for (int t = 1; t < ntile; t += 2) {
+            tile_body(t, std::integral_constant<int, 1>{}, full_c{}, no_c{});
+            if (t + 1 < ntile) tile_body(t + 1, std::integral_constant<int, 0>{}, full_c{}, no_c{});
+        }
+    } else if constexpr (NSLOT == 2) {
+        for (int t = 0; t < ntile; t += 2) {
+            tile_body(t, std::integral_constant<int, 0>{}, full_c{}, no_c{});
+            if (t + 1 < ntile) tile_body(t + 1, std::integral_constant<int, 1>{}, full_c{}, no_c{});
+        }
+    } else {
+        tile_body(0, 0, full_c{}, yes_c{});
+        int slot = NSLOT > 1 ? 1 : 0;
+        for (int t = 1; t < ntile; ++t) {
+            tile_body(t, slot, full_c{}, no_c{});
+            slot = slot + 1 == NSLOT ? 0 : slot + 1;
+        }
+    }
+
+    int li_s = li, lg_s = lg;
+    if constexpr (RMV) {
+        int t2 = tid;
+        asm volatile("" : "+v"(t2));
+        li_s = t2 & 15;
+        lg_s = (t2 >> 4) & 3;
+    }
+#pragma unroll
+    for (int fq = 0; fq < 2; ++fq) {
+        float rowsum = lacc[fq][0];
+        if constexpr (VSUM) {
+            rowsum = vsum[fq];
+            rowsum += lane_xor<16>(rowsum);
+            rowsum += lane_xor<32>(rowsum);
+        }
+        const float inv = 1.0f / rowsum;
+        const int q = q0 + 16 * fq + li_s;
+        if (q < p.npad) {
+            uint4 w0, w1;
+            w0.x = pack_bf2(o[0][fq][0] * inv, o[0][fq][1] * inv);
+            w0.y = pack_bf2(o[0][fq][2] * inv, o[0][fq][3] * inv);
+            w0.z = pack_bf2(o[1][fq][0] * inv, o[1][fq][1] * inv);
+            w0.w = pack_bf2(o[1][fq][2] * inv, o[1][fq][3] * inv);
+            w1.x = pack_bf2(o[2][fq][0] * inv, o[2][fq][1] * inv);
+            w1.y = pack_bf2(o[2][fq][2] * inv, o[2][fq][3] * inv);
+            w1.z = pack_bf2(o[3][fq][0] * inv, o[3][fq][1] * inv);
+            w1.w = pack_bf2(o[3][fq][2] * inv, o[3][fq][3] * inv);
+            if constexpr (RMV) {
+                const bool odd = (lg_s & 1) != 0;
+                const uint4 a0 = w0, a1 = w1;
+                w0.x = odd ? a0.z : a0.x; w0.y = odd ? a0.w : a0.y; w0.z = odd ? a0.x : a0.z; w0.w = odd ? a0.y : a0.w;
+                w1.x = odd ? a1.z : a1.x; w1.y = odd ? a1.w : a1.y; w1.z = odd ? a1.x : a1.z; w1.w = odd ? a1.y : a1.w;
+            }
+            uint4* dst = (uint4*)(p.O + (rowbase + q) * p.ldo + h * HD + lg_s * 16);
+            dst[0] = w0;
+            dst[1] = w1;
+        }
+    }
+}
+
+}
diff --git a/freepose_amd/csrc/capi.hip b/freepose_amd/csrc/capi.hip
--- a/freepose_amd/csrc/capi.hip
+++ b/freepose_amd/csrc/capi.hip
@@ -533,6 +533,12 @@
     return fp_attention_fwd((const bf16_t*)QK, ldqk, (const bf16_t*)Vt, (bf16_t*)O, ldo, B, H, n_tok, npad, q_prescaled != 0,
                             (hipStream_t)stream);
 }
+extern "C" int fp_op_attention_qkv(const void* QKV, int ldqkv, void* O, int ldo, int B, int H, int n_tok, int npad, int q_prescaled,
+                                   void* stream) {
+    FP_REQUIRE(QKV && O, "op_attention_qkv: null argument");
+    FP_REQUIRE(((uintptr_t)QKV | (uintptr_t)O) % 16 == 0, "op_attention_qkv: QKV and O must be 16-byte aligned");
+    return fp_attention_fwd_qkv((const bf16_t*)QKV, ldqkv, (bf16_t*)O, ldo, B, H, n_tok, npad, q_prescaled != 0, (hipStream_t)stream);
+}
 extern "C" int fp_op_attention_hd(const void* QKV, int ldqkv, void* O, int ldo, int B, int heads, int head_dim, int n_tok, int npad,
                                   float scale, void* stream) {
     return fp_attention_hd_fwd((const bf16_t*)QKV, ldqkv, (bf16_t*)O, ldo, B, heads, head_dim, n_tok, npad, scale, (hipStream_t)stream);
diff --git a/freepose_amd/csrc/internal.h b/freepose_amd/csrc/internal.h
--- a/freepose_amd/csrc/internal.h
+++ b/freepose_amd/csrc/internal.h
@@ -38,6 +38,8 @@
 constexpr float FP_ATTN_QSCALE = 1.4426950408889634f / 8.0f;
 int fp_attention_fwd(const bf16_t* QK, int ldqk, const bf16_t* Vt, bf16_t* O, int ldo, int B, int H, int n_tok,
                      int npad, bool q_prescaled, hipStream_t stream);
+int fp_attention_fwd_qkv(const bf16_t* QKV, int ldqkv, bf16_t* O, int ldo, int B, int H, int n_tok, int npad, bool q_prescaled,
+                         hipStream_t stream);
 int fp_attention_hd_fwd(const bf16_t* QKV, int ldqkv, bf16_t* O, int ldo, int B, int heads, int head_dim, int n_tok, int npad, float scale,
                         hipStream_t stream);
 int fp_attention_causal_fwd(const bf16_t* QKV, int ldqkv, bf16_t* O, int ldo, int B, int heads, int head_dim, int n_tok, int npad, float scale,
diff --git a/freepose_amd/csrc/vit.hip b/freepose_amd/csrc/vit.hip
--- a/freepose_amd/csrc/vit.hip
+++ b/freepose_amd/csrc/vit.hip
@@ -162,7 +162,7 @@
     FP_REQUIRE(M * (size_t)a.mlp_dim * 2 < 0xffffffffull, "vit_forward: batch too large for 32-bit tile offsets (B=%d)", B);
     const int Mi = (int)M;
 
-    bf16_t *A0, *X, *Y, *QK, *Vt, *AO, *H1;
+    bf16_t *A0, *X, *Y, *QKV, *AO, *H1;
     int rc;
     const bool lnf = ctx->opt_ln_fused != 0 && D % 64 == 0;
     LnStats st{nullptr, nullptr, nullptr, Mi, D, a.ln_eps};
@@ -186,8 +186,7 @@
     FP_WS(ctx, "vit.im2col", (size_t)B * P * v->emb.KP * 2, A0);
     FP_WS(ctx, "vit.x", M * D * 2, X);
     FP_WS(ctx, "vit.y", M * D * 2, Y);
-    FP_WS(ctx, "vit.qk", M * 2 * D * 2, QK);
-    FP_WS(ctx, "vit.vt", M * D * 2 + 256, Vt);
+    FP_WS(ctx, "vit.qkv", M * 3 * D * 2, QKV);
     FP_WS(ctx, "vit.ao", M * D * 2, AO);
     FP_WS(ctx, "vit.h1", M * (size_t)a.mlp_dim * 2, H1);
 
@@ -202,21 +201,19 @@
         const fp_vit::VitFold& f = v->fold[i];
         {
             ProfScope ps(&v->prof, s, TOWER_OTHER);
-            if ((rc = lnf ? st.ready(i == 0 ? X : nullptr, 2 * D, s) : fp_layernorm(X, Y, w.n1w, w.n1b, Mi, D, a.ln_eps, 0, 0, 0, s))) return rc;
+            if ((rc = lnf ? st.ready(i == 0 ? X : nullptr, 3 * D, s) : fp_layernorm(X, Y, w.n1w, w.n1b, Mi, D, a.ln_eps, 0, 0, 0, s))) return rc;
         }
         {
             ProfScope ps(&v->prof, s, TOWER_GEMM);
             const bf16_t* qkvw = lnf ? f.qkvw : w.qkvw;
-            GemmStep qk(in, D, qkvw, D, QK, 2 * D, w.qkvb, Mi, 2 * D), vt(in, D, qkvw + (size_t)2 * D * D, D, Vt, 8, w.qkvb + 2 * D, Mi, D);
-            vt.transposed_v(npad, a.heads);
-            if (lnf && ((rc = st.attach(qk, f.qkv_cb)) || (rc = st.attach(vt, f.qkv_cb + 2 * D)))) return rc;
-            if ((rc = qk.run(ctx, s))) return rc;
-            if ((rc = vt.run(ctx, s))) return rc;
-            t.count(2.0 * 3.0 * D * D, 2);
+            GemmStep qkv(in, D, qkvw, D, QKV, 3 * D, w.qkvb, Mi, 3 * D);
+            if (lnf && (rc = st.attach(qkv, f.qkv_cb))) return rc;
+            if ((rc = qkv.run(ctx, s))) return rc;
+            t.count(2.0 * 3.0 * D * D, 1);
         }
         {
             ProfScope ps(&v->prof, s, TOWER_ATTN);
-            if ((rc = fp_attention_fwd(QK, 2 * D, Vt, AO, D, B, a.heads, n_tok, npad, lnf, s))) return rc;
+            if ((rc = fp_attention_fwd_qkv(QKV, 3 * D, AO, D, B, a.heads, n_tok, npad, lnf, s))) return rc;
         }
         if ((rc = fp_tower_out_proj(t, w, st.part))) return rc;
         if ((rc = fp_tower_mlp(t, w, lnf ? &st : nullptr, f.fc1w, f.fc1_cb, i + 1 < L ? st.part : nullptr))) return rc;
diff --git a/freepose_amd/ops.py b/freepose_amd/ops.py
--- a/freepose_amd/ops.py
+++ b/freepose_amd/ops.py
@@ -920,6 +920,22 @@
     return out
 
 
+def attention_qkv(qkv: torch.Tensor, heads: int, n_tok: int, out: Optional[torch.Tensor] = None, q_prescaled: bool = False) -> torch.Tensor:
+    lib = _lib.load()
+    if not qkv.is_cuda or qkv.dtype != torch.bfloat16:
+        qkv = _dev(qkv, torch.bfloat16)
+    if qkv.dim() != 3 or qkv.shape[2] != 3 * heads * 64 or qkv.stride(2) != 1 or qkv.stride(0) != qkv.shape[1] * qkv.stride(1):
+        raise ValueError(f"attention_qkv: qkv of shape {tuple(qkv.shape)}, strides {tuple(qkv.stride())} ([B, npad, 3*heads*64] rows) with heads={heads}")
+    B, npad, _ = qkv.shape
+    if out is None:
+        out = torch.zeros((B * npad, heads * 64), dtype=torch.bfloat16, device=qkv.device)
+    if out.shape != (B * npad, heads * 64) or out.stride(1) != 1 or out.dtype != torch.bfloat16:
+        raise ValueError(f"attention_qkv: out of shape {tuple(out.shape)}, expected bf16 {(B * npad, heads * 64)} rows")
+    check(lib.fp_op_attention_qkv(ptr(qkv), int(qkv.stride(1)), ptr(out), int(out.stride(0)), B, heads, int(n_tok), npad,
+                                  int(bool(q_prescaled)), current_stream()), "fp_op_attention_qkv")
+    return out
+
+
 def attention_hd(qkv: torch.Tensor, heads: int, n_tok: int, scale: Optional[float] = None, out: Optional[torch.Tensor] = None) -> torch.Tensor:
     lib = _lib.load()
     qkv = _dev(qkv, torch.bfloat16)
diff --git a/include/freepose_hip.h b/include/freepose_hip.h
--- a/include/freepose_hip.h
+++ b/include/freepose_hip.h
@@ -126,6 +126,8 @@
 int fp_op_gelu(const void* d_x, void* d_y, size_t n, void* stream);
 int fp_op_attention(const void* d_QK, int ldqk, const void* d_Vt, void* d_O, int ldo, int B, int H, int n_tok,
                     int npad, int q_prescaled, void* stream);
+int fp_op_attention_qkv(const void* d_QKV, int ldqkv, void* d_O, int ldo, int B, int H, int n_tok, int npad, int q_prescaled,
+                        void* stream);
 int fp_op_layernorm(const void* d_X, void* d_Y, const void* d_gamma, const void* d_beta, int rows, int D, float eps,
                     void* stream);
 int fp_op_im2col_norm(const void* d_img, void* d_A, int B, int H, int W, int ps, int KP, void* stream);
```

Result: no change. 2.015, median of 6 (+0.3%).
